# Crocodoctopus/zkstark

Measured on AMD Instinct MI355X. Metric: field-elements/s through LDE+Merkle+FRI (full STARK-101 prover), higher is better.
Workload: dtype u32 (mod 3*2^30+1) + SHA-256

## Files before the change

zkstark_amd/build.py:

```python
import concurrent.futures
import hashlib
import os
import shutil
import subprocess
import sys

HERE = os.path.dirname(os.path.abspath(__file__))
CSRC = os.path.join(HERE, "csrc")
OBJDIR = os.path.join(HERE, "build")
LIB = os.path.join(HERE, "libzkstark_amd.so")
HASHFILE = LIB + ".hash"
SOURCES = ["kernels.hip", "ntt_fast.hip", "domain.hip", "zkstark.hip", "batch.hip", "shard.hip", "verify.hip", "grind.hip", "host_sha.cpp", "version.cpp"]
HEADERS = ["field.hpp", "sha256.hpp", "blake2s.hpp", "sha256_quad.hpp", "fieldhash.hpp", "fieldhash_f64.hpp", "kernels.hpp", "transcript.hpp", "host_sha.hpp", "internal.hpp", "pool.hpp",
           "shard.hpp", "board.hpp", "peer.hpp", os.path.join("..", "..", "include", "zkstark_amd.h")]
ARCH = "gfx950"
FLAGS = ["-O3", "-std=c++17", f"--offload-arch={ARCH}", "-fPIC", "-Wall", "-Wno-unused-function"]
FLAGS += os.environ.get("ZK_BUILD_DEFS", "").split()


def _read(rel):
    with open(os.path.join(CSRC, rel), "rb") as f:
        return f.read()


def source_hash():
    h = hashlib.sha256()
    for rel in SOURCES + HEADERS:
        h.update(os.path.basename(rel).encode() + b"\0")
        h.update(_read(rel))
        h.update(b"\0")
    h.update(" ".join(FLAGS).encode())
    return h.hexdigest()[:24]


def built_hash():
    if not os.path.exists(LIB):
        return None
    try:
        with open(HASHFILE) as f:
            side = f.read().strip()
        if side and os.path.getmtime(HASHFILE) >= os.path.getmtime(LIB):
            return side
    except OSError:
        pass
    try:
        with open(LIB, "rb") as f:
            blob = f.read()
        i = blob.find(b"zkstark_amd.build_hash=")
        if i < 0:
            return None
        tail = blob[i + len(b"zkstark_amd.build_hash="):i + len(b"zkstark_amd.build_hash=") + 64]
        return tail.split(b"\0", 1)[0].decode("ascii", "replace") or None
    except OSError:
        return None


def is_stale():
    return built_hash() != source_hash()


def build(force=False, verbose=False, if_missing_only=False):
    if not force and os.path.exists(LIB) and (if_missing_only or not is_stale()):
        return LIB
    import fcntl
    with open(LIB + ".lock", "w") as lock:
        fcntl.flock(lock, fcntl.LOCK_EX)
        if not force and os.path.exists(LIB) and (if_missing_only or not is_stale()):
            return LIB
        return _build(verbose)


def _compile(hipcc, src, want, headers_blob, verbose):
    extra = [f'-DZK_SRC_HASH="{want}"'] if src == "version.cpp" else []
    key = hashlib.sha256(_read(src) + b"\0" + (want.encode() if extra else headers_blob) + " ".join(FLAGS).encode()).hexdigest()[:20]
    obj = os.path.join(OBJDIR, f"{os.path.splitext(src)[0]}.{key}.o")
    if os.path.exists(obj):
        return obj
    for old in os.listdir(OBJDIR):
        if old.startswith(os.path.splitext(src)[0] + ".") and old.endswith(".o"):
            os.unlink(os.path.join(OBJDIR, old))
    tmp = obj + f".tmp{os.getpid()}"
    cmd = [hipcc] + FLAGS + extra + ["-c", os.path.join(CSRC, src), "-o", tmp]
    if verbose:
        print(" ".join(cmd), file=sys.stderr)
    subprocess.check_call(cmd)
    os.replace(tmp, obj)
    return obj


def _build(verbose):
    hipcc = shutil.which("hipcc") or "/opt/rocm/bin/hipcc"
    if not os.path.exists(hipcc):
        raise RuntimeError("hipcc not found: cannot build libzkstark_amd.so")
    os.makedirs(OBJDIR, exist_ok=True)
    want = source_hash()
    headers_blob = b"\0".join(_read(h) for h in HEADERS)
    workers = max(1, min(len(SOURCES), (os.cpu_count() or 2) - 1, 6))
    with concurrent.futures.ThreadPoolExecutor(workers) as ex:
        objs = list(ex.map(lambda s: _compile(hipcc, s, want, headers_blob, verbose), SOURCES))
    tmp = LIB + f".tmp{os.getpid()}"
    cmd = [hipcc, f"--offload-arch={ARCH}", "-shared", "-fPIC", "-o", tmp] + objs + ["-ldl", "-lpthread", "-lrt"]
    if verbose:
        print(" ".join(cmd), file=sys.stderr)
    subprocess.check_call(cmd)
    os.replace(tmp, LIB)
    with open(HASHFILE + ".tmp", "w") as f:
        f.write(want + "\n")
    os.replace(HASHFILE + ".tmp", HASHFILE)
    return LIB


if __name__ == "__main__":
    print(build(force="--force" in sys.argv, verbose=True))
```

zkstark_amd/csrc/domain.hip:

```cpp
#include <chrono>
#include <cstdarg>
#include <cstdio>
#include <new>

#include "internal.hpp"

namespace zk {
namespace impl {

namespace {
thread_local std::string g_last_error;
}

int fail(int code, const char* fmt, ...) {
    char buf[512];
    va_list ap;
    va_start(ap, fmt);
    vsnprintf(buf, sizeof buf, fmt, ap);
    va_end(ap);
    g_last_error = buf;
    return code;
}
const char* last_error() { return g_last_error.c_str(); }

Plan make_plan(uint32_t log_m) {
    Plan p;
    uint32_t np = (log_m + kMaxRadixLog - 1) / kMaxRadixLog;
    if (np == 0) np = 1;
    uint32_t base = log_m / np, extra = log_m % np;
    p.nd = np;
    for (uint32_t d = 0; d < np; ++d) p.bits[d] = base + (d < extra ? 1 : 0);
    return p;
}

uint32_t pick_logC(uint32_t log_total, uint32_t logR) {
    uint32_t cols = log_total - logR, cap = ntt_pass_tile_log(log_total, logR) - logR;
    return cols < cap ? cols : cap;
}

int build_table(uint32_t root, uint32_t log_order, DevTable* t) {
    uint32_t lo_bits = (log_order + 1) / 2, hi_bits = log_order - lo_bits;
    std::vector<uint32_t> lo((size_t)1 << lo_bits), hi((size_t)1 << hi_bits);
    uint32_t acc = 1;
    for (size_t j = 0; j < lo.size(); ++j) { lo[j] = to_mont(acc); acc = mulmod(acc, root); }
    uint32_t step = powmod(root, (uint64_t)1 << lo_bits);
    acc = 1;
    for (size_t j = 0; j < hi.size(); ++j) { hi[j] = to_mont(acc); acc = mulmod(acc, step); }
    HIPCHK(hipMalloc(&t->lo, lo.size() * 4));
    HIPCHK(hipMalloc(&t->hi, hi.size() * 4));
    HIPCHK(hipMemcpy(t->lo, lo.data(), lo.size() * 4, hipMemcpyHostToDevice));
    HIPCHK(hipMemcpy(t->hi, hi.data(), hi.size() * 4, hipMemcpyHostToDevice));
    t->lo_bits = lo_bits;
    return ZK_OK;
}
void free_table(DevTable* t) {
    if (t->lo) (void)hipFree(t->lo);
    if (t->hi) (void)hipFree(t->hi);
    t->lo = t->hi = nullptr;
}

int run_dif(const uint32_t* src, uint32_t* data, uint32_t log_m, const Plan& pl, PowTable tw_inv, uint32_t L, uint32_t scale_mont, hipStream_t s, Profiler* prof,
            uint32_t batch, size_t src_stride, size_t data_stride) {
    uint32_t inner = log_m;
    for (uint32_t d = 0; d < pl.nd; ++d) {
        inner -= pl.bits[d];
        NttPassArgs a{};
        a.batch = batch; a.src_stride = d == 0 ? src_stride : data_stride; a.dst_stride = data_stride;
        a.src = d == 0 ? src : data; a.dst = data; a.log_total = log_m;
        a.logR = pl.bits[d]; a.logS = inner; a.logC = pick_logC(log_m, a.logR); a.tile_log = ntt_pass_tile_log(log_m, a.logR);
        a.L = L; a.tw = tw_inv; a.scale_mont = (inner == 0) ? scale_mont : 0;
        HIPCHK(launch_ntt_pass(a, NTT_DIF, s, prof));
    }
    return ZK_OK;
}
int run_dit(uint32_t* data, uint32_t log_m, const Plan& pl, PowTable tw, uint32_t L, hipStream_t s) {
    uint32_t inner = 0;
    for (int d = (int)pl.nd - 1; d >= 0; --d) {
        NttPassArgs a{};
        a.src = data; a.dst = data; a.log_total = log_m;
        a.logR = pl.bits[d]; a.logS = inner; a.logC = pick_logC(log_m, a.logR); a.tile_log = ntt_pass_tile_log(log_m, a.logR);
        a.L = L; a.tw = tw;
        HIPCHK(launch_ntt_pass(a, NTT_DIT, s));
        inner += pl.bits[d];
    }
    return ZK_OK;
}



void dom_free(zk_dom* d) {
    if (!d) return;
    free_table(&d->H); free_table(&d->Hinv); free_table(&d->W);
    if (d->d_inv_xm1) (void)hipFree(d->d_inv_xm1);
    delete d;
}

int dom_make(int device, uint32_t log_n, uint32_t log_b, uint32_t shift, bool fold_only, hipStream_t stream, zk_dom** out) {
    *out = nullptr;
    if (log_n < 1 || log_b > 5 || log_n + log_b > 30 || log_n + log_b < 1)
        return fail(ZK_ERR_INVALID, "domain: need 1 <= log_n, log_blowup <= 5, log_n + log_blowup <= 30 (got %u, %u)", log_n, log_b);
    if (shift == 0 || shift >= P) return fail(ZK_ERR_INVALID, "domain: shift must be a non-zero canonical residue");
    HIPCHK(hipSetDevice(device));
    zk_dom* d = new (std::nothrow) zk_dom();
    if (!d) return fail(ZK_ERR_NOMEM, "out of host memory");
    d->device = device;
    d->log_n = log_n; d->log_b = log_b; d->L = log_n + log_b;
    d->n = (size_t)1 << log_n; d->B = (size_t)1 << log_b; d->N = d->n << log_b;
    d->shift = shift;
    d->g = root_of_unity(log_n);
    d->h = root_of_unity(d->L);
    d->plan = make_plan(log_n);
    int rc;
    if ((rc = build_table(d->h, d->L, &d->H)) || (rc = build_table(invmod(d->h), d->L, &d->Hinv))) { dom_free(d); return rc; }
    uint32_t gm1 = invmod(d->g);
    d->shift_mont = to_mont(shift);
    d->gm1_mont = to_mont(gm1);
    d->gm2_mont = to_mont(mulmod(gm1, gm1));
    d->gm3_mont = to_mont(mulmod(mulmod(gm1, gm1), gm1));
    d->ninv_mont = to_mont(invmod((uint32_t)(d->n % P)));
    d->inv2_mont = to_mont(invmod(2));
    {
        const uint32_t inv2 = invmod(2);
        uint32_t wr = shift;
        for (uint32_t r = 0; r < d->L && r < 32; ++r) { d->fold_k[r] = mulmod(invmod(wr), inv2); wr = mulmod(wr, wr); }
        uint32_t xn = powmod(shift, d->n);
        const uint32_t hn = powmod(d->h, d->n);
        for (size_t r = 0; r < d->B; ++r) { const uint32_t den = sub(xn, 1); d->inv_den[r] = den ? invmod(den) : 0u; xn = mulmod(xn, hn); }
    }
    if (!fold_only) {
        if ((rc = build_table(shift, log_n, &d->W))) { dom_free(d); return rc; }
        if (powmod(shift, d->N) == 1) { dom_free(d); return fail(ZK_ERR_INVALID, "domain: shift lies in the evaluation subgroup"); }
        hipError_t e = hipMalloc((void**)&d->d_inv_xm1, d->N * 4);
        if (e != hipSuccess) { dom_free(d); return fail(ZK_ERR_NOMEM, "hipMalloc(%zu) failed", d->N * 4); }
        d->device_bytes += d->N * 4;
        e = launch_build_inv_xm1(d->d_inv_xm1, d->L, d->H.view(), d->shift_mont, stream);
        if (e == hipSuccess) e = hipStreamSynchronize(stream);
        if (e != hipSuccess) { dom_free(d); return fail(ZK_ERR_HIP, "inv_xm1 build failed: %s", hipGetErrorString(e)); }
    }
    *out = d;
    return ZK_OK;
}

int dom_lde(const zk_dom* d, const uint32_t* d_trace, uint32_t* d_coef, uint32_t* d_out, hipStream_t s, Profiler* prof, uint32_t batch) {
    const size_t ts = batch > 1 ? d->n : 0, cs = batch > 1 ? 2 * d->n : 0, os = batch > 1 ? d->N : 0;
    int rc = run_dif(d_trace, d_coef, d->log_n, d->plan, d->Hinv.view(), d->L, 0, s, prof, batch, ts, cs);
    if (rc) return rc;
    uint32_t* d_prep = d_coef + d->n;
    CoefPrepArgs pa{};
    pa.log_n = d->log_n; pa.log_b = d->log_b;
    pa.tw = d->H.view(); pa.wtab = d->W.view(); pa.ninv_mont = d->ninv_mont;
    pa.nd = d->plan.nd;
    for (uint32_t t = 0; t < d->plan.nd; ++t) pa.dig_bits[t] = d->plan.bits[t];
    uint32_t inner = d->log_b;
    for (int q = (int)d->plan.nd - 1; q >= 0; --q) {
        NttPassArgs a{};
        a.log_total = d->L; a.logR = d->plan.bits[q]; a.logS = inner; a.logC = pick_logC(d->L, a.logR); a.tile_log = ntt_pass_tile_log(d->L, a.logR);
        a.L = d->L; a.tw = d->H.view();
        a.dst = d_out;
        a.batch = batch; a.dst_stride = os; a.src_stride = os;
        if (q == (int)d->plan.nd - 1) {
            if (a.logC < d->log_b) a.logC = d->log_b;
            a.src_stride = cs;
            const bool fuse = ntt_fast_ok(a, NTT_DIT_LDE);
            if (fuse) {
                a.src = d_coef;
                a.prep = 1; a.prep_log_n = d->log_n; a.prep_log_b = d->log_b; a.prep_ninv_mont = d->ninv_mont;
                a.prep_nd = d->plan.nd; a.prep_wtab = d->W.view();
                for (uint32_t t = 0; t < d->plan.nd; ++t) a.prep_bits[t] = d->plan.bits[t];
            } else {
                HIPCHK(launch_coef_prepare(d_coef, d_prep, pa, s, prof, batch, cs, cs));
                a.src = d_prep;
            }
            HIPCHK(launch_ntt_pass(a, NTT_DIT_LDE, s, prof));
        } else {
            a.src = d_out;
            HIPCHK(launch_ntt_pass(a, NTT_DIT, s, prof));
        }
        inner += d->plan.bits[q];
    }
    return ZK_OK;
}

int compose_args(const zk_dom* d, const uint32_t* d_f, uint32_t* d_cp, uint32_t first, uint32_t last,
                 const uint32_t alpha_raw[3], ComposeArgs& a) {
    a = ComposeArgs{};
    a.f = d_f; a.inv_xm1 = d->d_inv_xm1; a.cp = d_cp;
    a.logN = d->L; a.log_b = d->log_b;
    a.htab = d->H.view();
    a.w_mont = d->shift_mont; a.gm1_mont = d->gm1_mont; a.gm2_mont = d->gm2_mont; a.gm3_mont = d->gm3_mont;
    a.first = first % P; a.last = last % P;
    uint32_t a0 = alpha_raw[0] % P, a1 = alpha_raw[1] % P, a2 = alpha_raw[2] % P;
    a.alpha0_mont = to_mont(a0);
    a.alpha1g2_mont = to_mont(mulmod(a1, mulmod(d->g, d->g)));
    for (size_t r = 0; r < d->B; ++r) {
        if (d->inv_den[r] == 0) return fail(ZK_ERR_INVALID, "compose: x^n = 1 on the domain");
        a.zz[r] = to_mont(to_mont(mulmod(a2, d->inv_den[r])));
    }
    return ZK_OK;
}
int dom_compose(const zk_dom* d, const uint32_t* d_f, uint32_t* d_cp, uint32_t first, uint32_t last,
                const uint32_t alpha_raw[3], hipStream_t s, Profiler* prof) {
    ComposeArgs a;
    int rc = compose_args(d, d_f, d_cp, first, last, alpha_raw, a);
    if (rc) return rc;
    HIPCHK(launch_compose(a, s, prof));
    return ZK_OK;
}

int fold_args(const zk_dom* d, const uint32_t* d_in, uint32_t* d_out, uint32_t log_m, uint32_t round, uint32_t beta_raw, FoldArgs& a) {
    if (log_m < 1 || log_m + round != d->L) return fail(ZK_ERR_INVALID, "fold: layer size 2^%u does not match round %u of a 2^%u domain", log_m, round, d->L);
    a = FoldArgs{};
    a.in = d_in; a.out = d_out; a.log_m = log_m; a.round = round;
    a.hinv = d->Hinv.view(); a.L = d->L;
    a.inv2_mont = d->inv2_mont;
    a.c_mont = to_mont(mulmod(beta_raw % P, d->fold_k[round]));
    return ZK_OK;
}
int dom_fold(const zk_dom* d, const uint32_t* d_in, uint32_t* d_out, uint32_t log_m, uint32_t round, uint32_t beta_raw,
             hipStream_t s, Profiler* prof) {
    FoldArgs a;
    int rc = fold_args(d, d_in, d_out, log_m, round, beta_raw, a);
    if (rc) return rc;
    HIPCHK(launch_fri_fold(a, s, prof));
    return ZK_OK;
}

int fold_multi_args(const zk_dom* d, const uint32_t* d_in, uint32_t* d_out, uint32_t log_m, uint32_t round, uint32_t steps, uint32_t beta_raw,
                    FoldMultiArgs& a) {
    if (steps < 1 || steps > 3) return fail(ZK_ERR_INVALID, "fold: steps must be 1..3 (got %u)", steps);
    if (log_m < steps || log_m + round != d->L)
        return fail(ZK_ERR_INVALID, "fold: layer size 2^%u does not match round %u + %u steps of a 2^%u domain", log_m, round, steps, d->L);
    a = FoldMultiArgs{};
    a.in = d_in; a.out = d_out; a.log_m = log_m; a.round = round; a.steps = steps;
    a.hinv = d->Hinv.view();
    a.scale_mont = to_mont(invmod(1u << steps));
    const uint32_t S = 1u << steps;
    const uint32_t om_inv = invmod(powmod(d->h, (uint64_t)d->N >> steps));
    uint32_t bk = beta_raw % P, ok = om_inv;
    for (uint32_t k = 0; k < steps; ++k) {
        const uint32_t base = mulmod(bk, mulmod(d->fold_k[round + k], 2));
        uint32_t tw = 1;
        for (uint32_t t = 0; t < (S >> (k + 1)); ++t) { a.c_mont[S - (S >> k) + t] = to_mont(mulmod(base, tw)); tw = mulmod(tw, ok); }
        bk = mulmod(bk, bk); ok = mulmod(ok, ok);
    }
    return ZK_OK;
}
int fold_multi_batch_args(const zk_dom* d, const uint32_t* d_in, uint32_t* d_out, uint32_t log_m, uint32_t round, uint32_t steps,
                          const uint32_t* d_beta_raw, uint32_t beta_stride, uint32_t* d_work, uint32_t batch, FoldMultiBatchArgs& a) {
    a = FoldMultiBatchArgs{};
    if (int rc = fold_multi_args(d, d_in, d_out, log_m, round, steps, 1u, a.a)) return rc;
    if (batch < 1 || ((uint64_t)batch << log_m) > ((uint64_t)1 << 32))
        return fail(ZK_ERR_INVALID, "fold: a batch of %u layers of 2^%u values does not fit 2^32 values", batch, log_m);
    a.beta_raw = d_beta_raw; a.beta_stride = beta_stride; a.cb = d_work; a.batch = batch;
    return ZK_OK;
}
int dom_fold_multi_batch(const zk_dom* d, const uint32_t* d_in, uint32_t* d_out, uint32_t log_m, uint32_t round, uint32_t steps,
                         const uint32_t* d_beta_raw, uint32_t beta_stride, uint32_t* d_work, uint32_t batch, hipStream_t s, Profiler* prof) {
    FoldMultiBatchArgs a;
    int rc = fold_multi_batch_args(d, d_in, d_out, log_m, round, steps, d_beta_raw, beta_stride, d_work, batch, a);
    if (rc) return rc;
    HIPCHK(launch_fri_fold_multi_batch(a, s, prof));
    return ZK_OK;
}
int dom_fold_multi(const zk_dom* d, const uint32_t* d_in, uint32_t* d_out, uint32_t log_m, uint32_t round, uint32_t steps, uint32_t beta_raw,
                   hipStream_t s, Profiler* prof) {
    if (steps == 1) return dom_fold(d, d_in, d_out, log_m, round, beta_raw, s, prof);
    FoldMultiArgs a;
    int rc = fold_multi_args(d, d_in, d_out, log_m, round, steps, beta_raw, a);
    if (rc) return rc;
    HIPCHK(launch_fri_fold_multi(a, s, prof));
    return ZK_OK;
}

int dom_final_poly(const zk_dom* d, const uint32_t* d_in, uint32_t* d_out, uint32_t log_m, uint32_t round, uint32_t bound, hipStream_t s,
                   Profiler* prof, uint32_t polys, size_t in_stride, size_t out_stride) {
    if (log_m < 1 || log_m > kFinalPolyMaxLog || log_m + round != d->L)
        return fail(ZK_ERR_INVALID, "final polynomial: layer size 2^%u does not match round %u of a 2^%u domain, or exceeds 2^%u values", log_m, round, d->L, kFinalPolyMaxLog);
    FinalPolyArgs a{};
    a.in = d_in; a.out = d_out; a.in_stride = in_stride; a.out_stride = out_stride; a.polys = polys;
    a.log_m = log_m; a.bound = bound;
    a.hinv = d->Hinv.view(); a.L = d->L;
    a.minv_mont = to_mont(invmod(1u << log_m));
    a.sinv_mont = to_mont(mulmod(d->fold_k[round], 2));
    HIPCHK(launch_fri_final_poly(a, s, prof));
    return ZK_OK;
}

int dom_final_poly_batch(const zk_dom* d, const uint32_t* d_in, uint32_t* d_out, uint32_t log_m, uint32_t round, uint32_t bound, uint32_t batch,
                         hipStream_t s, Profiler* prof) {
    if (log_m < 1 || log_m > kFinalPolyMaxLog || log_m + round != d->L || bound < 1 || bound > (1u << log_m) || batch < 1)
        return fail(ZK_ERR_INVALID, "final polynomials: %u layers of 2^%u values, bound %u, do not match round %u of a 2^%u domain (at most 2^%u values)",
                    batch, log_m, bound, round, d->L, kFinalPolyMaxLog);
    FinalPolyArgs a{};
    a.in = d_in; a.out = d_out; a.in_stride = (size_t)1 << log_m; a.out_stride = (size_t)bound + 1; a.polys = batch;
    a.log_m = log_m; a.bound = bound;
    a.hinv = d->Hinv.view(); a.L = d->L;
    a.minv_mont = to_mont(invmod(1u << log_m));
    a.sinv_mont = to_mont(mulmod(d->fold_k[round], 2));
    HIPCHK(launch_fri_final_poly_batch(a, s, prof));
    return ZK_OK;
}

int wait_flag(const uint32_t* flag, uint32_t want, hipStream_t stream, int (*poll)(void*), void* poll_user, double timeout_s) {
    auto t0 = std::chrono::steady_clock::now();
    uint64_t spins = 0;
    while (__atomic_load_n(flag, __ATOMIC_ACQUIRE) != want) {
#if !defined(__HIP_DEVICE_COMPILE__) && (defined(__x86_64__) || defined(__i386__))
        __builtin_ia32_pause();
#endif
        if (poll && (++spins & 0xFFF) == 0) {
            if (int prc = poll(poll_user)) return prc;
        } else if (!poll) {
            ++spins;
        }
        if ((spins & 0xFFFF) == 0) {
            hipError_t q = hipStreamQuery(stream);
            if (q == hipSuccess && __atomic_load_n(flag, __ATOMIC_ACQUIRE) != want)
                return fail(ZK_ERR_HIP, "merkle digests were never posted (stream drained)");
            if (q != hipSuccess && q != hipErrorNotReady)
                return fail(ZK_ERR_HIP, "device error while waiting for merkle digests: %s", hipGetErrorString(q));
            if (std::chrono::duration<double>(std::chrono::steady_clock::now() - t0).count() > timeout_s)
                return fail(ZK_ERR_HIP, "timed out after %.0f s waiting for merkle digests", timeout_s);
        }
    }
    return ZK_OK;
}

double now_us() { return std::chrono::duration<double, std::micro>(std::chrono::steady_clock::now().time_since_epoch()).count(); }

void path_nodes(size_t m, size_t leaf, std::vector<size_t>& out) {
    size_t i = leaf + (2 * m - 1) / 2;
    while (i != 0) {
        if (i % 2 == 0) { out.push_back(i - 1); i -= 2; }
        else { out.push_back(i + 1); i -= 1; }
        i >>= 1;
    }
}

}
}
```

zkstark_amd/csrc/host_sha.cpp:

```cpp
#include "host_sha.hpp"

#include <atomic>

#if !defined(__HIP_DEVICE_COMPILE__)
#include <immintrin.h>
#include <stdlib.h>
#include <string.h>

namespace zk {
namespace {

#define ZK_SHA_TARGET __attribute__((target("sha,sse4.1,ssse3")))

alignas(16) const uint32_t K[64] = {
    0x428a2f98u, 0x71374491u, 0xb5c0fbcfu, 0xe9b5dba5u, 0x3956c25bu, 0x59f111f1u, 0x923f82a4u, 0xab1c5ed5u,
    0xd807aa98u, 0x12835b01u, 0x243185beu, 0x550c7dc3u, 0x72be5d74u, 0x80deb1feu, 0x9bdc06a7u, 0xc19bf174u,
    0xe49b69c1u, 0xefbe4786u, 0x0fc19dc6u, 0x240ca1ccu, 0x2de92c6fu, 0x4a7484aau, 0x5cb0a9dcu, 0x76f988dau,
    0x983e5152u, 0xa831c66du, 0xb00327c8u, 0xbf597fc7u, 0xc6e00bf3u, 0xd5a79147u, 0x06ca6351u, 0x14292967u,
    0x27b70a85u, 0x2e1b2138u, 0x4d2c6dfcu, 0x53380d13u, 0x650a7354u, 0x766a0abbu, 0x81c2c92eu, 0x92722c85u,
    0xa2bfe8a1u, 0xa81a664bu, 0xc24b8b70u, 0xc76c51a3u, 0xd192e819u, 0xd6990624u, 0xf40e3585u, 0x106aa070u,
    0x19a4c116u, 0x1e376c08u, 0x2748774cu, 0x34b0bcb5u, 0x391c0cb3u, 0x4ed8aa4au, 0x5b9cca4fu, 0x682e6ff3u,
    0x748f82eeu, 0x78a5636fu, 0x84c87814u, 0x8cc70208u, 0x90befffau, 0xa4506cebu, 0xbef9a3f7u, 0xc67178f2u};
const uint32_t IV[8] = {0x6a09e667u, 0xbb67ae85u, 0x3c6ef372u, 0xa54ff53au, 0x510e527fu, 0x9b05688cu, 0x1f83d9abu, 0x5be0cd19u};

alignas(16) uint32_t PADKW[64];
bool g_cpu_has_sha = false, g_cpu_has_x16 = false;
std::atomic<bool> g_have_sha{false}, g_have_x16{false};
std::atomic<bool> g_want_x16{true};

inline uint32_t rotr(uint32_t x, int n) { return (x >> n) | (x << (32 - n)); }

struct Init {
    Init() {
        __builtin_cpu_init();
        g_cpu_has_sha = __builtin_cpu_supports("sha") && __builtin_cpu_supports("sse4.1") && __builtin_cpu_supports("ssse3");
        g_cpu_has_x16 = g_cpu_has_sha && __builtin_cpu_supports("avx512f");
        g_have_sha = g_cpu_has_sha;
        g_have_x16 = g_cpu_has_x16;
        uint32_t w[64] = {0x80000000u};
        w[15] = 512u;
        for (int t = 16; t < 64; ++t) {
            uint32_t s0 = rotr(w[t - 15], 7) ^ rotr(w[t - 15], 18) ^ (w[t - 15] >> 3);
            uint32_t s1 = rotr(w[t - 2], 17) ^ rotr(w[t - 2], 19) ^ (w[t - 2] >> 10);
            w[t] = w[t - 16] + s0 + w[t - 7] + s1;
        }
        for (int t = 0; t < 64; ++t) PADKW[t] = K[t] + w[t];
    }
} g_init;

ZK_SHA_TARGET inline void load_state(const uint32_t st[8], __m128i& s0, __m128i& s1) {
    __m128i t = _mm_loadu_si128((const __m128i*)st);
    s1 = _mm_loadu_si128((const __m128i*)(st + 4));
    t = _mm_shuffle_epi32(t, 0xB1);
    s1 = _mm_shuffle_epi32(s1, 0x1B);
    s0 = _mm_alignr_epi8(t, s1, 8);
    s1 = _mm_blend_epi16(s1, t, 0xF0);
}
ZK_SHA_TARGET inline void store_state(uint32_t st[8], __m128i s0, __m128i s1) {
    __m128i t = _mm_shuffle_epi32(s0, 0x1B);
    s1 = _mm_shuffle_epi32(s1, 0xB1);
    s0 = _mm_blend_epi16(t, s1, 0xF0);
    s1 = _mm_alignr_epi8(s1, t, 8);
    _mm_storeu_si128((__m128i*)st, s0);
    _mm_storeu_si128((__m128i*)(st + 4), s1);
}

ZK_SHA_TARGET inline void rounds_msg(__m128i& s0, __m128i& s1, __m128i m[4]) {
    const __m128i a0 = s0, a1 = s1;
#pragma GCC unroll 16
    for (int g = 0; g < 16; ++g) {
        __m128i cur = m[g & 3];
        __m128i msg = _mm_add_epi32(cur, _mm_load_si128((const __m128i*)(K + 4 * g)));
        s1 = _mm_sha256rnds2_epu32(s1, s0, msg);
        if (g >= 3 && g <= 14) {
            __m128i t = _mm_alignr_epi8(cur, m[(g + 3) & 3], 4);
            m[(g + 1) & 3] = _mm_sha256msg2_epu32(_mm_add_epi32(m[(g + 1) & 3], t), cur);
        }
        msg = _mm_shuffle_epi32(msg, 0x0E);
        s0 = _mm_sha256rnds2_epu32(s0, s1, msg);
        if (g >= 1 && g <= 12) m[(g + 3) & 3] = _mm_sha256msg1_epu32(m[(g + 3) & 3], cur);
    }
    s0 = _mm_add_epi32(s0, a0);
    s1 = _mm_add_epi32(s1, a1);
}
ZK_SHA_TARGET inline void rounds_pad64(__m128i& s0, __m128i& s1) {
    const __m128i a0 = s0, a1 = s1;
#pragma GCC unroll 16
    for (int g = 0; g < 16; ++g) {
        __m128i msg = _mm_load_si128((const __m128i*)(PADKW + 4 * g));
        s1 = _mm_sha256rnds2_epu32(s1, s0, msg);
        msg = _mm_shuffle_epi32(msg, 0x0E);
        s0 = _mm_sha256rnds2_epu32(s0, s1, msg);
    }
    s0 = _mm_add_epi32(s0, a0);
    s1 = _mm_add_epi32(s1, a1);
}

ZK_SHA_TARGET void inner_ni(const uint32_t* l, const uint32_t* r, uint32_t* out) {
    __m128i s0, s1, m[4];
    load_state(IV, s0, s1);
    m[0] = _mm_loadu_si128((const __m128i*)l);
    m[1] = _mm_loadu_si128((const __m128i*)(l + 4));
    m[2] = _mm_loadu_si128((const __m128i*)r);
    m[3] = _mm_loadu_si128((const __m128i*)(r + 4));
    rounds_msg(s0, s1, m);
    rounds_pad64(s0, s1);
    store_state(out, s0, s1);
}
ZK_SHA_TARGET void inner_ni_x2(const uint32_t* in, uint32_t* out) {
    __m128i s0, s1, u0, u1, m[4], n[4];
    load_state(IV, s0, s1);
    u0 = s0; u1 = s1;
    const __m128i a0 = s0, a1 = s1;
    for (int i = 0; i < 4; ++i) {
        m[i] = _mm_loadu_si128((const __m128i*)(in + 4 * i));
        n[i] = _mm_loadu_si128((const __m128i*)(in + 16 + 4 * i));
    }
#pragma GCC unroll 16
    for (int g = 0; g < 16; ++g) {
        const __m128i k = _mm_load_si128((const __m128i*)(K + 4 * g));
        __m128i cm = m[g & 3], cn = n[g & 3];
        __m128i xm = _mm_add_epi32(cm, k), xn = _mm_add_epi32(cn, k);
        s1 = _mm_sha256rnds2_epu32(s1, s0, xm);
        u1 = _mm_sha256rnds2_epu32(u1, u0, xn);
        if (g >= 3 && g <= 14) {
            __m128i tm = _mm_alignr_epi8(cm, m[(g + 3) & 3], 4), tn = _mm_alignr_epi8(cn, n[(g + 3) & 3], 4);
            m[(g + 1) & 3] = _mm_sha256msg2_epu32(_mm_add_epi32(m[(g + 1) & 3], tm), cm);
            n[(g + 1) & 3] = _mm_sha256msg2_epu32(_mm_add_epi32(n[(g + 1) & 3], tn), cn);
        }
        xm = _mm_shuffle_epi32(xm, 0x0E);
        xn = _mm_shuffle_epi32(xn, 0x0E);
        s0 = _mm_sha256rnds2_epu32(s0, s1, xm);
        u0 = _mm_sha256rnds2_epu32(u0, u1, xn);
        if (g >= 1 && g <= 12) {
            m[(g + 3) & 3] = _mm_sha256msg1_epu32(m[(g + 3) & 3], cm);
            n[(g + 3) & 3] = _mm_sha256msg1_epu32(n[(g + 3) & 3], cn);
        }
    }
    s0 = _mm_add_epi32(s0, a0); s1 = _mm_add_epi32(s1, a1);
    u0 = _mm_add_epi32(u0, a0); u1 = _mm_add_epi32(u1, a1);
    const __m128i b0 = s0, b1 = s1, c0 = u0, c1 = u1;
#pragma GCC unroll 16
    for (int g = 0; g < 16; ++g) {
        __m128i msg = _mm_load_si128((const __m128i*)(PADKW + 4 * g));
        s1 = _mm_sha256rnds2_epu32(s1, s0, msg);
        u1 = _mm_sha256rnds2_epu32(u1, u0, msg);
        msg = _mm_shuffle_epi32(msg, 0x0E);
        s0 = _mm_sha256rnds2_epu32(s0, s1, msg);
        u0 = _mm_sha256rnds2_epu32(u0, u1, msg);
    }
    s0 = _mm_add_epi32(s0, b0); s1 = _mm_add_epi32(s1, b1);
    u0 = _mm_add_epi32(u0, c0); u1 = _mm_add_epi32(u1, c1);
    store_state(out, s0, s1);
    store_state(out + 8, u0, u1);
}
ZK_SHA_TARGET void compress_ni(uint32_t* st, const uint32_t* blk) {
    __m128i s0, s1, m[4];
    load_state(st, s0, s1);
    for (int i = 0; i < 4; ++i) m[i] = _mm_loadu_si128((const __m128i*)(blk + 4 * i));
    rounds_msg(s0, s1, m);
    store_state(st, s0, s1);
}
ZK_SHA_TARGET void blocks_ni(uint32_t* st, const uint8_t* data, size_t blocks) {
    const __m128i be = _mm_set_epi64x(0x0c0d0e0f08090a0bLL, 0x0405060700010203LL);
    __m128i s0, s1, m[4];
    load_state(st, s0, s1);
    for (; blocks; --blocks, data += 64) {
        for (int i = 0; i < 4; ++i) m[i] = _mm_shuffle_epi8(_mm_loadu_si128((const __m128i*)(data + 16 * i)), be);
        rounds_msg(s0, s1, m);
    }
    store_state(st, s0, s1);
}
ZK_SHA_TARGET void leaf_ni(uint32_t v, uint32_t* out) {
    __m128i s0, s1, m[4];
    load_state(IV, s0, s1);
    m[0] = _mm_set_epi32(0, 0, (int)0x80000000u, (int)v);
    m[1] = _mm_setzero_si128();
    m[2] = _mm_setzero_si128();
    m[3] = _mm_set_epi32(32, 0, 0, 0);
    rounds_msg(s0, s1, m);
    store_state(out, s0, s1);
}
#define ZK_X16_TARGET __attribute__((target("avx512f")))
#define ZK_ROR(x, n) _mm512_ror_epi32((x), (n))
#define ZK_XOR3(a, b, c) _mm512_ternarylogic_epi32((a), (b), (c), 0x96)

ZK_X16_TARGET inline void transpose16(__m512i r[16]) {
    __m512i t[16], u[16];
    for (int i = 0; i < 8; ++i) {
        t[2 * i] = _mm512_unpacklo_epi32(r[2 * i], r[2 * i + 1]);
        t[2 * i + 1] = _mm512_unpackhi_epi32(r[2 * i], r[2 * i + 1]);
    }
    for (int i = 0; i < 16; i += 4) {
        u[i] = _mm512_unpacklo_epi64(t[i], t[i + 2]);
        u[i + 1] = _mm512_unpackhi_epi64(t[i], t[i + 2]);
        u[i + 2] = _mm512_unpacklo_epi64(t[i + 1], t[i + 3]);
        u[i + 3] = _mm512_unpackhi_epi64(t[i + 1], t[i + 3]);
    }
    for (int k = 0; k < 4; ++k) {
        t[k] = _mm512_shuffle_i32x4(u[k], u[4 + k], 0x88);
        t[4 + k] = _mm512_shuffle_i32x4(u[k], u[4 + k], 0xdd);
        t[8 + k] = _mm512_shuffle_i32x4(u[8 + k], u[12 + k], 0x88);
        t[12 + k] = _mm512_shuffle_i32x4(u[8 + k], u[12 + k], 0xdd);
    }
    for (int k = 0; k < 4; ++k) {
        r[k] = _mm512_shuffle_i32x4(t[k], t[8 + k], 0x88);
        r[8 + k] = _mm512_shuffle_i32x4(t[k], t[8 + k], 0xdd);
        r[4 + k] = _mm512_shuffle_i32x4(t[4 + k], t[12 + k], 0x88);
        r[12 + k] = _mm512_shuffle_i32x4(t[4 + k], t[12 + k], 0xdd);
    }
}

template <bool MSG>
ZK_X16_TARGET inline void rounds_x16(__m512i st[8], __m512i w[16]) {
    __m512i a = st[0], b = st[1], c = st[2], d = st[3], e = st[4], f = st[5], g = st[6], h = st[7];
#pragma GCC unroll 64
    for (int t = 0; t < 64; ++t) {
        __m512i wk;
        if (MSG) {
            if (t >= 16) {
                const __m512i w15 = w[(t + 1) & 15], w2 = w[(t + 14) & 15];
                const __m512i s0 = ZK_XOR3(ZK_ROR(w15, 7), ZK_ROR(w15, 18), _mm512_srli_epi32(w15, 3));
                const __m512i s1 = ZK_XOR3(ZK_ROR(w2, 17), ZK_ROR(w2, 19), _mm512_srli_epi32(w2, 10));
                w[t & 15] = _mm512_add_epi32(_mm512_add_epi32(w[t & 15], s0), _mm512_add_epi32(w[(t + 9) & 15], s1));
            }
            wk = _mm512_add_epi32(w[t & 15], _mm512_set1_epi32((int)K[t]));
        } else {
            wk = _mm512_set1_epi32((int)PADKW[t]);
        }
        const __m512i S1 = ZK_XOR3(ZK_ROR(e, 6), ZK_ROR(e, 11), ZK_ROR(e, 25));
        const __m512i t1 = _mm512_add_epi32(_mm512_add_epi32(h, S1), _mm512_add_epi32(_mm512_ternarylogic_epi32(e, f, g, 0xCA), wk));
        const __m512i S0 = ZK_XOR3(ZK_ROR(a, 2), ZK_ROR(a, 13), ZK_ROR(a, 22));
        const __m512i t2 = _mm512_add_epi32(S0, _mm512_ternarylogic_epi32(a, b, c, 0xE8));
        h = g; g = f; f = e; e = _mm512_add_epi32(d, t1); d = c; c = b; b = a; a = _mm512_add_epi32(t1, t2);
    }
    st[0] = _mm512_add_epi32(st[0], a); st[1] = _mm512_add_epi32(st[1], b); st[2] = _mm512_add_epi32(st[2], c); st[3] = _mm512_add_epi32(st[3], d);
    st[4] = _mm512_add_epi32(st[4], e); st[5] = _mm512_add_epi32(st[5], f); st[6] = _mm512_add_epi32(st[6], g); st[7] = _mm512_add_epi32(st[7], h);
}
ZK_X16_TARGET inline void store_x16(const __m512i st[8], uint32_t* out) {
    __m512i r[16];
    for (int i = 0; i < 8; ++i) { r[i] = st[i]; r[8 + i] = _mm512_setzero_si512(); }
    transpose16(r);
    for (int n = 0; n < 16; ++n) _mm256_storeu_si256((__m256i*)(out + 8 * n), _mm512_castsi512_si256(r[n]));
}
ZK_X16_TARGET void inner_x16(const uint32_t* in, uint32_t* out) {
    __m512i w[16], st[8];
    for (int n = 0; n < 16; ++n) w[n] = _mm512_loadu_si512((const void*)(in + 16 * n));
    transpose16(w);
    for (int i = 0; i < 8; ++i) st[i] = _mm512_set1_epi32((int)IV[i]);
    rounds_x16<true>(st, w);
    rounds_x16<false>(st, w);
    store_x16(st, out);
}
ZK_X16_TARGET void leaves_x16(const uint32_t* vals, uint32_t* out) {
    __m512i w[16], st[8];
    w[0] = _mm512_loadu_si512((const void*)vals);
    w[1] = _mm512_set1_epi32((int)0x80000000u);
    for (int i = 2; i < 15; ++i) w[i] = _mm512_setzero_si512();
    w[15] = _mm512_set1_epi32(32);
    for (int i = 0; i < 8; ++i) st[i] = _mm512_set1_epi32((int)IV[i]);
    rounds_x16<true>(st, w);
    store_x16(st, out);
}

void inner_run(const uint32_t* child, uint32_t* out, size_t cnt) {
    size_t i = 0;
    if (g_have_x16)
        for (; i + 16 <= cnt; i += 16) inner_x16(child + 16 * i, out + 8 * i);
    for (; i + 2 <= cnt; i += 2) inner_ni_x2(child + 16 * i, out + 8 * i);
    for (; i < cnt; ++i) inner_ni(child + 16 * i, child + 16 * i + 8, out + 8 * i);
}

ZK_SHA_TARGET void reduce_ni(uint32_t* nodes, uint32_t depth) {
    for (uint32_t d = depth; d-- > 0;) {
        const size_t base = ((size_t)1 << d) - 1, child = ((size_t)2 << d) - 1, cnt = (size_t)1 << d;
        inner_run(nodes + 8 * child, nodes + 8 * base, cnt);
    }
}

ZK_SHA_TARGET void reduce_sub_ni(uint32_t* nodes, uint32_t depth, uint32_t top, size_t sub) {
    for (uint32_t d = depth; d-- > top;) {
        const size_t cnt = (size_t)1 << (d - top);
        const size_t base = ((size_t)1 << d) - 1 + sub * cnt, child = ((size_t)2 << d) - 1 + 2 * sub * cnt;
        inner_run(nodes + 8 * child, nodes + 8 * base, cnt);
    }
}

void compress_generic(uint32_t st[8], const uint32_t blk[16]) {
    uint32_t w[64];
    memcpy(w, blk, 64);
    for (int t = 16; t < 64; ++t) {
        uint32_t s0 = rotr(w[t - 15], 7) ^ rotr(w[t - 15], 18) ^ (w[t - 15] >> 3);
        uint32_t s1 = rotr(w[t - 2], 17) ^ rotr(w[t - 2], 19) ^ (w[t - 2] >> 10);
        w[t] = w[t - 16] + s0 + w[t - 7] + s1;
    }
    uint32_t a = st[0], b = st[1], c = st[2], d = st[3], e = st[4], f = st[5], g = st[6], h = st[7];
    for (int t = 0; t < 64; ++t) {
        uint32_t t1 = h + (rotr(e, 6) ^ rotr(e, 11) ^ rotr(e, 25)) + ((e & f) ^ (~e & g)) + K[t] + w[t];
        uint32_t t2 = (rotr(a, 2) ^ rotr(a, 13) ^ rotr(a, 22)) + ((a & b) ^ (a & c) ^ (b & c));
        h = g; g = f; f = e; e = d + t1; d = c; c = b; b = a; a = t1 + t2;
    }
    st[0] += a; st[1] += b; st[2] += c; st[3] += d; st[4] += e; st[5] += f; st[6] += g; st[7] += h;
}

}

bool host_sha_available() { return g_have_sha; }
void host_sha_use_extensions(bool on) {
    g_have_sha = on && g_cpu_has_sha;
    g_have_x16 = on && g_cpu_has_x16 && g_want_x16.load(std::memory_order_relaxed);
}
bool host_sha_wide_available() { return g_have_x16; }
void host_sha_use_wide(bool on) {
    g_want_x16 = on;
    g_have_x16 = on && g_have_sha.load(std::memory_order_relaxed) && g_cpu_has_x16;
}

void host_sha_compress(uint32_t state[8], const uint32_t block[16]) {
    if (g_have_sha) compress_ni(state, block);
    else compress_generic(state, block);
}

void host_sha_blocks(uint32_t state[8], const uint8_t* data, size_t blocks) {
    if (g_have_sha) { blocks_ni(state, data, blocks); return; }
    for (; blocks; --blocks, data += 64) {
        uint32_t w[16];
        for (int i = 0; i < 16; ++i)
            w[i] = ((uint32_t)data[4 * i] << 24) | ((uint32_t)data[4 * i + 1] << 16) | ((uint32_t)data[4 * i + 2] << 8) | data[4 * i + 3];
        compress_generic(state, w);
    }
}

void host_sha_leaf(uint32_t v, uint32_t out[8]) {
    if (g_have_sha) { leaf_ni(v, out); return; }
    uint32_t blk[16] = {v, 0x80000000u, 0, 0, 0, 0, 0, 0, 0, 0, 0, 0, 0, 0, 0, 32u};
    uint32_t st[8];
    memcpy(st, IV, 32);
    compress_generic(st, blk);
    memcpy(out, st, 32);
}

void host_sha_leaves(const uint32_t* vals, size_t n, uint32_t* out) {
    size_t i = 0;
    if (g_have_x16)
        for (; i + 16 <= n; i += 16) leaves_x16(vals + i, out + 8 * i);
    for (; i < n; ++i) host_sha_leaf(vals[i], out + 8 * i);
}

void host_sha_inner(const uint32_t left[8], const uint32_t right[8], uint32_t out[8]) {
    if (g_have_sha) { inner_ni(left, right, out); return; }
    uint32_t blk[16], st[8];
    memcpy(blk, left, 32);
    memcpy(blk + 8, right, 32);
    memcpy(st, IV, 32);
    compress_generic(st, blk);
    uint32_t pad[16] = {0x80000000u, 0, 0, 0, 0, 0, 0, 0, 0, 0, 0, 0, 0, 0, 0, 512u};
    compress_generic(st, pad);
    memcpy(out, st, 32);
}

void host_sha_inner_run(const uint32_t* children, uint32_t* out, size_t cnt) {
    if (g_have_sha) { inner_run(children, out, cnt); return; }
    for (size_t i = 0; i < cnt; ++i) host_sha_inner(children + 16 * i, children + 16 * i + 8, out + 8 * i);
}

void host_sha_reduce_sub(uint32_t* nodes, uint32_t depth, uint32_t top, size_t sub) {
    if (g_have_sha) { reduce_sub_ni(nodes, depth, top, sub); return; }
    for (uint32_t d = depth; d-- > top;) {
        const size_t cnt = (size_t)1 << (d - top);
        const size_t base = ((size_t)1 << d) - 1 + sub * cnt, child = ((size_t)2 << d) - 1 + 2 * sub * cnt;
        for (size_t i = 0; i < cnt; ++i)
            host_sha_inner(nodes + 8 * (child + 2 * i), nodes + 8 * (child + 2 * i + 1), nodes + 8 * (base + i));
    }
}

void host_sha_reduce(uint32_t* nodes, uint32_t depth) {
    if (g_have_sha) { reduce_ni(nodes, depth); return; }
    for (uint32_t d = depth; d-- > 0;) {
        const size_t base = ((size_t)1 << d) - 1, child = ((size_t)2 << d) - 1, cnt = (size_t)1 << d;
        for (size_t i = 0; i < cnt; ++i)
            host_sha_inner(nodes + 8 * (child + 2 * i), nodes + 8 * (child + 2 * i + 1), nodes + 8 * (base + i));
    }
}

}
#endif
```

zkstark_amd/csrc/host_sha.hpp:

```cpp
#pragma once
#include <stddef.h>
#include <stdint.h>

namespace zk {

bool host_sha_available();
void host_sha_use_extensions(bool on);
bool host_sha_wide_available();
void host_sha_use_wide(bool on);
void host_sha_compress(uint32_t state[8], const uint32_t block[16]);
void host_sha_blocks(uint32_t state[8], const uint8_t* data, size_t blocks);
void host_sha_leaf(uint32_t v, uint32_t out[8]);
void host_sha_leaves(const uint32_t* vals, size_t n, uint32_t* out);
void host_sha_inner(const uint32_t left[8], const uint32_t right[8], uint32_t out[8]);
void host_sha_inner_run(const uint32_t* children, uint32_t* out, size_t cnt);
void host_sha_reduce(uint32_t* nodes, uint32_t depth);
void host_sha_reduce_sub(uint32_t* nodes, uint32_t depth, uint32_t top, size_t sub);

}
```

zkstark_amd/csrc/internal.hpp:

```cpp
#pragma once
#include <hip/hip_runtime.h>

#include <cstddef>
#include <cstring>
#include <string>
#include <vector>

#include "../../include/zkstark_amd.h"
#include "field.hpp"
#include "kernels.hpp"
#include "transcript.hpp"

struct zk_channel {
    zk::Channel ch;
};

namespace zk {
namespace impl {

int fail(int code, const char* fmt, ...);
const char* last_error();

#define HIPCHK(expr)                                                                          \
    do {                                                                                      \
        hipError_t _e = (expr);                                                               \
        if (_e != hipSuccess)                                                                 \
            return ::zk::impl::fail(ZK_ERR_HIP, "%s failed: %s (%s:%d)", #expr, hipGetErrorString(_e), __FILE__, __LINE__); \
    } while (0)

template <class T> struct AbiMin;
template <> struct AbiMin<zk_transcript_info> { static constexpr uint32_t v = 1244; static constexpr const char* name = "zk_transcript_info"; };
template <> struct AbiMin<zk_kernel_stat>     { static constexpr uint32_t v = 40;   static constexpr const char* name = "zk_kernel_stat"; };
template <> struct AbiMin<zk_shard_options>   { static constexpr uint32_t v = 48;   static constexpr const char* name = "zk_shard_options"; };
template <> struct AbiMin<zk_shard_stats>     { static constexpr uint32_t v = 112;  static constexpr const char* name = "zk_shard_stats"; };
template <> struct AbiMin<zk_shard_plan_info> { static constexpr uint32_t v = 200;  static constexpr const char* name = "zk_shard_plan_info"; };
template <> struct AbiMin<zk_chain_probe>     { static constexpr uint32_t v = 48;   static constexpr const char* name = "zk_chain_probe"; };
template <class T> inline size_t abi_bytes(const T* p, const char* who) {
    static_assert(sizeof(T) >= AbiMin<T>::v && offsetof(T, struct_size) == 0, "a struct of the C ABI shrank or lost its size field");
    const uint32_t n = p->struct_size;
    if (n < AbiMin<T>::v || n > (1u << 16) || (n > AbiMin<T>::v && n < sizeof(T))) {
        fail(ZK_ERR_INVALID, "%s: %s.struct_size is %u; the caller sets it to sizeof(%s) before the call (ZK_STRUCT_INIT): at least %u bytes "
                             "(ABI version 6), %zu in this library (ABI version %u) -- was the caller compiled against another zkstark_amd.h?",
             who, AbiMin<T>::name, n, AbiMin<T>::name, AbiMin<T>::v, sizeof(T), (unsigned)ZK_ABI_VERSION);
        return 0;
    }
    return n < sizeof(T) ? n : sizeof(T);
}
template <class T> inline int abi_put(T* out, const T& src, const char* who) {
    const size_t k = abi_bytes(out, who);
    if (!k) return ZK_ERR_INVALID;
    memcpy(reinterpret_cast<char*>(out) + sizeof(uint32_t), reinterpret_cast<const char*>(&src) + sizeof(uint32_t), k - sizeof(uint32_t));
    return ZK_OK;
}
template <class T> inline int abi_get(const T* in, T* local, const char* who) {
    const size_t k = abi_bytes(in, who);
    if (!k) return ZK_ERR_INVALID;
    memset(static_cast<void*>(local), 0, sizeof(T));
    memcpy(static_cast<void*>(local), in, k);
    local->struct_size = (uint32_t)sizeof(T);
    return ZK_OK;
}

constexpr uint32_t kMaxQueries = 64;
constexpr uint32_t kHostTopSingle = 8;
constexpr uint32_t kMaxHostLog = 10;
constexpr size_t kMailValsOff = kMailDigests + ((size_t)8 << kMaxHostLog);
constexpr size_t kMailWords = kMailValsOff + ((size_t)2 << kMaxHostLog);
constexpr uint32_t kMaxRadixLog = 8;

inline int check_proof_size(const char* who, uint32_t log_n, uint32_t log_b, uint32_t log_extra = 0) {
    if (log_n < 2 || log_b < 1 || log_b > 5 || log_n + log_b + log_extra > 30)
        return fail(ZK_ERR_INVALID, "%s: need 2 <= log_n, 1 <= log_blowup <= 5, log_n + log_blowup%s <= 30 (got %u, %u)", who,
                    log_extra ? " + log_batch" : "", log_n, log_b);
    if (log_n == 3)
        return fail(ZK_ERR_INVALID, "%s: n = 8 is degenerate for the Fibonacci-square constraints (the degree asserts of prover.rs:156/:169 would fail)", who);
    return ZK_OK;
}

struct Plan {
    uint32_t nd = 0;
    uint32_t bits[kMaxDigits] = {0};
};
Plan make_plan(uint32_t log_m);
uint32_t pick_logC(uint32_t log_total, uint32_t logR);

struct DevTable {
    uint32_t* lo = nullptr;
    uint32_t* hi = nullptr;
    uint32_t lo_bits = 0;
    PowTable view() const { return PowTable{lo, hi, lo_bits}; }
};
int build_table(uint32_t root, uint32_t log_order, DevTable* t);
void free_table(DevTable* t);

int run_dif(const uint32_t* src, uint32_t* data, uint32_t log_m, const Plan& pl, PowTable tw_inv, uint32_t L, uint32_t scale_mont,
            hipStream_t s, Profiler* prof = nullptr, uint32_t batch = 1, size_t src_stride = 0, size_t data_stride = 0);
int run_dit(uint32_t* data, uint32_t log_m, const Plan& pl, PowTable tw, uint32_t L, hipStream_t s);

constexpr uint32_t kGrindHostMaxBits = 10;
struct Grinder;
int grinder_create(int device, void* stream, uint32_t max_jobs, Grinder** out);
void grinder_destroy(Grinder* g);
int grind_device(Grinder* g, const uint8_t* states, size_t count, uint32_t bits, uint64_t start, uint64_t* nonces_out);
int grind_host(const uint8_t state[32], uint32_t bits, uint64_t start, uint32_t threads, uint64_t* nonce_out);
int grind_channel(Grinder* g, Channel& ch, uint32_t bits, uint64_t* nonce_out);

}
}

struct zk_dom {
    int device = 0;
    uint32_t log_n = 0, log_b = 0, L = 0;
    size_t n = 0, N = 0, B = 0;
    uint32_t shift = 0, g = 0, h = 0;
    zk::impl::DevTable H, Hinv, W;
    uint32_t* d_inv_xm1 = nullptr;
    zk::impl::Plan plan;
    uint32_t shift_mont = 0, gm1_mont = 0, gm2_mont = 0, gm3_mont = 0, ninv_mont = 0, inv2_mont = 0;
    uint32_t fold_k[32] = {0};
    uint32_t inv_den[32] = {0};
    size_t device_bytes = 0;
};

namespace zk {
namespace impl {

void dom_free(zk_dom* d);
int dom_make(int device, uint32_t log_n, uint32_t log_b, uint32_t shift, bool fold_only, hipStream_t stream, zk_dom** out);
int dom_lde(const zk_dom* d, const uint32_t* d_trace, uint32_t* d_coef, uint32_t* d_out, hipStream_t s, Profiler* prof, uint32_t batch = 1);
int compose_args(const zk_dom* d, const uint32_t* d_f, uint32_t* d_cp, uint32_t first, uint32_t last, const uint32_t alpha_raw[3], ComposeArgs& a);
int dom_compose(const zk_dom* d, const uint32_t* d_f, uint32_t* d_cp, uint32_t first, uint32_t last, const uint32_t alpha_raw[3],
                hipStream_t s, Profiler* prof);
int fold_args(const zk_dom* d, const uint32_t* d_in, uint32_t* d_out, uint32_t log_m, uint32_t round, uint32_t beta_raw, FoldArgs& a);
int dom_fold(const zk_dom* d, const uint32_t* d_in, uint32_t* d_out, uint32_t log_m, uint32_t round, uint32_t beta_raw, hipStream_t s,
             Profiler* prof);
int fold_multi_args(const zk_dom* d, const uint32_t* d_in, uint32_t* d_out, uint32_t log_m, uint32_t round, uint32_t steps, uint32_t beta_raw,
                    FoldMultiArgs& a);
int dom_fold_multi(const zk_dom* d, const uint32_t* d_in, uint32_t* d_out, uint32_t log_m, uint32_t round, uint32_t steps, uint32_t beta_raw,
                   hipStream_t s, Profiler* prof = nullptr);
int dom_final_poly(const zk_dom* d, const uint32_t* d_in, uint32_t* d_out, uint32_t log_m, uint32_t round, uint32_t bound, hipStream_t s,
                   Profiler* prof = nullptr, uint32_t polys = 1, size_t in_stride = 0, size_t out_stride = 0);
int dom_final_poly_batch(const zk_dom* d, const uint32_t* d_in, uint32_t* d_out, uint32_t log_m, uint32_t round, uint32_t bound, uint32_t batch,
                         hipStream_t s, Profiler* prof = nullptr);
int fold_multi_batch_args(const zk_dom* d, const uint32_t* d_in, uint32_t* d_out, uint32_t log_m, uint32_t round, uint32_t steps,
                          const uint32_t* d_beta_raw, uint32_t beta_stride, uint32_t* d_work, uint32_t batch, FoldMultiBatchArgs& a);
int dom_fold_multi_batch(const zk_dom* d, const uint32_t* d_in, uint32_t* d_out, uint32_t log_m, uint32_t round, uint32_t steps,
                         const uint32_t* d_beta_raw, uint32_t beta_stride, uint32_t* d_work, uint32_t batch, hipStream_t s,
                         Profiler* prof = nullptr);

int wait_flag(const uint32_t* flag, uint32_t want, hipStream_t stream, int (*poll)(void*) = nullptr, void* poll_user = nullptr, double timeout_s = 30.0);
double now_us();
int tail_open_begin(zk_ctx* tail, size_t x);
int tail_open_end(zk_ctx* tail, uint32_t* vals_out, uint8_t* paths_out);
void path_nodes(size_t m, size_t leaf, std::vector<size_t>& out);
int merkle_nodes_to_host(int device, hipStream_t s, const uint32_t* d_heap, size_t first, size_t count, uint8_t* out);

}
}
```

zkstark_amd/csrc/kernels.hip:

```cpp
#include "kernels.hpp"

#include <cstdlib>

#include "blake2s.hpp"
#include "field.hpp"
#include "fieldhash_f64.hpp"
#include "sha256_quad.hpp"
#include "sha256.hpp"

namespace zk {

__device__ __forceinline__ uint32_t pow_lookup(const PowTable& t, uint32_t e) {
    return mont_mul(t.hi[e >> t.lo_bits], t.lo[e & ((1u << t.lo_bits) - 1u)]);
}

constexpr uint32_t R2_MONT = R2;

__device__ uint32_t mont_inv(uint32_t a) {
    uint32_t r = R1, b = a;
    uint32_t e = P - 2;
#pragma unroll 1
    for (int i = 0; i < 32; ++i) {
        if (e & 1) r = mont_mul(r, b);
        b = mont_mul(b, b);
        e >>= 1;
    }
    return r;
}


constexpr int kNttThreads = 256;

__device__ __forceinline__ void tile_coords(uint32_t l, uint32_t logR, uint32_t logS, uint32_t logC,
                                            uint32_t& t, uint32_t& c) {
    if (logS >= logC) {
        t = l >> logC;
        c = l & ((1u << logC) - 1u);
    } else {
        uint32_t s = l & ((1u << logS) - 1u);
        t = (l >> logS) & ((1u << logR) - 1u);
        c = ((l >> (logR + logS)) << logS) | s;
    }
}

template <uint32_t MODE>
__global__ __launch_bounds__(kNttThreads) void ntt_pass_kernel(NttPassArgs p) {
    extern __shared__ __attribute__((aligned(16))) uint32_t smem[];
    p.src += (size_t)blockIdx.y * p.src_stride;
    p.dst += (size_t)blockIdx.y * p.dst_stride;
    const uint32_t logR = p.logR, logS = p.logS, logC = p.logC;
    const uint32_t R = 1u << logR, C = 1u << logC, pitch = C + 1u;
    uint32_t* tile = smem;
    uint32_t* twl = smem + R * pitch;
    const uint32_t tid = threadIdx.x;
    const uint32_t col0 = blockIdx.x << logC;
    const uint32_t tile_elems = R << logC;
    const uint32_t tw_shift = p.L - logR - logS;
    const uint32_t smask = (1u << logS) - 1u;

    for (uint32_t j = tid; j < (R >> 1); j += kNttThreads) twl[j] = pow_lookup(p.tw, j << (p.L - logR));

    if (MODE == NTT_DIT_LDE) {
        const uint32_t logB = logS;
        const uint32_t a0 = col0 >> logB;
        for (uint32_t u = tid; u < (tile_elems >> logB); u += kNttThreads) {
            uint32_t ao = u >> logR, t = u & (R - 1u);
            uint32_t v = p.src[((size_t)(a0 + ao) << logR) | t];
            uint32_t row = __brev(t) >> (32u - logR);
            uint32_t* dstp = &tile[row * pitch + (ao << logB)];
            dstp[0] = v;
            for (uint32_t s = 1; s <= smask; ++s) dstp[s] = mont_mul(v, pow_lookup(p.tw, (t * s) << tw_shift));
        }
    } else {
        for (uint32_t l = tid; l < tile_elems; l += kNttThreads) {
            uint32_t t, c;
            tile_coords(l, logR, logS, logC, t, c);
            uint32_t col = col0 + c, a = col >> logS, s = col & smask;
            size_t addr = ((size_t)a << (logR + logS)) | ((size_t)t << logS) | s;
            uint32_t v = p.src[addr];
            uint32_t row = t;
            if (MODE == NTT_DIT) {
                if (logS) v = mont_mul(v, pow_lookup(p.tw, (t * s) << tw_shift));
                row = __brev(t) >> (32u - logR);
            }
            tile[row * pitch + c] = v;
        }
    }
    __syncthreads();

    const uint32_t nb = tile_elems >> 1;
    if (MODE == NTT_DIF) {
        for (int ll = (int)logR - 1; ll >= 0; --ll) {
            for (uint32_t b = tid; b < nb; b += kNttThreads) {
                uint32_t c = b & (C - 1u), pi = b >> logC;
                uint32_t j = pi & ((1u << ll) - 1u);
                uint32_t i = ((pi >> ll) << (ll + 1)) | j;
                uint32_t* x0 = &tile[i * pitch + c];
                uint32_t* x1 = x0 + (pitch << ll);
                uint32_t u = *x0, v = *x1;
                *x0 = add(u, v);
                *x1 = mont_mul(sub(u, v), twl[j << (logR - 1u - ll)]);
            }
            __syncthreads();
        }
    } else {
        for (uint32_t ll = 0; ll < logR; ++ll) {
            for (uint32_t b = tid; b < nb; b += kNttThreads) {
                uint32_t c = b & (C - 1u), pi = b >> logC;
                uint32_t j = pi & ((1u << ll) - 1u);
                uint32_t i = ((pi >> ll) << (ll + 1)) | j;
                uint32_t* x0 = &tile[i * pitch + c];
                uint32_t* x1 = x0 + (pitch << ll);
                uint32_t u = *x0, v = mont_mul(*x1, twl[j << (logR - 1u - ll)]);
                *x0 = add(u, v);
                *x1 = sub(u, v);
            }
            __syncthreads();
        }
    }

    for (uint32_t l = tid; l < tile_elems; l += kNttThreads) {
        uint32_t t, c;
        tile_coords(l, logR, logS, logC, t, c);
        uint32_t col = col0 + c, a = col >> logS, s = col & smask;
        size_t addr = ((size_t)a << (logR + logS)) | ((size_t)t << logS) | s;
        uint32_t v;
        if (MODE == NTT_DIF) {
            v = tile[(__brev(t) >> (32u - logR)) * pitch + c];
            if (logS) v = mont_mul(v, pow_lookup(p.tw, (t * s) << tw_shift));
            else if (p.scale_mont) v = mont_mul(v, p.scale_mont);
        } else {
            v = tile[t * pitch + c];
        }
        p.dst[addr] = v;
    }
}

bool launch_ntt_pass_fast(const NttPassArgs& a, NttMode mode, hipStream_t s, hipError_t* err);

hipError_t launch_ntt_pass(const NttPassArgs& a, NttMode mode, hipStream_t s, Profiler* prof) {
    double bytes = mode == NTT_DIT_LDE ? 4.0 * ((double)((size_t)1 << (a.log_total - a.logS)) + (double)((size_t)1 << a.log_total))
                                       : 8.0 * (double)((size_t)1 << a.log_total);
    const uint32_t batch = a.batch ? a.batch : 1;
    ScopedKernelTimer tm(prof, K_NTT, bytes * batch, s, kNttOpsPerElement * (double)((size_t)1 << a.log_total) * batch * (double)a.logR / 7.0);
    hipError_t ferr = hipSuccess;
    if (launch_ntt_pass_fast(a, mode, s, &ferr)) return ferr;
    uint32_t cols_log = a.log_total - a.logR;
    uint32_t blocks = 1u << (cols_log - a.logC);
    size_t shmem = ((size_t)(1u << a.logR) * ((1u << a.logC) + 1u) + (1u << a.logR) / 2u) * sizeof(uint32_t);
    switch (mode) {
        case NTT_DIF: hipLaunchKernelGGL(ntt_pass_kernel<NTT_DIF>, dim3(blocks, batch), dim3(kNttThreads), shmem, s, a); break;
        case NTT_DIT: hipLaunchKernelGGL(ntt_pass_kernel<NTT_DIT>, dim3(blocks, batch), dim3(kNttThreads), shmem, s, a); break;
        case NTT_DIT_LDE: hipLaunchKernelGGL(ntt_pass_kernel<NTT_DIT_LDE>, dim3(blocks, batch), dim3(kNttThreads), shmem, s, a); break;
    }
    return hipGetLastError();
}

__global__ __launch_bounds__(256) void coef_prepare_kernel(const uint32_t* U, uint32_t* out, CoefPrepArgs a, size_t u_stride, size_t out_stride) {
    const uint32_t pos = blockIdx.x * blockDim.x + threadIdx.x, n = 1u << a.log_n;
    if (pos >= n) return;
    U += (size_t)blockIdx.y * u_stride;
    out += (size_t)blockIdx.y * out_stride;
    uint32_t k = 0, rem = a.log_n, sh = 0;
    for (uint32_t d = 0; d < a.nd; ++d) {
        rem -= a.dig_bits[d];
        k |= ((pos >> rem) & ((1u << a.dig_bits[d]) - 1u)) << sh;
        sh += a.dig_bits[d];
    }
    const uint32_t c_top = U[n - 1u];
    uint32_t v = sub(U[pos], mont_mul(c_top, pow_lookup(a.tw, ((k + 1u) & (n - 1u)) << a.log_b)));
    out[pos] = mont_mul(v, mont_mul(pow_lookup(a.wtab, k), a.ninv_mont));
}

hipError_t launch_coef_prepare(const uint32_t* U, uint32_t* out, const CoefPrepArgs& a, hipStream_t s, Profiler* prof,
                               uint32_t batch, size_t u_stride, size_t out_stride) {
    uint32_t n = 1u << a.log_n;
    ScopedKernelTimer tm(prof, K_NTT, 8.0 * n * batch, s);
    hipLaunchKernelGGL(coef_prepare_kernel, dim3((n + 255) / 256, batch), dim3(256), 0, s, U, out, a, u_stride, out_stride);
    return hipGetLastError();
}

struct DigitArgs {
    uint32_t nd;
    uint32_t bits[kMaxDigits];
};

__global__ void digit_reverse_kernel(const uint32_t* in, uint32_t* out, uint32_t log_m, DigitArgs dg, int to_natural) {
    size_t pos = (size_t)blockIdx.x * blockDim.x + threadIdx.x;
    if (pos >= ((size_t)1 << log_m)) return;
    uint32_t k = 0, rem = log_m, sh = 0;
    for (uint32_t d = 0; d < dg.nd; ++d) {
        rem -= dg.bits[d];
        k |= (((uint32_t)pos >> rem) & ((1u << dg.bits[d]) - 1u)) << sh;
        sh += dg.bits[d];
    }
    if (to_natural) out[k] = in[pos];
    else out[pos] = in[k];
}

hipError_t launch_digit_reverse(const uint32_t* in, uint32_t* out, uint32_t log_m, uint32_t nd,
                                const uint32_t* dig_bits, int to_natural, hipStream_t s) {
    DigitArgs dg{};
    dg.nd = nd;
    for (uint32_t i = 0; i < nd; ++i) dg.bits[i] = dig_bits[i];
    size_t m = (size_t)1 << log_m;
    uint32_t threads = 256, blocks = (uint32_t)((m + threads - 1) / threads);
    hipLaunchKernelGGL(digit_reverse_kernel, dim3(blocks), dim3(threads), 0, s, in, out, log_m, dg, to_natural);
    return hipGetLastError();
}

__global__ void degree_check_kernel(const uint32_t* coef, uint32_t log_m, DigitArgs dg, uint32_t bound, uint32_t* out) {
    size_t pos = (size_t)blockIdx.x * blockDim.x + threadIdx.x;
    if (pos >= ((size_t)1 << log_m)) return;
    uint32_t k = 0, rem = log_m, sh = 0;
    for (uint32_t d = 0; d < dg.nd; ++d) {
        rem -= dg.bits[d];
        k |= (((uint32_t)pos >> rem) & ((1u << dg.bits[d]) - 1u)) << sh;
        sh += dg.bits[d];
    }
    const uint32_t v = coef[pos];
    if (k >= bound && v != 0) atomicAdd(&out[0], 1u);
    if (k + 1 == bound) out[1] = v;
}
hipError_t launch_degree_check(const uint32_t* coef, uint32_t log_m, uint32_t nd, const uint32_t* dig_bits, uint32_t bound, uint32_t* out, hipStream_t s) {
    DigitArgs dg{};
    dg.nd = nd;
    for (uint32_t i = 0; i < nd; ++i) dg.bits[i] = dig_bits[i];
    size_t m = (size_t)1 << log_m;
    hipLaunchKernelGGL(degree_check_kernel, dim3((uint32_t)((m + 255) / 256)), dim3(256), 0, s, coef, log_m, dg, bound, out);
    return hipGetLastError();
}


constexpr int kInvBatch = 8;

__global__ __launch_bounds__(256) void build_inv_xm1_kernel(uint32_t* out, size_t count, uint32_t e0, uint32_t order_mask, PowTable htab, uint32_t w_mont) {
    size_t gid = (size_t)blockIdx.x * blockDim.x + threadIdx.x;
    size_t base = gid * kInvBatch;
    if (base >= count) return;
    uint32_t d[kInvBatch], pre[kInvBatch];
    uint32_t acc = R1;
#pragma unroll
    for (int e = 0; e < kInvBatch; ++e) {
        size_t i = base + e;
        uint32_t x = i < count ? mont_mul(pow_lookup(htab, (e0 + (uint32_t)i) & order_mask), w_mont) : add(R1, R1);
        d[e] = sub(x, R1);
        pre[e] = acc;
        acc = mont_mul(acc, d[e]);
    }
    uint32_t inv = mont_inv(acc);
#pragma unroll
    for (int e = kInvBatch - 1; e >= 0; --e) {
        size_t i = base + e;
        uint32_t r = mont_mul(inv, pre[e]);
        inv = mont_mul(inv, d[e]);
        if (i < count) out[i] = r;
    }
}

hipError_t launch_build_inv_xm1_range(uint32_t* out, size_t count, uint32_t e0, uint32_t log_order, PowTable htab, uint32_t shift_mont, hipStream_t s) {
    size_t threads_total = (count + kInvBatch - 1) / kInvBatch;
    uint32_t blocks = (uint32_t)((threads_total + 255) / 256);
    if (!blocks) return hipSuccess;
    hipLaunchKernelGGL(build_inv_xm1_kernel, dim3(blocks), dim3(256), 0, s, out, count, e0, (uint32_t)(((uint64_t)1 << log_order) - 1u), htab, shift_mont);
    return hipGetLastError();
}
hipError_t launch_build_inv_xm1(uint32_t* out, uint32_t logN, PowTable htab, uint32_t shift_mont, hipStream_t s) {
    return launch_build_inv_xm1_range(out, (size_t)1 << logN, 0u, logN, htab, shift_mont, s);
}

struct ComposeRaw { uint32_t f0, f1, f2, inv0, inv2, x_hi, x_lo, zz; };
__device__ __forceinline__ ComposeRaw compose_fetch(const ComposeArgs& a, const uint32_t* f, size_t i) {
    const size_t N = (size_t)1 << a.logN;
    const uint32_t B = 1u << a.log_b;
    const size_t i1 = (i + B) & (N - 1), i2 = (i + 2 * (size_t)B) & (N - 1);
    ComposeRaw r;
    r.f0 = f[i]; r.f1 = f[i1]; r.f2 = f[i2];
    r.inv0 = a.inv_xm1[i]; r.inv2 = a.inv_xm1[i2];
    r.x_hi = a.htab.hi[(uint32_t)i >> a.htab.lo_bits]; r.x_lo = a.htab.lo[(uint32_t)i & ((1u << a.htab.lo_bits) - 1u)];
    r.zz = a.zz[i & (B - 1)];
    return r;
}
template <bool BATCH>
__device__ __forceinline__ uint32_t compose_eval(const ComposeArgs& a, uint32_t f0, uint32_t f1, uint32_t f2, uint32_t inv0, uint32_t inv2,
                                                 uint32_t x, uint32_t zz, uint32_t first, uint32_t last, uint32_t al0, uint32_t al1g2, uint32_t al2) {
    uint32_t t0 = mont_mul(mont_mul(sub(f0, first), inv0), al0);
    uint32_t t1 = mont_mul(mont_mul(sub(f0, last), inv2), al1g2);
    uint32_t v3 = mont_mul(mont_mul(sub(x, a.gm3_mont), sub(x, a.gm2_mont)), sub(x, a.gm1_mont));
    uint32_t y = mont_mul(v3, zz);
    if (BATCH) y = mont_mul(y, al2);
    uint32_t num = sub(sub(mont_mul(f2, 1u), mont_mul(f1, f1)), mont_mul(f0, f0));
    uint32_t t2 = mont_mul(num, y);
    return add(add(t0, t1), t2);
}
template <bool BATCH>
__device__ __forceinline__ uint32_t compose_finish(const ComposeArgs& a, const ComposeRaw& r, uint32_t first, uint32_t last, uint32_t al0,
                                                   uint32_t al1g2, uint32_t al2) {
    const uint32_t x = mont_mul(mont_mul(r.x_hi, r.x_lo), a.w_mont);
    return compose_eval<BATCH>(a, r.f0, r.f1, r.f2, r.inv0, r.inv2, x, r.zz, first, last, al0, al1g2, al2);
}
template <bool BATCH>
__device__ __forceinline__ uint32_t compose_core(const ComposeArgs& a, const uint32_t* f, uint32_t first, uint32_t last, uint32_t al0,
                                                 uint32_t al1g2, uint32_t al2, size_t i) {
    return compose_finish<BATCH>(a, compose_fetch(a, f, i), first, last, al0, al1g2, al2);
// ... 818 lines not shown
            }
            __syncthreads();
            Digest d0;
            if (active && is_main) {
#pragma unroll
                for (int i = 0; i < 16; ++i) wv[i] = xb0[i * 128 + node];
                sha256_rounds16<48>(st, wv);
#pragma unroll
                for (int i = 0; i < 8; ++i) d0.w[i] = st[i] + SHA_IV[i];
                uint32_t pad[16] = {0x80000000u, 0, 0, 0, 0, 0, 0, 0, 0, 0, 0, 0, 0, 0, 0, 512u};
                sha256_compress(d0.w, pad);
            }
            __syncthreads();
            if (active && is_main) { lds_store(&lvl[2 * node], d0); store_digest(nodes, out_base + node, d0); }
            __syncthreads();
            continue;
        }
        if (HASH == 1 && w > kFieldRowMaxNodes && w <= kFieldQuadMaxNodes) {
            const uint32_t q = tid & 3u, grp = tid >> 2;
            uint32_t res[2][4];
#pragma unroll
            for (uint32_t b = 0; b < 2; ++b) {
                if (b * 64 >= w) break;
                const uint32_t node = b * 64 + grp;
                const uint4 v = lvl[4 * (node < w ? node : 0u) + q];
                const uint32_t in[4] = {v.x, v.y, v.z, v.w};
                fieldhash_inner_quad_f64(in, q, res[b], g_fh_consts64);
            }
            __syncthreads();
#pragma unroll
            for (uint32_t b = 0; b < 2; ++b) {
                if (b * 64 >= w) break;
                const uint32_t node = b * 64 + grp;
                if (node < w && q < 2) {
                    const uint4 o = make_uint4(res[b][0], res[b][1], res[b][2], res[b][3]);
                    lvl[2 * node + q] = o;
                    reinterpret_cast<uint4*>(nodes + (out_base + node) * 8)[q] = o;
                }
            }
            __syncthreads();
            continue;
        }
        if (HASH == 1 && w <= kFieldRowMaxNodes) {
            const uint32_t g = tid & 15u, grp = tid >> 4;
            uint32_t res[4];
#pragma unroll
            for (uint32_t b = 0; b < 4; ++b) {
                if (b * 16 >= w) break;
                const uint32_t node = b * 16 + grp;
                const uint32_t* words = reinterpret_cast<const uint32_t*>(&lvl[4 * (node < w ? node : 0u)]);
                res[b] = fieldhash_inner_row16_f64(words[g], g, g_fh_consts64);
            }
            __syncthreads();
#pragma unroll
            for (uint32_t b = 0; b < 4; ++b) {
                if (b * 16 >= w) break;
                const uint32_t node = b * 16 + grp;
                if (node < w && g < 8) {
                    reinterpret_cast<uint32_t*>(&lvl[2 * node])[g] = res[b];
                    nodes[(out_base + node) * 8 + g] = res[b];
                }
            }
            __syncthreads();
            continue;
        }
        Digest d0, d1;
        const bool a0 = tid < w, a1 = tid + kWgThreads < w;
        if (a0) d0 = Hasher<HASH>::inner(lds_digest(&lvl[4 * tid]), lds_digest(&lvl[4 * tid + 2]));
        if (a1) d1 = Hasher<HASH>::inner(lds_digest(&lvl[4 * (tid + kWgThreads)]), lds_digest(&lvl[4 * (tid + kWgThreads) + 2]));
        __syncthreads();
        if (a0) { lds_store(&lvl[2 * tid], d0); store_digest(nodes, out_base + tid, d0); }
        if (a1) { lds_store(&lvl[2 * (tid + kWgThreads)], d1); store_digest(nodes, out_base + tid + kWgThreads, d1); }
        __syncthreads();
    }
    WG_STAMP((phase ? 24u : 2u) + lv);
    if (phase == 1 || j2 == 0) break;
    __shared__ uint32_t go_on;
    if (gridDim.x > 1) {
        if (kWgRelaxedPublish) {
            publish_node(nodes, (((size_t)1 << (depth_in - j)) - 1) + blockIdx.x, lvl, tid);
        } else {
            asm volatile("s_waitcnt vmcnt(0)" ::: "memory");
            __syncthreads();
        }
    }
    if (tid == 0) {
        uint32_t last = 1;
        if (gridDim.x > 1) {
            last = (kWgRelaxedPublish ? __hip_atomic_fetch_add(mail.counter + 1, 1u, __ATOMIC_RELAXED, __HIP_MEMORY_SCOPE_AGENT)
                                      : __hip_atomic_fetch_add(mail.counter + 1, 1u, __ATOMIC_ACQ_REL, __HIP_MEMORY_SCOPE_AGENT)) == gridDim.x - 1;
            if (last) __hip_atomic_store(mail.counter + 1, 0u, __ATOMIC_RELAXED, __HIP_MEMORY_SCOPE_AGENT);
        }
        go_on = last;
    }
    __syncthreads();
    if (!go_on) return;
    if (kWgRelaxedPublish && LEAF && mail.dump_src) __builtin_amdgcn_fence(__ATOMIC_ACQUIRE, "agent");
#ifdef ZK_WG_TRACE
    if (tid == 0) wg_rec = __hip_atomic_load(&g_wg_trace_cur, __ATOMIC_RELAXED, __HIP_MEMORY_SCOPE_AGENT);
    WG_STAMP(15);
#endif
    d_in = depth_in - j; lv = j2; cnt = gridDim.x; first = 0;
    {
        const size_t base2 = ((size_t)1 << d_in) - 1;
        Digest dd[kPer];
#pragma unroll
        for (uint32_t u = 0; u < kPer; ++u)
            if (tid + u * kWgThreads < cnt)
                dd[u] = (kWgRelaxedPublish && gridDim.x > 1) ? load_digest_agent(nodes, base2 + tid + u * kWgThreads) : load_digest(nodes, base2 + tid + u * kWgThreads);
#pragma unroll
        for (uint32_t u = 0; u < kPer; ++u)
            if (tid + u * kWgThreads < cnt) lds_store(&lvl[2 * (tid + u * kWgThreads)], dd[u]);
    }
    __syncthreads();
    WG_STAMP(16);
  }
    if (mail.mailbox && depth_in - j - j2 == mail.top && off == 0) {
        __shared__ uint32_t is_last;
        const bool relaxed = kWgRelaxedPublish && gridDim.x > 1 && j2 == 0 && mail.dump_src == nullptr;
        if (relaxed) publish_node(nodes, (((size_t)1 << mail.top) - 1) + blockIdx.x, lvl, tid);
        if (tid == 0) {
            uint32_t last = 1;
            if (gridDim.x > 1 && j2 == 0) {
                last = (relaxed ? __hip_atomic_fetch_add(mail.counter, 1u, __ATOMIC_RELAXED, __HIP_MEMORY_SCOPE_AGENT)
                                : __hip_atomic_fetch_add(mail.counter, 1u, __ATOMIC_ACQ_REL, __HIP_MEMORY_SCOPE_AGENT)) == gridDim.x - 1;
                if (last) __hip_atomic_store(mail.counter, 0u, __ATOMIC_RELAXED, __HIP_MEMORY_SCOPE_AGENT);
            }
            is_last = last;
        }
        __syncthreads();
        if (is_last) {
#ifdef ZK_WG_TRACE
            if (tid == 0 && wg_rec == 0xffffffffu) wg_rec = __hip_atomic_load(&g_wg_trace_cur, __ATOMIC_RELAXED, __HIP_MEMORY_SCOPE_AGENT);
            WG_STAMP(40);
#endif
            const uint4* sq = reinterpret_cast<const uint4*>(nodes + (((size_t)1 << mail.top) - 1) * 8);
            uint4* dq = reinterpret_cast<uint4*>(mail.mailbox + kMailDigests);
            if (relaxed) {
                for (uint32_t i = tid; i < (1u << mail.top); i += kWgThreads) {
                    const Digest d = load_digest_agent(nodes, (((size_t)1 << mail.top) - 1) + i);
                    dq[2 * i] = make_uint4(d.w[0], d.w[1], d.w[2], d.w[3]);
                    dq[2 * i + 1] = make_uint4(d.w[4], d.w[5], d.w[6], d.w[7]);
                }
            } else {
                for (uint32_t i = tid; i < (2u << mail.top); i += kWgThreads) dq[i] = sq[i];
            }
            if (mail.dump_src) {
                const uint4* sv = reinterpret_cast<const uint4*>(mail.dump_src);
                uint4* dv = reinterpret_cast<uint4*>(mail.mailbox + mail.vals_off);
                for (uint32_t i = tid; i < (1u << mail.dump_log) / 4; i += kWgThreads) dv[i] = sv[i];
            }
            __threadfence_system();
            __syncthreads();
            WG_STAMP(41);
            if (tid == 0) __hip_atomic_store(&mail.mailbox[0], mail.seq, __ATOMIC_RELEASE, __HIP_MEMORY_SCOPE_SYSTEM);
            WG_STAMP(42);
        }
    }
}

#ifdef ZK_WG_TRACE
void dump_wg_trace() {
    const char* path = getenv("ZK_WG_TRACE_FILE");
    unsigned int n = 0;
    if (!path || hipMemcpyFromSymbol(&n, HIP_SYMBOL(g_wg_trace_n), sizeof n) != hipSuccess || !n) return;
    if (n > kWgTraceLaunches) n = kWgTraceLaunches;
    std::vector<unsigned long long> rec((size_t)n * kWgTraceSlots);
    if (hipMemcpyFromSymbol(rec.data(), HIP_SYMBOL(g_wg_trace), rec.size() * 8) != hipSuccess) return;
    FILE* f = fopen(path, "a");
    if (!f) return;
    for (unsigned int r = 0; r < n; ++r) {
        const unsigned long long* x = &rec[(size_t)r * kWgTraceSlots];
        const unsigned long long m = x[0];
        fprintf(f, "wg depth_in=%llu j=%llu j2=%llu leaf=%llu hash=%llu top=%lld wgs=%llu abs0=%llu :", m & 255, (m >> 8) & 255, (m >> 16) & 255, (m >> 24) & 1, (m >> 25) & 1,
                (long long)((m >> 26) & 63) - 1, m >> 32, x[1]);
        for (uint32_t i = 1; i < kWgTraceSlots; ++i) fprintf(f, " %lld", x[i] ? (long long)(x[i] - x[1]) : -1LL);
        fprintf(f, "\n");
    }
    fclose(f);
    const unsigned int zero = 0;
    (void)hipMemcpyToSymbol(HIP_SYMBOL(g_wg_trace_n), &zero, sizeof zero);
}
#endif

template <int HASH, int S>
__device__ __forceinline__ Digest coset_leaf_digest(const uint32_t (&v)[S]) {
    Digest d;
    if (HASH == ZK_HASH_BLAKE2S) {
        d = blake2s_slots<S>(v);
    } else if (HASH == ZK_HASH_FIELD) {
        uint32_t in[kFhT];
#pragma unroll
        for (int i = 0; i < kFhT; ++i) in[i] = i < S ? v[i] : 0u;
        in[kFhT - 1] = (uint32_t)S;
        fh64_compress(in, d.w, g_fh_consts64);
    } else {
        uint32_t w[16];
#pragma unroll
        for (int i = 0; i < 16; ++i) w[i] = i < S ? v[i] : 0u;
        w[S] = 0x80000000u;
        w[15] = 32u * S;
#pragma unroll
        for (int i = 0; i < 8; ++i) d.w[i] = SHA_IV[i];
        sha256_compress(d.w, w);
    }
    return d;
}
constexpr int kCosetThreads = 256;
template <int HASH, int STEPS>
__global__ __launch_bounds__(kCosetThreads) void coset_leaf_hash_kernel(const uint32_t* __restrict__ layer, uint32_t log_len, uint32_t* __restrict__ nodes) {
    constexpr int S = 1 << STEPS;
    const size_t leaves = (size_t)1 << (log_len - STEPS);
    const size_t stride = (size_t)gridDim.x * kCosetThreads;
    size_t c = (size_t)blockIdx.x * kCosetThreads + threadIdx.x;
    if (c >= leaves) return;
    uint32_t v[S], nx[S] = {};
#pragma unroll
    for (int u = 0; u < S; ++u) v[u] = layer[c + (size_t)u * leaves];
    bool more;
#pragma unroll 1
    do {
        const size_t cn = c + stride;
        more = cn < leaves;
        if (more) {
#pragma unroll
            for (int u = 0; u < S; ++u) nx[u] = layer[cn + (size_t)u * leaves];
        }
        store_digest(nodes, leaves - 1 + c, coset_leaf_digest<HASH, S>(v));
#pragma unroll
        for (int u = 0; u < S; ++u) v[u] = nx[u];
        c = cn;
    } while (more);
}

static double merkle_bytes(bool leaf, uint32_t depth, uint32_t k) {
    double in = (double)((size_t)1 << depth);
    double produced = (leaf ? in : 0.0) + in * (1.0 - 1.0 / (double)((size_t)1 << k));
    return (leaf ? 4.0 : 32.0) * in + 32.0 * produced;
}
static double hash_leaf_ops(int hash) { return hash == ZK_HASH_FIELD ? kFieldLeafOps : hash == ZK_HASH_BLAKE2S ? kB2sLeafOps : kShaLeafOps; }
static double merkle_ops(bool leaf, uint32_t depth, uint32_t k, int hash) {
    double in = (double)((size_t)1 << depth);
    double lo = hash_leaf_ops(hash), io = hash == ZK_HASH_FIELD ? kFieldInnerOps : hash == ZK_HASH_BLAKE2S ? kB2sInnerOps : kShaInnerOps;
    return (leaf ? in * lo : 0.0) + in * (1.0 - 1.0 / (double)((size_t)1 << k)) * io;
}

static hipError_t ensure_fieldhash_consts() {
    static bool done[64] = {false};
    int dev = 0;
    hipError_t e = hipGetDevice(&dev);
    if (e != hipSuccess) return e;
    if (dev < 0 || dev >= 64 || done[dev]) return hipSuccess;
    FieldHashConsts c;
    fieldhash_make_consts(c);
    e = hipMemcpyToSymbol(HIP_SYMBOL(g_fh_consts), &c, sizeof c);
    if (e != hipSuccess) return e;
    static FieldHashConsts64 c64;
    fieldhash_make_consts64(c, c64);
    e = hipMemcpyToSymbol(HIP_SYMBOL(g_fh_consts64), &c64, sizeof c64);
    if (e == hipSuccess) done[dev] = true;
    return e;
}

#ifndef ZK_MERKLE_MAX_K
#define ZK_MERKLE_MAX_K 4
#endif
#ifndef ZK_MERKLE_LATENCY_LOG
#define ZK_MERKLE_LATENCY_LOG 17
#endif
#ifndef ZK_MERKLE_CHUNK_K
#define ZK_MERKLE_CHUNK_K 3
#endif
static_assert(ZK_MERKLE_MAX_K >= 1 && ZK_MERKLE_MAX_K <= (int)kMerkleMaxK && ZK_MERKLE_CHUNK_K >= 1 && ZK_MERKLE_CHUNK_K <= (int)kMerkleMaxK, "levels per launch");
static_assert(ZK_MERKLE_LATENCY_LOG >= 12 && ZK_MERKLE_LATENCY_LOG <= 24, "latency switch");
static uint32_t g_merkle_latency_log = ZK_MERKLE_LATENCY_LOG;
static constexpr uint32_t merkle_max_k() { return ZK_MERKLE_MAX_K; }
static uint32_t merkle_latency_log() { return __atomic_load_n(&g_merkle_latency_log, __ATOMIC_RELAXED); }
bool set_merkle_latency_log(uint32_t v) {
    if (v == 0) v = ZK_MERKLE_LATENCY_LOG;
    if (v < 12 || v > 24) return false;
    __atomic_store_n(&g_merkle_latency_log, v, __ATOMIC_RELAXED);
    return true;
}

constexpr double kB2sLevelUs = kB2sInnerOps * 4.6 / kShaInnerOps, kB2sLeafUs = kB2sLeafOps * 2.6 / kShaLeafOps;
static double wg_level_us(uint32_t w, int hash) {
    if (w == 0) return 0.0;
    if (hash == ZK_HASH_BLAKE2S) return (double)((w + 255) / 256) * kB2sLevelUs;
    if (hash == ZK_HASH_FIELD) return w <= kFieldRowMaxNodes ? (double)((w + 15) / 16) * 3.7 : w <= kFieldQuadMaxNodes ? (double)((w + 63) / 64) * 5.3 : (double)((w + 255) / 256) * 10.8;
    return w <= 64 ? 3.1 : w <= 128 ? 4.9 : (double)((w + 255) / 256) * 4.6;
}
static double wg_phase_us(bool leaf, uint32_t cnt_log, uint32_t levels, int hash, uint32_t blocks) {
    const uint32_t cnt = 1u << cnt_log;
    double us = !leaf ? 1.0
                : hash == ZK_HASH_FIELD ? (cnt <= kFieldRowLeafMax ? (double)((cnt + 15) / 16) * 3.7 : (double)((cnt + 255) / 256) * 10.8)
                : (double)((cnt + 255) / 256) * (hash == ZK_HASH_BLAKE2S ? kB2sLeafUs : 2.6);
    for (uint32_t t = 1; t <= levels; ++t) us += wg_level_us(cnt >> t, hash);
    return blocks > 256 ? us * (double)blocks / 256.0 : us;
}
#ifndef ZK_MERKLE_CONTINUATION
#define ZK_MERKLE_CONTINUATION 1
#endif
static constexpr bool g_merkle_continuation = ZK_MERKLE_CONTINUATION != 0;
constexpr double kContinueUs = 6.0;
constexpr double kLaunchUs = 10.0;

template <class SRC>
static hipError_t merkle_build_t(SRC src, double src_bytes, uint32_t log_m, uint32_t* nodes, hipStream_t s, Profiler* prof,
                                 const MailArgs& mail_in, int hash, uint32_t log_sub = 0xffffffffu, size_t chunk = 0,
                                 bool leaf_mode = true, uint32_t tp_floor = 0) {
    if (hash == ZK_HASH_BLAKE2S && !B2sSrc<SRC>::ok) return hipErrorInvalidValue;
    if (hash == ZK_HASH_FIELD) {
        hipError_t e = ensure_fieldhash_consts();
        if (e != hipSuccess) return e;
    }
    if (log_sub == 0xffffffffu) log_sub = log_m;
    const uint32_t stop = log_m - log_sub;
    uint32_t depth = log_m;
    bool leaf = leaf_mode;
    const PlainSrc none{nullptr};
    auto first_bytes = [&](double b) { return leaf ? b - 4.0 * (double)((size_t)1 << log_sub) + src_bytes : b; };
    const uint32_t kMerkleLatencyLog = merkle_latency_log();
    auto off_at = [&](uint32_t d) { return (size_t)chunk << (d - stop); };
    const bool throughput_only = tp_floor != 0;
    const uint32_t floor_depth = throughput_only ? tp_floor : stop + kMerkleLatencyLog;
    while (depth > floor_depth) {
        uint32_t k = depth - floor_depth;
        if (k > merkle_max_k()) k = merkle_max_k();
        size_t lanes = (size_t)1 << (depth - stop - k);
        uint32_t blocks = (uint32_t)(lanes / kMerkleThreads);
        size_t sh = (size_t)(kMerkleThreads / 64) * (k + 1) * 128 * sizeof(uint4);
        ScopedKernelTimer tm(prof, leaf ? K_MERKLE_LEAF : K_MERKLE_INNER, first_bytes(merkle_bytes(leaf, depth - stop, k)), s, merkle_ops(leaf, depth - stop, k, hash));
        if (hash == ZK_HASH_BLAKE2S) {
            if constexpr (B2sSrc<SRC>::ok) {
                if (leaf) hipLaunchKernelGGL((b2s_subtree_kernel<SRC, true>), dim3(blocks), dim3(kMerkleThreads), sh, s, src, nodes, depth, k, off_at(depth));
                else hipLaunchKernelGGL((b2s_subtree_kernel<PlainSrc, false>), dim3(blocks), dim3(kMerkleThreads), sh, s, none, nodes, depth, k, off_at(depth));
            }
        } else if (hash == ZK_HASH_FIELD) {
            if (leaf) hipLaunchKernelGGL((merkle_subtree_kernel<SRC, true, 1>), dim3(blocks), dim3(kMerkleThreads), sh, s, src, nodes, depth, k, off_at(depth));
            else hipLaunchKernelGGL((merkle_subtree_kernel<PlainSrc, false, 1>), dim3(blocks), dim3(kMerkleThreads), sh, s, none, nodes, depth, k, off_at(depth));
        } else {
            if (leaf) hipLaunchKernelGGL((merkle_subtree_kernel<SRC, true, 0>), dim3(blocks), dim3(kMerkleThreads), sh, s, src, nodes, depth, k, off_at(depth));
            else hipLaunchKernelGGL((merkle_subtree_kernel<PlainSrc, false, 0>), dim3(blocks), dim3(kMerkleThreads), sh, s, none, nodes, depth, k, off_at(depth));
        }
        leaf = false;
        depth -= k;
    }
    if (throughput_only) return hipGetLastError();
    MailArgs mail = mail_in;
    if (stop != 0 || mail.top >= log_m) mail.top = 0;
    const uint32_t end = stop == 0 ? mail.top : stop;
    auto launch_wg = [&](uint32_t j, uint32_t j2) {
        const uint32_t span = depth - stop;
        const uint32_t blocks = 1u << (span - j);
        const uint32_t lds_log = j2 && span - j > j ? span - j : j;
        const size_t sh = ((size_t)2 << lds_log) * sizeof(uint4) + 2 * 16 * 128 * sizeof(uint32_t);
        ScopedKernelTimer tm(prof, K_MERKLE_TOP, first_bytes(merkle_bytes(leaf, span, j)) + (j2 ? merkle_bytes(false, span - j, j2) : 0.0), s,
                             merkle_ops(leaf, span, j, hash) + (j2 ? merkle_ops(false, span - j, j2, hash) : 0.0));
        if (hash == ZK_HASH_BLAKE2S) {
            if constexpr (B2sSrc<SRC>::ok) {
                if (leaf) hipLaunchKernelGGL((merkle_wg_kernel<SRC, true, 2>), dim3(blocks), dim3(kWgThreads), sh, s, src, nodes, depth, j, mail, off_at(depth), j2, lds_log);
                else hipLaunchKernelGGL((merkle_wg_kernel<PlainSrc, false, 2>), dim3(blocks), dim3(kWgThreads), sh, s, none, nodes, depth, j, mail, off_at(depth), j2, lds_log);
            }
        } else if (hash == ZK_HASH_FIELD) {
            if (leaf) hipLaunchKernelGGL((merkle_wg_kernel<SRC, true, 1>), dim3(blocks), dim3(kWgThreads), sh, s, src, nodes, depth, j, mail, off_at(depth), j2, lds_log);
            else hipLaunchKernelGGL((merkle_wg_kernel<PlainSrc, false, 1>), dim3(blocks), dim3(kWgThreads), sh, s, none, nodes, depth, j, mail, off_at(depth), j2, lds_log);
        } else {
            if (leaf) hipLaunchKernelGGL((merkle_wg_kernel<SRC, true, 0>), dim3(blocks), dim3(kWgThreads), sh, s, src, nodes, depth, j, mail, off_at(depth), j2, lds_log);
            else hipLaunchKernelGGL((merkle_wg_kernel<PlainSrc, false, 0>), dim3(blocks), dim3(kWgThreads), sh, s, none, nodes, depth, j, mail, off_at(depth), j2, lds_log);
        }
        leaf = false;
        depth -= j + j2;
    };
    const bool may_continue = stop == 0 && mail.counter != nullptr && g_merkle_continuation;
    do {
        const uint32_t span = depth - stop;
        const uint32_t levels = depth - end;
        const uint32_t launches = levels ? (levels + kWgMaxLog - 1) / kWgMaxLog : 1;
        const uint32_t jn = (levels + launches - 1) / launches;
        uint32_t best_j = jn, best_j2 = 0;
        if (may_continue && levels <= 2 * kWgMaxLog) {
            double best = wg_phase_us(leaf, jn, jn, hash, 1u << (span - jn));
            if (launches == 2 && span - jn <= kWgMaxLog) best += kLaunchUs + wg_phase_us(false, span - jn, levels - jn, hash, 1);
            else if (launches > 1) best = 0.0;
            for (uint32_t j = 1; j < levels && j <= kWgMaxLog; ++j) {
                const uint32_t j2 = levels - j;
                if (j2 > kWgMaxLog || span - j > kWgMaxLog) continue;
                const double us = wg_phase_us(leaf, j, j, hash, 1u << (span - j)) + kContinueUs + wg_phase_us(false, span - j, j2, hash, 1);
                if (us < best) { best = us; best_j = j; best_j2 = j2; }
            }
        }
        launch_wg(best_j, best_j2);
    } while (depth > end);
    return hipGetLastError();
}

hipError_t launch_merkle_build(const uint32_t* vals, uint32_t log_m, uint32_t* nodes, hipStream_t s, Profiler* prof,
                               const MailArgs& mail, int hash) {
    return merkle_build_t(PlainSrc{vals}, 4.0 * (double)((size_t)1 << log_m), log_m, nodes, s, prof, mail, hash);
}
template <int HASH>
static void coset_leaf_launch(const uint32_t* vals, uint32_t log_len, uint32_t steps, uint32_t* nodes, uint32_t blocks, hipStream_t s) {
    const dim3 g(blocks), b(kCosetThreads);
    if (steps == 1) hipLaunchKernelGGL((coset_leaf_hash_kernel<HASH, 1>), g, b, 0, s, vals, log_len, nodes);
    else if (steps == 2) hipLaunchKernelGGL((coset_leaf_hash_kernel<HASH, 2>), g, b, 0, s, vals, log_len, nodes);
    else hipLaunchKernelGGL((coset_leaf_hash_kernel<HASH, 3>), g, b, 0, s, vals, log_len, nodes);
}
hipError_t launch_merkle_build_coset(const uint32_t* vals, uint32_t log_len, uint32_t steps, uint32_t* nodes, hipStream_t s, Profiler* prof,
                                     const MailArgs& mail, int hash) {
    if (steps == 0) return launch_merkle_build(vals, log_len, nodes, s, prof, mail, hash);
    if (steps > 3 || log_len <= steps) return hipErrorInvalidValue;
    if (hash == ZK_HASH_FIELD) {
        hipError_t e = ensure_fieldhash_consts();
        if (e != hipSuccess) return e;
    }
    const uint32_t log_m = log_len - steps;
    const size_t leaves = (size_t)1 << log_m;
    const size_t lanes = leaves > 4 * (size_t)kCosetThreads ? leaves / 4 : leaves;
    const uint32_t blocks = (uint32_t)((lanes + kCosetThreads - 1) / kCosetThreads);
    {
        ScopedKernelTimer tm(prof, K_MERKLE_LEAF, 4.0 * (double)((size_t)1 << log_len) + 32.0 * (double)leaves, s,
                             (double)leaves * hash_leaf_ops(hash));
        if (hash == ZK_HASH_BLAKE2S) coset_leaf_launch<2>(vals, log_len, steps, nodes, blocks, s);
        else if (hash == ZK_HASH_FIELD) coset_leaf_launch<1>(vals, log_len, steps, nodes, blocks, s);
        else coset_leaf_launch<0>(vals, log_len, steps, nodes, blocks, s);
    }
    hipError_t e = hipGetLastError();
    if (e != hipSuccess) return e;
    return merkle_build_t(PlainSrc{nullptr}, 0.0, log_m, nodes, s, prof, mail, hash, log_m, 0, false);
}
template <int HASH, int STEPS>
__global__ __launch_bounds__(kCosetThreads) void coset_leaf_hash_batch_kernel(const uint32_t* __restrict__ vals, uint32_t log_len, uint32_t log_batch,
                                                                              uint32_t* __restrict__ nodes) {
    constexpr int S = 1 << STEPS;
    const uint32_t log_m = log_len - STEPS;
    const size_t m = (size_t)1 << log_m;
    const size_t total = m << log_batch;
    const size_t stride = (size_t)gridDim.x * kCosetThreads;
    size_t g = (size_t)blockIdx.x * kCosetThreads + threadIdx.x;
    if (g >= total) return;
    uint32_t v[S], nx[S] = {};
    {
        const uint32_t* src = vals + ((g >> log_m) << log_len) + (g & (m - 1));
#pragma unroll
        for (int u = 0; u < S; ++u) v[u] = src[(size_t)u * m];
    }
    bool more;
#pragma unroll 1
    do {
        const size_t gn = g + stride;
        more = gn < total;
        if (more) {
            const uint32_t* src = vals + ((gn >> log_m) << log_len) + (gn & (m - 1));
#pragma unroll
            for (int u = 0; u < S; ++u) nx[u] = src[(size_t)u * m];
        }
        store_digest(nodes, total - 1 + g, coset_leaf_digest<HASH, S>(v));
#pragma unroll
        for (int u = 0; u < S; ++u) v[u] = nx[u];
        g = gn;
    } while (more);
}
template <int HASH>
static void coset_leaf_batch_launch(const uint32_t* vals, uint32_t log_len, uint32_t steps, uint32_t log_batch, uint32_t* nodes, uint32_t blocks,
                                    hipStream_t s) {
    const dim3 g(blocks), b(kCosetThreads);
    if (steps == 1) hipLaunchKernelGGL((coset_leaf_hash_batch_kernel<HASH, 1>), g, b, 0, s, vals, log_len, log_batch, nodes);
    else if (steps == 2) hipLaunchKernelGGL((coset_leaf_hash_batch_kernel<HASH, 2>), g, b, 0, s, vals, log_len, log_batch, nodes);
    else hipLaunchKernelGGL((coset_leaf_hash_batch_kernel<HASH, 3>), g, b, 0, s, vals, log_len, log_batch, nodes);
}
hipError_t launch_merkle_build_coset_batch(const uint32_t* vals, uint32_t log_len, uint32_t steps, uint32_t log_batch, uint32_t* nodes, hipStream_t s,
                                           Profiler* prof, const MailArgs& mail, int hash) {
    if (steps < 1 || steps > 3 || log_len <= steps || log_len + log_batch > 32) return hipErrorInvalidValue;
    if (hash == ZK_HASH_BLAKE2S) return hipErrorInvalidValue;
    if (hash == ZK_HASH_FIELD) {
        hipError_t e = ensure_fieldhash_consts();
        if (e != hipSuccess) return e;
    }
    const uint32_t log_m = log_len - steps + log_batch;
    const size_t leaves = (size_t)1 << log_m;
    const size_t lanes = leaves > 4 * (size_t)kCosetThreads ? leaves / 4 : leaves;
    const uint32_t blocks = (uint32_t)((lanes + kCosetThreads - 1) / kCosetThreads);
    {
        ScopedKernelTimer tm(prof, K_MERKLE_LEAF, 4.0 * (double)((size_t)1 << (log_len + log_batch)) + 32.0 * (double)leaves, s,
                             (double)leaves * hash_leaf_ops(hash));
        if (hash == ZK_HASH_FIELD) coset_leaf_batch_launch<1>(vals, log_len, steps, log_batch, nodes, blocks, s);
        else coset_leaf_batch_launch<0>(vals, log_len, steps, log_batch, nodes, blocks, s);
    }
    hipError_t e = hipGetLastError();
    if (e != hipSuccess) return e;
    return merkle_build_t(PlainSrc{nullptr}, 0.0, log_m, nodes, s, prof, mail, hash, log_m, 0, false);
}
hipError_t launch_merkle_build_interleaved(const uint32_t* recv, uint32_t log_parts, uint32_t log_cnt, uint32_t* nodes, hipStream_t s,
                                           Profiler* prof, int hash, const MailArgs& mail) {
    uint32_t log_m = log_parts + log_cnt;
    return merkle_build_t(InterleaveSrc{recv, log_parts, log_cnt}, 4.0 * (double)((size_t)1 << log_m), log_m, nodes, s, prof, mail, hash);
}
static constexpr uint32_t merkle_chunk_k() { return ZK_MERKLE_CHUNK_K; }
static uint32_t chunk_handover_depth(uint32_t log_m, uint32_t log_chunks) {
    const uint32_t lat = merkle_latency_log();
    if (!(log_m > lat && lat >= log_chunks + 8)) return log_chunks;
    uint32_t k = log_m - lat < merkle_max_k() ? log_m - lat : merkle_max_k();
    if (k > merkle_chunk_k()) k = merkle_chunk_k();
    return log_m - k;
}
uint32_t merkle_finish_start_depth(uint32_t log_m, uint32_t log_chunks) { return chunk_handover_depth(log_m, log_chunks); }
hipError_t launch_merkle_build_chunk(const uint32_t* recv, uint32_t log_parts, uint32_t log_cnt, uint32_t* nodes, uint32_t log_m,
                                     uint32_t chunk, hipStream_t s, Profiler* prof, int hash) {
    uint32_t log_sub = log_parts + log_cnt;
    const uint32_t h = chunk_handover_depth(log_m, log_m - log_sub);
    return merkle_build_t(InterleaveSrc{recv, log_parts, log_cnt}, 4.0 * (double)((size_t)1 << log_sub), log_m, nodes, s, prof, MailArgs{}, hash,
                          log_sub, chunk, true, h != log_m - log_sub ? h : 0u);
}
hipError_t launch_merkle_finish(uint32_t* nodes, uint32_t log_m, uint32_t log_chunks, hipStream_t s, Profiler* prof, int hash,
                                const MailArgs& mail) {
    const uint32_t start = chunk_handover_depth(log_m, log_chunks);
    if (start == 0) return hipSuccess;
    return merkle_build_t(PlainSrc{nullptr}, 0.0, start, nodes, s, prof, mail, hash, start, 0, false);
}
hipError_t launch_fold_merkle(const FoldArgs& a, uint32_t* nodes, hipStream_t s, Profiler* prof, const MailArgs& mail, int hash) {
    uint32_t log_out = a.log_m - 1;
    return merkle_build_t(FoldSrc{a}, 12.0 * (double)((size_t)1 << log_out), log_out, nodes, s, prof, mail, hash);
}
hipError_t launch_compose_merkle(const ComposeArgs& a, uint32_t* nodes, hipStream_t s, Profiler* prof, const MailArgs& mail, int hash) {
    return merkle_build_t(ComposeSrc{a}, 8.0 * (double)((size_t)1 << a.logN), a.logN, nodes, s, prof, mail, hash);
}

hipError_t launch_compose_block_merkle(const ComposeBlockArgs& b, uint32_t* nodes, hipStream_t s, Profiler* prof, const MailArgs& mail, int hash) {
    return merkle_build_t(ComposeBlockSrc{b}, 8.0 * (double)((size_t)1 << b.log_m), b.log_m, nodes, s, prof, mail, hash);
}

hipError_t launch_compose_merkle_batch(const ComposeBatchArgs& a, uint32_t log_batch, uint32_t* nodes, hipStream_t s, Profiler* prof,
                                       const MailArgs& mail, int hash) {
    uint32_t log_m = a.a.logN + log_batch;
    return merkle_build_t(ComposeBatchSrc{a.a, a.chal}, 8.0 * (double)((size_t)1 << log_m), log_m, nodes, s, prof, mail, hash);
}
hipError_t launch_fold_merkle_batch(const FoldBatchArgs& a, uint32_t log_batch, uint32_t* nodes, hipStream_t s, Profiler* prof,
                                    const MailArgs& mail, int hash) {
    uint32_t log_out = a.a.log_m - 1 + log_batch;
    return merkle_build_t(FoldBatchSrc{a.a, a.chal}, 12.0 * (double)((size_t)1 << log_out), log_out, nodes, s, prof, mail, hash);
}

__global__ __launch_bounds__(1024) void scatter_kernel(const uint32_t* stage, const ScatterSeg* segs, uint32_t* trees, uint32_t* layers) {
    const ScatterSeg sg = segs[blockIdx.x];
    uint32_t* dst = (sg.kind ? layers : trees) + sg.dst;
    const uint32_t* src = stage + sg.src;
    if (((sg.src | sg.dst | sg.words) & 3) == 0) {
        const uint4* s4 = reinterpret_cast<const uint4*>(src);
        uint4* d4 = reinterpret_cast<uint4*>(dst);
        for (uint32_t i = threadIdx.x; i < sg.words / 4; i += blockDim.x) d4[i] = s4[i];
    } else {
        for (uint32_t i = threadIdx.x; i < sg.words; i += blockDim.x) dst[i] = src[i];
    }
}
hipError_t launch_scatter(const uint32_t* stage, const ScatterSeg* segs, uint32_t count, double words, uint32_t* trees, uint32_t* layers,
                          hipStream_t s, Profiler* prof) {
    if (!count) return hipSuccess;
    ScopedKernelTimer tm(prof, K_GATHER, 8.0 * words, s);
    hipLaunchKernelGGL(scatter_kernel, dim3(count), dim3(1024), 0, s, stage, segs, trees, layers);
    return hipGetLastError();
}

template <int HASH>
__global__ __launch_bounds__(256) void hash_chain_probe_kernel(uint32_t* out, uint32_t seed, uint32_t hashes, unsigned long long* rec) {
    Digest d;
#pragma unroll
    for (int i = 0; i < 8; ++i) d.w[i] = (seed * (uint32_t)(i + 1) + threadIdx.x + blockIdx.x * 977u) % P;
    const unsigned long long c0 = __builtin_amdgcn_s_memtime(), r0 = __builtin_amdgcn_s_memrealtime();
#pragma unroll 1
    for (uint32_t it = 0; it < hashes; ++it) {
        Digest r = d;
        r.w[0] ^= seed;
        if (HASH == ZK_HASH_FIELD) r.w[0] &= 0x7fffffffu;
        d = Hasher<HASH>::inner(d, r);
    }
    const unsigned long long c1 = __builtin_amdgcn_s_memtime(), r1 = __builtin_amdgcn_s_memrealtime();
    uint32_t x = 0;
#pragma unroll
    for (int i = 0; i < 8; ++i) x ^= d.w[i];
    out[blockIdx.x * 256 + threadIdx.x] = x;
    if (rec && (threadIdx.x & 63) == 0) {
        rec[((size_t)blockIdx.x * 4 + (threadIdx.x >> 6)) * 2] = c1 - c0;
        rec[((size_t)blockIdx.x * 4 + (threadIdx.x >> 6)) * 2 + 1] = r1 - r0;
    }
}
hipError_t launch_hash_chain_probe(int hash, uint32_t blocks, uint32_t* out, uint32_t seed, uint32_t hashes, unsigned long long* rec, hipStream_t s) {
    if (hash == ZK_HASH_BLAKE2S) {
        hipLaunchKernelGGL(hash_chain_probe_kernel<2>, dim3(blocks), dim3(256), 0, s, out, seed, hashes, rec);
    } else if (hash == ZK_HASH_FIELD) {
        hipError_t e = ensure_fieldhash_consts();
        if (e != hipSuccess) return e;
        hipLaunchKernelGGL(hash_chain_probe_kernel<1>, dim3(blocks), dim3(256), 0, s, out, seed, hashes, rec);
    } else {
        hipLaunchKernelGGL(hash_chain_probe_kernel<0>, dim3(blocks), dim3(256), 0, s, out, seed, hashes, rec);
    }
    return hipGetLastError();
}

__global__ __launch_bounds__(256) void fieldhash_forms_kernel(uint32_t seed, uint32_t* bad, uint32_t* first_bad) {
    const uint32_t t = blockIdx.x * blockDim.x + threadIdx.x;
    uint32_t x = (t + 1u) * 2654435761u + seed;
    auto rnd = [&]() { x ^= x << 13; x ^= x >> 17; x ^= x << 5; return x; };
    Digest l, r;
#pragma unroll
    for (int i = 0; i < 8; ++i) { l.w[i] = rnd() % P; r.w[i] = rnd() % P; }
    if ((t & 15u) == 1) { l.w[t & 7u] = 0; r.w[(t >> 4) & 7u] = P - 1; }
    if ((t & 15u) == 2) {
#pragma unroll
        for (int i = 0; i < 8; ++i) { l.w[i] = P - 1; r.w[i] = P - 1; }
    }
    if ((t & 15u) == 3) { l.w[0] = 0xFFFFFFFFu; r.w[7] = P; r.w[3] = P + 5; }
    if ((t & 15u) == 4) {
#pragma unroll
        for (int i = 0; i < 8; ++i) { l.w[i] = 0; r.w[i] = 0; }
    }
    uint32_t v = rnd();
    if ((t & 7u) == 0) v = (t & 8u) ? 0xFFFFFFFFu : P - 1;
    if (t == 5) v = 0;
    const Digest a = fieldhash_inner(l, r, g_fh_consts), b = fieldhash_inner64(l, r, g_fh_consts64);
    const Digest c = fieldhash_leaf(v, g_fh_consts), d = fieldhash_leaf64(v, g_fh_consts64);
    bool ok = true;
#pragma unroll
    for (int i = 0; i < 8; ++i) ok = ok && a.w[i] == b.w[i] && c.w[i] == d.w[i] && b.w[i] < P && d.w[i] < P;
    const uint32_t g = threadIdx.x & 15u;
    uint32_t word = 0;
#pragma unroll
    for (int i = 0; i < 8; ++i) {
        const uint32_t lw = __shfl(l.w[i], (int)(threadIdx.x & ~15u) & 63, 64), rw = __shfl(r.w[i], (int)(threadIdx.x & ~15u) & 63, 64);
        if (g == (uint32_t)i) word = lw;
        if (g == (uint32_t)i + 8u) word = rw;
    }
    {
        const uint32_t q4 = threadIdx.x & 3u;
        const int src = (int)(threadIdx.x & ~3u) & 63;
        uint32_t in4[4], out4[4];
#pragma unroll
        for (int j = 0; j < 4; ++j) {
            uint32_t wsel = 0;
#pragma unroll
            for (int i = 0; i < 8; ++i) {
                const uint32_t lw = __shfl(l.w[i], src, 64), rw = __shfl(r.w[i], src, 64);
                if ((int)(4 * q4) + j == i) wsel = lw;
                if ((int)(4 * q4) + j == i + 8) wsel = rw;
            }
            in4[j] = wsel;
        }
        fieldhash_inner_quad_f64(in4, q4, out4, g_fh_consts64);
#pragma unroll
        for (int i = 0; i < 8; ++i) {
            const uint32_t want = __shfl(b.w[i], src, 64);
            if (q4 < 2 && (int)(4 * q4) <= i && i < (int)(4 * q4) + 4 && out4[i - 4 * (int)q4 < 0 ? 0 : (i - 4 * (int)q4) & 3] != want) ok = false;
        }
    }
    const uint32_t row = fieldhash_inner_row16(word, g, g_fh_consts), row64 = fieldhash_inner_row16_f64(word, g, g_fh_consts64);
#pragma unroll
    for (int i = 0; i < 8; ++i) {
        const uint32_t want = __shfl(b.w[i], (int)(threadIdx.x & ~15u) & 63, 64);
        if (g == (uint32_t)i && (row != want || row64 != want)) ok = false;
    }
    {
        const double mags[6] = {236118324143.0 , 3829546563953.0 , 4104397301943.0 , 4398046511103.0 ,
                                (double)P * 1365.0, (double)P * 1024.0};
        const uint32_t k = t % 6u;
        double xd = mags[k] + (double)(int)((rnd() & 0xFFFFu)) - 32768.0 + (k >= 4 ? (double)(rnd() % 3u) - 1.0 : 0.0);
        if (t & 8u) xd = -xd;
        const long long xi = (long long)xd;
        const uint64_t res = (uint64_t)(((xi % (long long)P) + (long long)P) % (long long)P);
        const uint64_t x2 = res * res % P, x4 = x2 * x2 % P, want5 = x4 * res % P;
        if (fh64_canonical(fh64_sbox(xd)) != (uint32_t)want5) ok = false;
        double st[kFhT];
        uint64_t ref[kFhT];
#pragma unroll
        for (int i = 0; i < kFhT; ++i) { st[i] = i ? (double)(l.w[i & 7] >> 1) - (double)(r.w[i & 7] >> 2) : xd; }
#pragma unroll
        for (int i = 0; i < kFhT; ++i) { const long long v = (long long)st[i]; ref[i] = (uint64_t)(((v % (long long)P) + (long long)P) % (long long)P); }
        const double rc = g_fh_consts64.rc_part[t % kFhRP];
        fh64_partial_round<true>(st, rc);
        {
            const uint64_t y = (ref[0] + (uint64_t)rc) % P, y2 = y * y % P, y4 = y2 * y2 % P;
            ref[0] = y4 * y % P;
            uint64_t sum = 0;
#pragma unroll
            for (int i = 0; i < kFhT; ++i) sum = (sum + ref[i]) % P;
            uint64_t outw[kFhT];
            outw[0] = (sum + 2 * (P - ref[0])) % P;
#pragma unroll
            for (int i = 1; i < kFhT; ++i) outw[i] = (((uint64_t)1 << (i - 1)) % P * ref[i] + sum) % P;
#pragma unroll
            for (int i = 0; i < kFhT; ++i)
                if (fh64_canonical(st[i]) != (uint32_t)outw[i]) ok = false;
        }
    }
    if (!ok) { atomicAdd(bad, 1u); atomicMin(first_bad, t); }
// ... 138 lines not shown
```

zkstark_amd/csrc/zkstark.hip:

```cpp
#include <hip/hip_runtime.h>

#include <algorithm>
#include <chrono>
#include <cstdarg>
#include <cstdio>
#include <cstdlib>
#include <cstring>
#include <atomic>
#include <condition_variable>
#include <functional>
#include <mutex>
#include <new>
#include <thread>
#include <string>
#include <vector>

#include "../../include/zkstark_amd.h"
#include "field.hpp"
#include "kernels.hpp"
#include "sha256.hpp"
#include "transcript.hpp"
#include "host_sha.hpp"
#include "internal.hpp"
#include "pool.hpp"

using namespace zk;
using namespace zk::impl;

struct zk_ctx {
    int device = 0;
    uint32_t log_n = 0, log_b = 0, L = 0;
    size_t n = 0, N = 0, B = 0;
    uint32_t R = 0;
    hipStream_t stream = nullptr;
    zk_dom* dom = nullptr;
    uint32_t* d_trace = nullptr;
    uint32_t* d_coef = nullptr;
    uint32_t* d_layers = nullptr;
    std::vector<size_t> layer_off, layer_len;
    uint32_t* d_trees = nullptr;
    std::vector<size_t> tree_off;
    uint64_t* d_gather_off = nullptr;
    uint32_t* d_gather_out = nullptr;
    uint64_t* h_gather_off = nullptr;
    uint32_t* h_gather_out = nullptr;
    uint64_t* dm_gather_off = nullptr;
    uint32_t* dm_gather_out = nullptr;
    const uint32_t* host_nodes[40] = {};
    size_t host_node_cnt[40] = {};
    const uint32_t* host_vals[40] = {};
    std::vector<const uint32_t*> fetch_vals, fetch_nodes;
    std::vector<uint32_t> fetch_vdev;
    std::vector<uint64_t> fetch_ditems;
    std::vector<uint8_t> commit_buf;
    bool pending_top = false;
    uint32_t pending_tree = 0;
    size_t open_nv = 0, open_ndg = 0, open_vi = 0;
    bool open_pending = false;
    uint32_t* h_small = nullptr;
    uint32_t* h_mailbox = nullptr;
    uint32_t* d_mailbox = nullptr;
    uint32_t* d_counter = nullptr;
    bool counters_dirty = false;
    uint32_t mail_seq = 0;
    uint32_t tree_seq[40] = {};
    bool early = false, early_ok = false, gate_pending = false;
    uint32_t* h_gate = nullptr;
    uint32_t* d_gate = nullptr;
    uint32_t* h_dyn = nullptr;
    uint32_t* d_dyn = nullptr;
    uint32_t gate_seq = 0;
    uint32_t host_top = 0, host_tail = 0;
    Pool* pool = nullptr;
    uint32_t* h_stage = nullptr;
    uint32_t* d_stage = nullptr;
    size_t stage_words = 0, stage_used = 0;
    ScatterSeg* h_segs = nullptr;
    ScatterSeg* d_segs = nullptr;
    uint32_t n_segs = 0;
    double seg_words = 0;
    std::vector<uint32_t> tail_vals;
    uint32_t tail_log = 0;
    bool tail_have = false;
    double t_wait = 0, t_host_hash = 0, t_launch = 0;
    bool tail = false;
    uint32_t hinv_host = 0;
    uint32_t queries = 1;
    uint32_t grind = 0;
    Grinder* grinder = nullptr;
    uint32_t fold = 1;
    uint64_t skipped_layers = 0, skipped_trees = 0;
    bool coset = false;
    uint8_t tree_steps[40] = {};
    uint32_t stop = 0;
    uint32_t* d_final = nullptr;
    std::vector<uint32_t> final_poly;
    int hash = 0;
    bool checks = false;
    uint32_t* d_check = nullptr;
    DevTable ones;
    size_t gather_cap = 0;
    size_t device_bytes = 0;
    double setup_ms = 0;
    bool have_trace = false, have_lde = false;
    uint32_t first = 0, last = 0;
    zk_transcript_info info{};
    Profiler prof;
    zk_kernel_stat kstat[K_COUNT] = {};
};

namespace {

template <typename T>
int dmalloc(zk_ctx* c, T** p, size_t bytes) {
    hipError_t e = hipMalloc((void**)p, bytes ? bytes : 4);
    if (e != hipSuccess) return fail(ZK_ERR_NOMEM, "hipMalloc(%zu) failed: %s", bytes, hipGetErrorString(e));
    c->device_bytes += bytes;
    return ZK_OK;
}

size_t layer_size(const zk_ctx* c, uint32_t layer) { return layer == 0 ? c->N : (c->N >> (layer - 1)); }
uint32_t layer_log(const zk_ctx* c, uint32_t layer) { return layer == 0 ? c->L : c->L - (layer - 1); }
uint32_t tree_log(const zk_ctx* c, uint32_t tree) { return layer_log(c, tree) - c->tree_steps[tree]; }
size_t tree_leaves(const zk_ctx* c, uint32_t tree) { return (size_t)1 << tree_log(c, tree); }

Profiler* prof_of(zk_ctx* c) { return c->prof.mask ? &c->prof : nullptr; }

void collect_kernel_stats(zk_ctx* c) {
    for (auto& r : c->prof.recs) {
        float ms = 0;
        (void)hipEventSynchronize(r.b);
        (void)hipEventElapsedTime(&ms, r.a, r.b);
        c->kstat[r.cls].launches += 1;
        c->kstat[r.cls].ms += ms;
        c->kstat[r.cls].bytes += r.bytes;
        c->kstat[r.cls].ops += r.ops;
        c->prof.pool.push_back(r.a);
        c->prof.pool.push_back(r.b);
    }
    c->prof.recs.clear();
}

int do_lde(zk_ctx* c) {
    int rc = dom_lde(c->dom, c->d_trace, c->d_coef, c->d_layers + c->layer_off[0], c->stream, prof_of(c));
    if (!rc) c->have_lde = true;
    return rc;
}

#ifndef ZK_HOST_SUB_LOG
#define ZK_HOST_SUB_LOG 8
#endif
static_assert(ZK_HOST_SUB_LOG >= 4 && ZK_HOST_SUB_LOG <= (int)kMaxHostLog, "host sub-tree size");
constexpr uint32_t host_sub_log() { return ZK_HOST_SUB_LOG; }
uint32_t top_of(const zk_ctx* c, uint32_t tree) {
    if (c->hash != 0 || !c->host_top) return 0;
    const uint32_t lg = tree_log(c, tree);
    return lg > c->host_top ? c->host_top : lg - 1;
}
MailArgs mail_of(zk_ctx* c, uint32_t tree, bool host, bool feed_tail = true, uint32_t steps = 0) {
    MailArgs m;
    c->tree_steps[tree] = (uint8_t)steps;
    if (c->counters_dirty) {
        (void)hipMemsetAsync(c->d_counter, 0, 64, c->stream);
        c->counters_dirty = false;
    }
    m.mailbox = c->d_mailbox;
    m.seq = ++c->mail_seq;
    c->tree_seq[tree] = m.seq;
    m.counter = c->d_counter;
    m.top = host ? top_of(c, tree) : 0;
    if (feed_tail && c->fold == 1 && !c->coset && !c->stop && m.top && c->host_tail && tree >= 1 && layer_log(c, tree) == c->host_tail + 1) {
        m.dump_src = c->d_layers + c->layer_off[tree];
        m.dump_log = c->host_tail + 1;
        m.vals_off = (uint32_t)kMailValsOff;
        c->tail_log = m.dump_log;
        c->tail_have = true;
    }
    return m;
}

int do_merkle(zk_ctx* c, uint32_t layer, bool host = false, bool feed_tail = true, uint32_t steps = 0) {
    HIPCHK(launch_merkle_build_coset(c->d_layers + c->layer_off[layer], layer_log(c, layer), steps, c->d_trees + c->tree_off[layer], c->stream,
                                     prof_of(c), mail_of(c, layer, host, feed_tail, steps), c->hash));
    return ZK_OK;
}

int do_compose_commit(zk_ctx* c, const uint32_t alpha_raw[3]) {
    ComposeArgs a;
    int rc = compose_args(c->dom, c->d_layers + c->layer_off[0], c->d_layers + c->layer_off[1], c->first, c->last, alpha_raw, a);
    if (rc) return rc;
    HIPCHK(launch_compose_merkle(a, c->d_trees + c->tree_off[1], c->stream, prof_of(c), mail_of(c, 1, true), c->hash));
    return ZK_OK;
}
int do_fold_commit(zk_ctx* c, uint32_t round, uint32_t beta_raw) {
    FoldArgs a;
    int rc = fold_args(c->dom, c->d_layers + c->layer_off[1 + round], c->d_layers + c->layer_off[2 + round], c->L - round, round, beta_raw, a);
    if (rc) return rc;
    HIPCHK(launch_fold_merkle(a, c->d_trees + c->tree_off[2 + round], c->stream, prof_of(c), mail_of(c, 2 + round, true), c->hash));
    return ZK_OK;
}

int wait_mail(zk_ctx* c, uint32_t seq) {
    double t0 = now_us();
    int rc = wait_flag(c->h_mailbox, seq, c->stream);
    c->t_wait += now_us() - t0;
    if (rc) c->counters_dirty = true;
    return rc;
}

int read_root(zk_ctx* c, uint32_t tree, uint8_t out[32]) {
    int rc = wait_mail(c, c->tree_seq[tree]);
    if (rc) return rc;
    digest_words_to_bytes(c->h_mailbox + kMailDigests, out);
    return ZK_OK;
}

uint32_t* stage_alloc(zk_ctx* c, size_t words) {
    if (c->stage_used + words > c->stage_words) return nullptr;
    uint32_t* p = c->h_stage + c->stage_used;
    c->stage_used += (words + 7) & ~(size_t)7;
    return p;
}
int stage_seg(zk_ctx* c, const uint32_t* src, size_t dst, size_t words, uint32_t kind) {
    if (c->n_segs >= 4 * 34) return fail(ZK_ERR_STATE, "scatter segment table full");
    c->h_segs[c->n_segs++] = ScatterSeg{(uint64_t)(src - c->h_stage), (uint64_t)dst, (uint32_t)words, kind};
    c->seg_words += (double)words;
    return ZK_OK;
}

int read_commit(zk_ctx* c, uint32_t tree, uint8_t root[32]) {
    const uint32_t H = top_of(c, tree);
    if (!H) return read_root(c, tree, root);
    const size_t cnt = (size_t)1 << H;
    uint32_t* nodes = stage_alloc(c, (2 * cnt - 1) * 8);
    if (!nodes) return fail(ZK_ERR_STATE, "host staging buffer exhausted");
    int rc = wait_mail(c, c->tree_seq[tree]);
    if (rc) return rc;
    double t0 = now_us();
    memcpy(nodes + 8 * (cnt - 1), c->h_mailbox + kMailDigests, cnt * 32);
    const uint32_t sub_log = host_sub_log();
    if (H > sub_log && c->pool) {
        const uint32_t top = H - sub_log;
        c->pool->run((size_t)1 << top, 1, [&](size_t sub) { host_sha_reduce_sub(nodes, H, top, sub); });
        host_sha_reduce(nodes, top);
    } else {
        host_sha_reduce(nodes, H);
    }
    digest_words_to_bytes(nodes, root);
    c->t_host_hash += now_us() - t0;
    if (c->tail_have && c->tail_log == layer_log(c, tree) && tree >= 1) {
        c->tail_vals.assign(c->h_mailbox + kMailValsOff, c->h_mailbox + kMailValsOff + ((size_t)1 << c->tail_log));
    }
    c->host_nodes[tree] = nodes;
    c->host_node_cnt[tree] = 2 * cnt - 1;
    return stage_seg(c, nodes, c->tree_off[tree], (cnt - 1) * 8, 0);
}

int host_fold_commit(zk_ctx* c, uint32_t round, uint32_t beta_raw, uint8_t root[32]) {
    const uint32_t log_out = c->L - round - 1;
    const size_t half = (size_t)1 << log_out;
    const double t_begin = now_us();
    uint32_t* vals = stage_alloc(c, half);
    uint32_t* nodes = stage_alloc(c, (2 * half - 1) * 8);
    if (!vals || !nodes) return fail(ZK_ERR_STATE, "host staging buffer exhausted");
    const zk_dom* d = c->dom;
    const uint32_t cc_m = to_mont(mulmod(beta_raw % P, d->fold_k[round]));
    const uint32_t step_m = to_mont(powmod(c->hinv_host, (uint64_t)1 << round));
    const uint32_t* in = c->tail_vals.data();
    uint32_t xinv_m = to_mont(1);
    for (size_t i = 0; i < half; ++i) {
        uint32_t u = in[i], v = in[i + half];
        vals[i] = add(mont_mul(add(u, v), d->inv2_mont), mont_mul(mont_mul(sub(u, v), xinv_m), cc_m));
        xinv_m = mont_mul(xinv_m, step_m);
    }
    host_sha_leaves(vals, half, nodes + 8 * (half - 1));
    host_sha_reduce(nodes, log_out);
    digest_words_to_bytes(nodes, root);
    c->tail_vals.assign(vals, vals + half);
    c->tail_log = log_out;
    c->t_host_hash += now_us() - t_begin;
    c->tree_steps[2 + round] = 0;
    c->host_vals[2 + round] = vals;
    c->host_nodes[2 + round] = nodes;
    c->host_node_cnt[2 + round] = 2 * half - 1;
    int rc = stage_seg(c, vals, c->layer_off[2 + round], half, 1);
    if (!rc) rc = stage_seg(c, nodes, c->tree_off[2 + round], (2 * half - 1) * 8, 0);
    return rc;
}

int fri_round_commit(zk_ctx* c, uint32_t round, uint32_t beta_raw, uint8_t root[32]) {
    if (c->tail_have && c->tail_log == c->L - round && c->L - round - 1 <= c->host_tail) return host_fold_commit(c, round, beta_raw, root);
    int rc = do_fold_commit(c, round, beta_raw);
    return rc ? rc : read_commit(c, 2 + round, root);
}
bool round_on_host(const zk_ctx* c, uint32_t round) {
    return c->hash == 0 && c->host_top && c->host_tail && c->L >= c->host_tail + 1 && c->L - round <= c->host_tail + 1;
}
bool can_gate(const zk_ctx* c, uint32_t round) { return c->fold == 1 && !c->coset && !c->stop && c->early && c->early_ok && !c->checks && round < c->R && !round_on_host(c, round); }
int enqueue_gated_fold(zk_ctx* c, uint32_t round) {
    FoldArgs a;
    int rc = fold_args(c->dom, c->d_layers + c->layer_off[1 + round], c->d_layers + c->layer_off[2 + round], c->L - round, round, 0u, a);
    if (rc) return rc;
    ++c->gate_seq;
    a.dyn = c->d_dyn + 16 * (c->gate_seq & 1u);
    HIPCHK(hipStreamWaitValue32(c->stream, c->d_gate, c->gate_seq, hipStreamWaitValueEq, 0xFFFFFFFFu));
    c->gate_pending = true;
    HIPCHK(launch_fold_merkle(a, c->d_trees + c->tree_off[2 + round], c->stream, prof_of(c), mail_of(c, 2 + round, true), c->hash));
    return ZK_OK;
}
void release_gate(zk_ctx* c, uint32_t c_mont) {
    c->h_dyn[16 * (c->gate_seq & 1u)] = c_mont;
    __atomic_store_n(c->h_gate, c->gate_seq, __ATOMIC_RELEASE);
    c->gate_pending = false;
}
void release_gated_fold(zk_ctx* c, uint32_t round, uint32_t beta_raw) {
    release_gate(c, to_mont(mulmod(beta_raw % P, c->dom->fold_k[round])));
}
struct GateGuard {
    zk_ctx* c;
    ~GateGuard() { if (c->gate_pending) release_gate(c, 0u); }
};

void begin_proof(zk_ctx* c) {
    c->stage_used = 0; c->n_segs = 0; c->seg_words = 0; c->tail_log = 0; c->tail_have = false;
    c->t_wait = c->t_host_hash = c->t_launch = 0;
    memset(c->host_nodes, 0, sizeof c->host_nodes);
    memset(c->host_node_cnt, 0, sizeof c->host_node_cnt);
    memset(c->host_vals, 0, sizeof c->host_vals);
}
int flush_host_parts(zk_ctx* c) {
    HIPCHK(launch_scatter(c->d_stage, c->d_segs, c->n_segs, c->seg_words, c->d_trees, c->d_layers, c->stream, prof_of(c)));
    c->n_segs = 0;
    c->pending_top = false;
    return ZK_OK;
}
int settle_pending(zk_ctx* c) { return c->pending_top ? flush_host_parts(c) : (int)ZK_OK; }
int last_layer_value(zk_ctx* c, uint32_t* out) {
    const uint32_t* v;
    if (c->tail_have && c->tail_log == c->log_b) v = c->tail_vals.data();
    else {
        HIPCHK(hipMemcpyAsync(c->h_small, c->d_layers + c->layer_off[1 + c->R], c->B * 4, hipMemcpyDeviceToHost, c->stream));
        HIPCHK(hipStreamSynchronize(c->stream));
        v = c->h_small;
    }
    for (size_t i = 1; i < c->B; ++i)
        if (v[i] != v[0]) return fail(ZK_ERR_CHECK, "last FRI layer is not constant (prover.rs:238): trace does not satisfy the constraints");
    *out = v[0];
    return ZK_OK;
}

int final_alloc(zk_ctx* c) {
    return c->d_final ? (int)ZK_OK : dmalloc(c, &c->d_final, (((size_t)1 << kFinalPolyMaxLog) + 1) * 4);
}
int final_poly_value(zk_ctx* c) {
    const uint32_t Rp = c->R - c->stop;
    const size_t cnt = (size_t)1 << c->stop;
    int rc = final_alloc(c);
    if (rc) return rc;
    if ((rc = dom_final_poly(c->dom, c->d_layers + c->layer_off[1 + Rp], c->d_final, c->L - Rp, Rp, (uint32_t)cnt, c->stream, prof_of(c)))) return rc;
    HIPCHK(hipMemcpyAsync(c->h_small, c->d_final, (cnt + 1) * 4, hipMemcpyDeviceToHost, c->stream));
    HIPCHK(hipStreamSynchronize(c->stream));
    if (c->h_small[0])
        return fail(ZK_ERR_CHECK, "final FRI layer has degree >= 2^%u: trace does not satisfy the constraints (%u non-zero coefficients above; cf. prover.rs:238)", c->stop, c->h_small[0]);
    c->final_poly.assign(c->h_small + 1, c->h_small + 1 + cnt);
    return ZK_OK;
}

int do_compose(zk_ctx* c, const uint32_t alpha_raw[3]) {
    return dom_compose(c->dom, c->d_layers + c->layer_off[0], c->d_layers + c->layer_off[1], c->first, c->last,
                       alpha_raw, c->stream, prof_of(c));
}

int do_fold(zk_ctx* c, uint32_t round, uint32_t beta_raw) {
    return dom_fold(c->dom, c->d_layers + c->layer_off[1 + round], c->d_layers + c->layer_off[2 + round],
                    c->L - round, round, beta_raw, c->stream, prof_of(c));
}


int checks_alloc(zk_ctx* c) {
    if (c->d_check) return ZK_OK;
    int rc = dmalloc(c, &c->d_check, (c->N + 2) * 4);
    if (rc) return rc;
    return build_table(1, c->log_n, &c->ones);
}
int check_interpolant(zk_ctx* c) {
    const zk_dom* d = c->dom;
    CoefPrepArgs pa{};
    pa.log_n = d->log_n; pa.log_b = d->log_b;
    pa.tw = d->H.view(); pa.wtab = c->ones.view(); pa.ninv_mont = d->ninv_mont;
    pa.nd = d->plan.nd;
    for (uint32_t t = 0; t < d->plan.nd; ++t) pa.dig_bits[t] = d->plan.bits[t];
    HIPCHK(launch_coef_prepare(c->d_coef, c->d_check, pa, c->stream));
    int rc = run_dit(c->d_check, d->log_n, d->plan, d->H.view(), d->L, c->stream);
    if (rc) return rc;
    std::vector<uint32_t> got(c->n), want(c->n);
    HIPCHK(hipMemcpyAsync(got.data(), c->d_check, c->n * 4, hipMemcpyDeviceToHost, c->stream));
    HIPCHK(hipMemcpyAsync(want.data(), c->d_trace, c->n * 4, hipMemcpyDeviceToHost, c->stream));
    HIPCHK(hipStreamSynchronize(c->stream));
    for (size_t i = 0; i + 1 < c->n; ++i)
        if (got[i] != want[i])
            return fail(ZK_ERR_CHECK, "self-check prover.rs:64-66 failed: f(g^%zu) = %u, trace value %u", i, got[i], want[i]);
    return ZK_OK;
}
int check_degree(zk_ctx* c, uint32_t layer, uint32_t want_deg, const char* cite) {
    const uint32_t lg = layer_log(c, layer);
    const size_t m = (size_t)1 << lg;
    const uint32_t* src = c->d_layers + c->layer_off[layer];
    if (lg <= 10) {
        std::vector<uint32_t> v(m);
        if (c->tail_have && c->tail_log == lg && layer >= 2) v.assign(c->tail_vals.begin(), c->tail_vals.begin() + m);
        else {
            HIPCHK(hipMemcpyAsync(v.data(), src, m * 4, hipMemcpyDeviceToHost, c->stream));
            HIPCHK(hipStreamSynchronize(c->stream));
        }
        const uint32_t winv = invmod(root_of_unity(lg));
        for (size_t k = m; k-- > want_deg; ) {
            uint32_t acc = 0, step = powmod(winv, k), x = 1;
            for (size_t i = 0; i < m; ++i) { acc = add(acc, mulmod(v[i], x)); x = mulmod(x, step); }
            if (k > want_deg && acc != 0)
                return fail(ZK_ERR_CHECK, "self-check %s failed: layer %u has a non-zero coefficient of degree %zu > %u", cite, layer, k, want_deg);
            if (k == want_deg && acc == 0)
                return fail(ZK_ERR_CHECK, "self-check %s failed: layer %u has degree below %u", cite, layer, want_deg);
        }
        return ZK_OK;
    }
    const Plan pl = make_plan(lg);
    int rc = run_dif(src, c->d_check, lg, pl, c->dom->Hinv.view(), c->dom->L, 0, c->stream);
    if (rc) return rc;
    uint32_t* res = c->d_check + c->N;
    HIPCHK(hipMemsetAsync(res, 0, 8, c->stream));
    HIPCHK(launch_degree_check(c->d_check, lg, pl.nd, pl.bits, want_deg + 1, res, c->stream));
    uint32_t h[2];
    HIPCHK(hipMemcpyAsync(h, res, 8, hipMemcpyDeviceToHost, c->stream));
    HIPCHK(hipStreamSynchronize(c->stream));
    if (h[0]) return fail(ZK_ERR_CHECK, "self-check %s failed: layer %u has %u non-zero coefficients of degree > %u (a division left a remainder)", cite, layer, h[0], want_deg);
    if (!h[1]) return fail(ZK_ERR_CHECK, "self-check %s failed: layer %u has degree below %u", cite, layer, want_deg);
    return ZK_OK;
}

void open_begin(zk_ctx* c, size_t nvals) {
    c->fetch_vals.assign(nvals, nullptr); c->fetch_vdev.assign(nvals, 0); c->fetch_nodes.clear(); c->fetch_ditems.clear();
    c->open_nv = c->open_ndg = c->open_vi = 0;
}
void open_val(zk_ctx* c, uint32_t layer, size_t x) {
    if (c->host_vals[layer]) c->fetch_vals[c->open_vi++] = c->host_vals[layer] + x;
    else { c->fetch_vdev[c->open_vi++] = (uint32_t)c->open_nv; c->h_gather_off[c->open_nv++] = (uint64_t)c->layer_off[layer] + x; }
}
void open_path(zk_ctx* c, uint32_t tree, size_t m, size_t leaf) {
    for (size_t i = leaf + m - 1; i != 0; i = (i - 1) >> 1) {
        const size_t nd = (i & 1) ? i + 1 : i - 1;
        if (nd < c->host_node_cnt[tree]) c->fetch_nodes.push_back(c->host_nodes[tree] + 8 * nd);
        else { c->fetch_nodes.push_back(c->h_gather_out + 8 * c->open_ndg); ++c->open_ndg; c->fetch_ditems.push_back((uint64_t)c->tree_off[tree] + (uint64_t)nd * 8); }
    }
}
int open_launch(zk_ctx* c) {
    const size_t nv = c->open_nv, ndg = c->open_ndg;
    if (nv + ndg > c->gather_cap) return fail(ZK_ERR_STATE, "gather capacity exceeded");
    if (ndg) memcpy(c->h_gather_off + nv, c->fetch_ditems.data(), ndg * 8);
    for (size_t i = 0; i < c->fetch_vals.size(); ++i)
        if (!c->fetch_vals[i]) c->fetch_vals[i] = c->h_gather_out + 8 * ndg + c->fetch_vdev[i];
    c->open_pending = nv + ndg != 0;
    if (c->open_pending)
        HIPCHK(launch_fetch(c->d_layers, c->d_trees, c->dm_gather_off, (uint32_t)nv, (uint32_t)ndg, c->dm_gather_out, c->d_mailbox,
                            ++c->mail_seq, c->d_counter, c->stream, prof_of(c)));
    return ZK_OK;
}
int open_wait(zk_ctx* c) {
    if (!c->open_pending) return ZK_OK;
    c->open_pending = false;
    return wait_mail(c, c->mail_seq);
}

int prove_fold_rounds(zk_ctx* c, Channel& ch) {
    const uint32_t R = c->R - c->stop, K = c->fold;
    uint8_t root[32];
    int rc;
    for (uint32_t r0 = 0; r0 < R; r0 += K) {
        const uint32_t steps = R - r0 < K ? R - r0 : K, id = 1 + r0 + steps;
        const uint32_t beta = c->info.beta_raw[r0] = ch.get_u32();
        if ((rc = dom_fold_multi(c->dom, c->d_layers + c->layer_off[1 + r0], c->d_layers + c->layer_off[id], c->L - r0, r0, steps, beta,
                                 c->stream, prof_of(c)))) return rc;
        const uint32_t leaf_steps = c->coset && r0 + steps < R ? (R - r0 - steps < K ? R - r0 - steps : K) : 0;
        const bool stopped = c->stop && r0 + steps == R;
        if (!stopped && ((rc = do_merkle(c, id, true, false, leaf_steps)) || (rc = read_commit(c, id, root)))) return rc;
        const size_t deg = c->n >> (r0 + steps);
        if (c->checks && (rc = check_degree(c, id, (uint32_t)deg - (deg ? 1 : 0), "prover.rs:228-251 (FRI layer degree)"))) return rc;
        if (!stopped) {
            ch.commit_hash(root);
            memcpy(c->info.roots[id], root, 32);
        }
        for (uint32_t l = 2 + r0; l < id; ++l) { c->skipped_layers |= (uint64_t)1 << l; c->skipped_trees |= (uint64_t)1 << l; }
    }
    if (c->stop) {
        c->skipped_trees |= (uint64_t)1 << (1 + R);
        for (uint32_t l = 2 + R; l <= c->R + 1; ++l) { c->skipped_layers |= (uint64_t)1 << l; c->skipped_trees |= (uint64_t)1 << l; }
    }
    return ZK_OK;
}

struct HostLaps {
    const bool on;
    std::chrono::steady_clock::time_point t0 = std::chrono::steady_clock::now();
    void operator()(const char* what) {
        if (!on) return;
        auto t = std::chrono::steady_clock::now();
        fprintf(stderr, "[zk timing] %-28s %8.1f us\n", what, std::chrono::duration<double, std::micro>(t - t0).count());
        t0 = t;
    }
};

int prove_finish(zk_ctx* c, Channel& ch, HostLaps& lap) {
    const uint32_t R = c->R - c->stop, K = c->fold, Q = c->queries, G = fold_groups(R, K);
    const size_t B = c->B, N = c->N, Lp = c->L;
    int rc;
    if (c->stop) {
        if ((rc = final_poly_value(c))) return rc;
        c->info.free_term = c->final_poly[0];
        std::vector<uint8_t>& cb = c->commit_buf;
        cb.resize(4 * c->final_poly.size());
        for (size_t k = 0; k < c->final_poly.size(); ++k)
            for (int i = 0; i < 4; ++i) cb[4 * k + i] = (uint8_t)(c->final_poly[k] >> (8 * i));
        ch.commit_bytes(cb.data(), cb.size());
    } else {
        uint32_t free_term = 0;
        if ((rc = last_layer_value(c, &free_term))) return rc;
        c->info.free_term = free_term;
        ch.commit_u32(free_term);
        c->final_poly.assign(1, free_term);
    }
    if (c->grind) {
        uint64_t w = 0;
        if ((rc = grind_channel(c->grinder, ch, c->grind, &w))) return rc;
        c->info.grind_bits = c->grind;
        c->info.grind_nonce = w;
        lap("grind");
    }
    uint32_t qraws[64];
    for (uint32_t k = 0; k < Q; ++k) qraws[k] = ch.get_u32();
    c->info.query_raw = qraws[0];

    size_t per_query = 0;
    const bool coset = c->coset;
    for_each_opening(c->log_n, c->log_b, K, 0, [&](uint32_t, uint32_t, size_t, uint32_t slots_log) { per_query += (size_t)1 << slots_log; }, coset, c->stop);
    open_begin(c, (size_t)Q * per_query);
    for (uint32_t k = 0; k < Q; ++k)
        for_each_opening(c->log_n, c->log_b, K, (size_t)qraws[k] % (N - 2 * B), [&](uint32_t layer, uint32_t log_leaves, size_t leaf, uint32_t slots_log) {
            for (size_t u = 0; u < ((size_t)1 << slots_log); ++u) open_val(c, layer, leaf + (u << log_leaves));
            open_path(c, layer, (size_t)1 << log_leaves, leaf);
        }, coset, c->stop);
    if ((rc = open_launch(c))) return rc;
    if ((rc = flush_host_parts(c))) return rc;
    lap("free term + fetch enqueue");
    if ((rc = open_wait(c))) return rc;
    lap("fetch wait");
    const uint32_t* const* vsrc = c->fetch_vals.data();
    const uint32_t* const* dsrc = c->fetch_nodes.data();
    std::vector<uint8_t>& buf = c->commit_buf;
    buf.resize(Channel::group_bytes((size_t)1 << fold_steps(R, K, 0), Lp));
    auto tuple = [&](size_t s, size_t plen, bool one_leaf) {
        ch.commit_group(buf.data(), s, plen, [&](size_t t) { return *vsrc[t]; },
                        [&](size_t i, uint8_t* out) { digest_words_to_bytes(dsrc[i], out); }, one_leaf);
        vsrc += s; dsrc += (one_leaf ? 1 : s) * plen;
    };
    for (uint32_t q = 0; q < Q; ++q) {
        for (int k = 0; k < (coset ? 3 : 4); ++k) tuple(1, Lp, false);
        for (uint32_t j = 0; j < G; ++j) {
            const size_t steps = fold_steps(R, K, j);
            tuple((size_t)1 << steps, Lp - (size_t)j * K - (coset ? steps : 0), coset);
        }
    }
    lap("decommit host hashing");
    return ZK_OK;
}

int prove_resident(zk_ctx* c, Channel& ch) {
    if (!c->have_trace) return fail(ZK_ERR_STATE, "zk_prove_resident: no trace uploaded");
    static const bool timing = getenv("ZK_HOST_TIMING") != nullptr;
    HostLaps lap{timing};
    const uint32_t R = c->R;
    ch.data.reserve(ch.data.size() + proof_data_len(c->log_n, c->log_b, c->queries, c->grind, c->fold, c->coset, c->stop));
    c->skipped_layers = c->skipped_trees = 0;
    uint8_t root[32];
    int rc;
    memset(&c->info, 0, sizeof c->info);
    c->info.public_last = c->last;
    c->pending_top = false;
    begin_proof(c);
    GateGuard gate_guard{c};
    if ((rc = do_lde(c))) return rc;
    if (c->checks && ((rc = checks_alloc(c)) || (rc = check_interpolant(c)))) return rc;
    if ((rc = do_merkle(c, 0, true))) return rc;
    if ((rc = read_commit(c, 0, root))) return rc;
    ch.commit_hash(root);
    memcpy(c->info.roots[0], root, 32);
    uint32_t alpha[3];
    for (int i = 0; i < 3; ++i) alpha[i] = c->info.alpha_raw[i] = ch.get_u32();
    if (c->coset) {
        if ((rc = do_compose(c, alpha)) || (rc = do_merkle(c, 1, true, false, fold_steps(R - c->stop, c->fold, 0)))) return rc;
    } else if ((rc = do_compose_commit(c, alpha))) return rc;
    if (can_gate(c, 0) && (rc = enqueue_gated_fold(c, 0))) return rc;
    if ((rc = read_commit(c, 1, root))) return rc;
    if (c->checks && (rc = check_degree(c, 1, (uint32_t)c->n - 1, "prover.rs:148-159/:169 (exact divisions, deg cp = n - 1)"))) return rc;
    ch.commit_hash(root);
    memcpy(c->info.roots[1], root, 32);
    if (c->fold > 1 || c->coset || c->stop) {
        if ((rc = prove_fold_rounds(c, ch))) return rc;
    } else for (uint32_t r = 0; r < R; ++r) {
        uint32_t beta = c->info.beta_raw[r] = ch.get_u32();
        if (c->gate_pending) {
            release_gated_fold(c, r, beta);
            if (can_gate(c, r + 1) && (rc = enqueue_gated_fold(c, r + 1))) return rc;
            if ((rc = read_commit(c, 2 + r, root))) return rc;
        } else if (c->tail_have && c->tail_log == c->L - r && c->L - r - 1 <= c->host_tail) {
            if ((rc = host_fold_commit(c, r, beta, root))) return rc;
        } else {
            if ((rc = do_fold_commit(c, r, beta))) return rc;
            if (can_gate(c, r + 1) && (rc = enqueue_gated_fold(c, r + 1))) return rc;
            if ((rc = read_commit(c, 2 + r, root))) return rc;
        }
        if (c->checks && (rc = check_degree(c, 2 + r, (uint32_t)(c->n >> (r + 1)) - ((c->n >> (r + 1)) ? 1 : 0), "prover.rs:228-251 (FRI layer degree)"))) return rc;
        ch.commit_hash(root);
        memcpy(c->info.roots[2 + r], root, 32);
    }
    lap("lde .. last root");
    if (timing) fprintf(stderr, "[zk timing]   of which: waiting for the device %.1f us, host hashing (tops + tail) %.1f us\n", c->t_wait, c->t_host_hash);
    return prove_finish(c, ch, lap);
}

}

namespace zk {
namespace impl {
int tail_open_begin(zk_ctx* c, size_t x) {
    if (!c || !c->tail) return fail(ZK_ERR_INVALID, "tail_open_begin: not a tail context");
    HIPCHK(hipSetDevice(c->device));
    open_begin(c, 2 * (size_t)c->R);
    for (uint32_t i = 0; i < c->R; ++i) {
        const size_t len = c->N >> i, xi = x % len, nx = (xi + len / 2) % len;
        open_val(c, 1 + i, xi); open_path(c, 1 + i, len, xi);
        open_val(c, 1 + i, nx); open_path(c, 1 + i, len, nx);
    }
    return open_launch(c);
}
int tail_open_end(zk_ctx* c, uint32_t* vals_out, uint8_t* paths_out) {
    int rc = open_wait(c);
    if (rc) return rc;
    for (size_t i = 0; i < c->fetch_vals.size(); ++i) vals_out[i] = *c->fetch_vals[i];
    for (size_t i = 0; i < c->fetch_nodes.size(); ++i) digest_words_to_bytes(c->fetch_nodes[i], paths_out + 32 * i);
    return ZK_OK;
}
int merkle_nodes_to_host(int device, hipStream_t s, const uint32_t* d_heap, size_t first, size_t count, uint8_t* out) {
    if (!count) return ZK_OK;
    HIPCHK(hipSetDevice(device));
    HIPCHK(hipMemcpyAsync(out, d_heap + first * 8, count * 32, hipMemcpyDeviceToHost, s));
    HIPCHK(hipStreamSynchronize(s));
    for (size_t i = 0; i < count; ++i) {
        uint32_t w[8];
        memcpy(w, out + 32 * i, 32);
        digest_words_to_bytes(w, out + 32 * i);
    }
    return ZK_OK;
}
}
}

extern "C" {

const char* zk_last_error(void) { return last_error(); }
int zk_host_hash_mode(void) { return host_sha_wide_available() ? 2 : host_sha_available() ? 1 : 0; }
int zk_host_set_hash_mode(int mode) {
    if (mode < 0 || mode > 2) return fail(ZK_ERR_INVALID, "zk_host_set_hash_mode: mode %d out of range (0 portable, 1 SHA extensions, 2 + AVX-512)", mode);
    host_sha_use_extensions(mode >= 1);
    host_sha_use_wide(mode >= 2);
    return ZK_OK;
}

uint32_t zk_field_add(uint32_t a, uint32_t b) { return add(a % P, b % P); }
uint32_t zk_field_sub(uint32_t a, uint32_t b) { return sub(a % P, b % P); }
uint32_t zk_field_mul(uint32_t a, uint32_t b) { return mulmod(a % P, b % P); }
uint32_t zk_field_neg(uint32_t a) { return neg(a % P); }
uint32_t zk_field_inv(uint32_t a) { return invmod(a % P); }
uint32_t zk_field_pow(uint32_t a, uint32_t e) { return powmod(a, e); }
uint32_t zk_field_from_u32(uint32_t v) { return v % P; }
uint32_t zk_field_from_i32(int32_t v) {
    if (v < 0) return neg(uint32_t(-int64_t(v)) % P);
    return uint32_t(v) % P;
}
uint32_t zk_field_div(uint32_t a, uint32_t b) {
    if (b % P == 0) { fail(ZK_ERR_INVALID, "zk_field_div: division by zero (field.rs:165-177 panics)"); return 0; }
    return mulmod(a % P, invmod(b % P));
}
uint32_t zk_field_rem(uint32_t a, uint32_t rhs) {
    if (rhs == 0) { fail(ZK_ERR_INVALID, "zk_field_rem: remainder by zero (field.rs:89-94 panics)"); return 0; }
    return (a % P) % rhs;
}
uint32_t zk_field_generator(void) {
    static const uint32_t g = [] {
        uint32_t factors[32], nf = 0, p = P - 1;
        for (uint32_t it = 2; p != 1; ++it) {
            if (p % it == 0) factors[nf++] = it;
            while (p % it == 0) p /= it;
        }
        for (uint32_t x = 2; x < P; ++x) {
            bool primitive = true;
            for (uint32_t i = 0; i < nf && primitive; ++i) primitive = powmod(x, (P - 1) / factors[i]) != 1;
            if (primitive) return x;
        }
        return 0u;
    }();
    return g;
}
uint32_t zk_field_order(uint32_t a) {
    a %= P;
    if (a == 0) return 0;
    uint32_t ord = P - 1;
    if (powmod(a, ord / 3) == 1) ord /= 3;
    while (ord % 2 == 0 && powmod(a, ord / 2) == 1) ord /= 2;
    return ord;
}
uint32_t zk_field_root_of_unity(uint32_t log_order) { return log_order > 30 ? 0 : root_of_unity(log_order); }

static int ctx_make(int device, uint32_t log_n, uint32_t log_b, uint32_t shift, bool tail, zk_ctx** out);
static int ctx_team(zk_ctx* c) {
    const uint32_t sub_log = host_sub_log();
    const unsigned want = c->host_top > sub_log ? (1u << (c->host_top - sub_log)) - 1u : 0u;
    if (c->pool && c->pool->workers() == want) return ZK_OK;
    delete c->pool;
    c->pool = nullptr;
    if (!want) return ZK_OK;
    const double spin_us = 5000.0;
    c->pool = new (std::nothrow) Pool(want, spin_us);
    return c->pool ? (int)ZK_OK : fail(ZK_ERR_NOMEM, "out of host memory");
}

int zk_ctx_create(int device, uint32_t log_n, uint32_t log_b, zk_ctx** out) {
    if (!out) return fail(ZK_ERR_INVALID, "zk_ctx_create: out is null");
    *out = nullptr;
    if (int rc = check_proof_size("zk_ctx_create", log_n, log_b)) return rc;
    return ctx_make(device, log_n, log_b, GEN_W, false, out);
}

static int ctx_make(int device, uint32_t log_n, uint32_t log_b, uint32_t shift, bool tail, zk_ctx** out) {
    auto t0 = std::chrono::steady_clock::now();
    HIPCHK(hipSetDevice(device));
    zk_ctx* c = new (std::nothrow) zk_ctx();
    if (!c) return fail(ZK_ERR_NOMEM, "out of host memory");
    c->device = device;
    c->log_n = log_n; c->log_b = log_b; c->L = log_n + log_b;
    c->n = (size_t)1 << log_n; c->B = (size_t)1 << log_b; c->N = c->n << log_b;
    c->R = log_n;
    int rc = ZK_OK;
    auto bail = [&](int code) { zk_ctx_destroy(c); return code; };
#define HIPCHK_C(expr)                                                                        \
    do {                                                                                      \
        hipError_t _e = (expr);                                                               \
        if (_e != hipSuccess) {                                                               \
            zk_ctx_destroy(c);                                                                \
            return fail(ZK_ERR_HIP, "%s failed: %s (%s:%d)", #expr, hipGetErrorString(_e), __FILE__, __LINE__); \
        }                                                                                     \
    } while (0)
    HIPCHK_C(hipStreamCreateWithFlags(&c->stream, hipStreamNonBlocking));
    if ((rc = dom_make(device, log_n, log_b, shift, tail, c->stream, &c->dom))) return bail(rc);
    c->tail = tail;
    c->hinv_host = invmod(c->dom->h);
    c->device_bytes += c->dom->device_bytes;
    size_t off = 0;
    for (uint32_t l = 0; l <= c->R + 1; ++l) {
        c->layer_off.push_back(off);
        c->layer_len.push_back(layer_size(c, l));
        off += layer_size(c, l);
    }
    size_t layer_words = off;
    off = 0;
    for (uint32_t l = 0; l <= c->R + 1; ++l) {
        c->tree_off.push_back(off);
        off += (2 * layer_size(c, l) - 1) * 8;
    }
    size_t tree_words = off;
    if ((rc = dmalloc(c, &c->d_trace, c->n * 4))) return bail(rc);
    if ((rc = dmalloc(c, &c->d_coef, 2 * c->n * 4))) return bail(rc);
    if ((rc = dmalloc(c, &c->d_layers, layer_words * 4))) return bail(rc);
    if ((rc = dmalloc(c, &c->d_trees, tree_words * 4))) return bail(rc);
    c->gather_cap = (size_t)kMaxQueries * (4 + 2 * c->R) * (c->L + 1) + 64;
    if ((rc = dmalloc(c, &c->d_gather_off, c->gather_cap * 8))) return bail(rc);
    if ((rc = dmalloc(c, &c->d_gather_out, c->gather_cap * 32))) return bail(rc);
    HIPCHK_C(hipHostMalloc((void**)&c->h_gather_off, c->gather_cap * 8, hipHostMallocMapped | hipHostMallocCoherent));
    HIPCHK_C(hipHostMalloc((void**)&c->h_gather_out, c->gather_cap * 32, hipHostMallocMapped | hipHostMallocCoherent));
    HIPCHK_C(hipHostGetDevicePointer((void**)&c->dm_gather_off, c->h_gather_off, 0));
    HIPCHK_C(hipHostGetDevicePointer((void**)&c->dm_gather_out, c->h_gather_out, 0));
    HIPCHK_C(hipHostMalloc((void**)&c->h_small, 4096));
    const size_t mail_bytes = kMailWords * 4;
    if ((rc = dmalloc(c, &c->d_counter, 64))) return bail(rc);
    HIPCHK_C(hipMemsetAsync(c->d_counter, 0, 64, c->stream));
    HIPCHK_C(hipHostMalloc((void**)&c->h_mailbox, mail_bytes, hipHostMallocMapped | hipHostMallocCoherent));
    memset(c->h_mailbox, 0, mail_bytes);
    HIPCHK_C(hipHostGetDevicePointer((void**)&c->d_mailbox, c->h_mailbox, 0));
    HIPCHK_C(hipHostMalloc((void**)&c->h_gate, 64, hipHostMallocMapped | hipHostMallocCoherent));
    HIPCHK_C(hipHostMalloc((void**)&c->h_dyn, 2 * 16 * 4, hipHostMallocMapped | hipHostMallocCoherent));
    memset(c->h_gate, 0, 64);
    memset(c->h_dyn, 0, 2 * 16 * 4);
    HIPCHK_C(hipHostGetDevicePointer((void**)&c->d_gate, c->h_gate, 0));
    HIPCHK_C(hipHostGetDevicePointer((void**)&c->d_dyn, c->h_dyn, 0));
    {
        int can = 0;
        if (hipDeviceGetAttribute(&can, hipDeviceAttributeCanUseStreamWaitValue, device) != hipSuccess) { can = 0; (void)hipGetLastError(); }
        c->early_ok = can != 0 && !tail;
    }
    c->stage_words = (size_t)(c->R + 2) * ((size_t)16 << kMaxHostLog) + ((size_t)64 << kMaxHostLog);
    const size_t seg_bytes = 4 * 34 * sizeof(ScatterSeg);
    HIPCHK_C(hipHostMalloc((void**)&c->h_stage, c->stage_words * 4 + seg_bytes, hipHostMallocMapped | hipHostMallocCoherent));
    HIPCHK_C(hipHostGetDevicePointer((void**)&c->d_stage, c->h_stage, 0));
    c->h_segs = reinterpret_cast<ScatterSeg*>(c->h_stage + c->stage_words);
    c->d_segs = reinterpret_cast<ScatterSeg*>(c->d_stage + c->stage_words);
    if (host_sha_available()) {
        c->host_top = 8;
        c->host_tail = 9;
    }
    if (int prc = ctx_team(c)) { zk_ctx_destroy(c); return prc; }
#undef HIPCHK_C
    c->setup_ms = std::chrono::duration<double, std::milli>(std::chrono::steady_clock::now() - t0).count();
    *out = c;
    return ZK_OK;
}

#ifdef ZK_WG_TRACE
extern "C++" { namespace zk { void dump_wg_trace(); } }
#endif

int zk_ctx_destroy(zk_ctx* c) {
    if (!c) return ZK_OK;
    (void)hipSetDevice(c->device);
    if (c->stream) (void)hipStreamSynchronize(c->stream);
#ifdef ZK_WG_TRACE
    zk::dump_wg_trace();
#endif
    dom_free(c->dom);
    if (c->d_trace) (void)hipFree(c->d_trace);
    if (c->d_coef) (void)hipFree(c->d_coef);
    if (c->d_layers) (void)hipFree(c->d_layers);
    if (c->d_trees) (void)hipFree(c->d_trees);
    if (c->d_counter) (void)hipFree(c->d_counter);
    if (c->d_check) (void)hipFree(c->d_check);
    if (c->d_final) (void)hipFree(c->d_final);
    free_table(&c->ones);
    if (c->d_gather_off) (void)hipFree(c->d_gather_off);
    if (c->d_gather_out) (void)hipFree(c->d_gather_out);
    if (c->h_gather_off) (void)hipHostFree(c->h_gather_off);
    if (c->h_gather_out) (void)hipHostFree(c->h_gather_out);
    if (c->h_small) (void)hipHostFree(c->h_small);
    if (c->h_mailbox) (void)hipHostFree(c->h_mailbox);
    if (c->h_gate) (void)hipHostFree(c->h_gate);
    if (c->h_dyn) (void)hipHostFree(c->h_dyn);
    if (c->h_stage) (void)hipHostFree(c->h_stage);
    grinder_destroy(c->grinder);
    collect_kernel_stats(c);
    delete c->pool;
    for (hipEvent_t e : c->prof.pool) (void)hipEventDestroy(e);
    if (c->stream) (void)hipStreamDestroy(c->stream);
    delete c;
    return ZK_OK;
}

double zk_ctx_setup_ms(const zk_ctx* c) { return c ? c->setup_ms : 0.0; }
size_t zk_ctx_device_bytes(const zk_ctx* c) { return c ? c->device_bytes : 0; }
void* zk_ctx_stream(zk_ctx* c) {
    if (!c) return nullptr;
    if (c->pending_top && hipSetDevice(c->device) == hipSuccess) (void)settle_pending(c);
    return (void*)c->stream;
}
int zk_ctx_sync(zk_ctx* c) {
    if (!c) return fail(ZK_ERR_INVALID, "null context");
    HIPCHK(hipSetDevice(c->device));
    if (int rc = settle_pending(c)) return rc;
    HIPCHK(hipStreamSynchronize(c->stream));
    return ZK_OK;
}
int zk_ctx_set_early_launch(zk_ctx* c, int on) {
    if (!c) return fail(ZK_ERR_INVALID, "null context");
    c->early = on != 0;
    return ZK_OK;
}
int zk_ctx_get_early_launch(const zk_ctx* c) { return c && c->early && c->early_ok && c->fold == 1 && !c->coset && !c->stop ? 1 : 0; }
int zk_ctx_set_fold(zk_ctx* c, uint32_t fold_log) {
    if (!c) return fail(ZK_ERR_INVALID, "null context");
    if (c->tail) return fail(ZK_ERR_STATE, "zk_ctx_set_fold: FRI-tail context");
    if (fold_log < 1 || fold_log > kMaxFoldLog) return fail(ZK_ERR_INVALID, "zk_ctx_set_fold: need 1 <= fold_log <= %u (got %u)", kMaxFoldLog, fold_log);
    size_t opened = 4;
    for (uint32_t r0 = 0; r0 < c->R; r0 += fold_log) opened += (size_t)1 << (c->R - r0 < fold_log ? c->R - r0 : fold_log);
    const size_t cap = (size_t)kMaxQueries * opened * (c->L + 1) + 64;
    if (cap > c->gather_cap) {
        HIPCHK(hipSetDevice(c->device));
        HIPCHK(hipStreamSynchronize(c->stream));
        uint64_t *d_off = nullptr, *h_off = nullptr, *dm_off = nullptr;
        uint32_t *d_out = nullptr, *h_out = nullptr, *dm_out = nullptr;
        hipError_t e = hipMalloc((void**)&d_off, cap * 8);
        if (e == hipSuccess) e = hipMalloc((void**)&d_out, cap * 32);
        if (e == hipSuccess) e = hipHostMalloc((void**)&h_off, cap * 8, hipHostMallocMapped | hipHostMallocCoherent);
        if (e == hipSuccess) e = hipHostMalloc((void**)&h_out, cap * 32, hipHostMallocMapped | hipHostMallocCoherent);
        if (e == hipSuccess) e = hipHostGetDevicePointer((void**)&dm_off, h_off, 0);
        if (e == hipSuccess) e = hipHostGetDevicePointer((void**)&dm_out, h_out, 0);
        if (e != hipSuccess) {
            if (d_off) (void)hipFree(d_off);
            if (d_out) (void)hipFree(d_out);
            if (h_off) (void)hipHostFree(h_off);
            if (h_out) (void)hipHostFree(h_out);
            return fail(ZK_ERR_NOMEM, "zk_ctx_set_fold: decommitment buffers: %s", hipGetErrorString(e));
        }
        (void)hipFree(c->d_gather_off); (void)hipFree(c->d_gather_out);
        (void)hipHostFree(c->h_gather_off); (void)hipHostFree(c->h_gather_out);
        c->d_gather_off = d_off; c->d_gather_out = d_out; c->h_gather_off = h_off; c->h_gather_out = h_out;
        c->dm_gather_off = dm_off; c->dm_gather_out = dm_out;
        c->device_bytes += (cap - c->gather_cap) * 40;
        c->gather_cap = cap;
    }
    c->fold = fold_log;
    return ZK_OK;
}
uint32_t zk_ctx_get_fold(const zk_ctx* c) { return c ? c->fold : 0; }
int zk_ctx_set_coset_leaves(zk_ctx* c, int on) {
    if (!c) return fail(ZK_ERR_INVALID, "null context");
    if (c->tail) return fail(ZK_ERR_STATE, "zk_ctx_set_coset_leaves: FRI-tail context");
    c->coset = on != 0;
    return ZK_OK;
}
int zk_ctx_get_coset_leaves(const zk_ctx* c) { return c && c->coset ? 1 : 0; }
int zk_ctx_set_fri_stop(zk_ctx* c, uint32_t stop_log) {
    if (!c) return fail(ZK_ERR_INVALID, "null context");
    if (c->tail) return fail(ZK_ERR_STATE, "zk_ctx_set_fri_stop: FRI-tail context");
    if (!stop_ok(c->log_n, c->log_b, stop_log))
        return fail(ZK_ERR_INVALID, "zk_ctx_set_fri_stop: need stop_log <= %u, stop_log <= log_n - 1 = %u and stop_log + log_blowup <= %u (got %u)",
                    kMaxStopLog, c->log_n - 1, kMaxStopLayerLog, stop_log);
    if (stop_log) {
        HIPCHK(hipSetDevice(c->device));
        if (int rc = final_alloc(c)) return rc;
    }
    c->stop = stop_log;
    return ZK_OK;
}
uint32_t zk_ctx_get_fri_stop(const zk_ctx* c) { return c ? c->stop : 0; }
int zk_ctx_final_poly(const zk_ctx* c, uint32_t* out, size_t cap, size_t* count) {
    if (!c || !count || (!out && cap)) return fail(ZK_ERR_INVALID, "zk_ctx_final_poly: null argument");
    if (c->final_poly.empty()) return fail(ZK_ERR_STATE, "zk_ctx_final_poly: no proof made yet");
    *count = c->final_poly.size();
    if (c->final_poly.size() > cap) return fail(ZK_ERR_BUFFER, "zk_ctx_final_poly: %zu coefficients, room for %zu", c->final_poly.size(), cap);
    memcpy(out, c->final_poly.data(), c->final_poly.size() * 4);
    return ZK_OK;
}
int zk_ctx_set_queries(zk_ctx* c, uint32_t n_queries) {
    if (!c) return fail(ZK_ERR_INVALID, "null context");
    if (n_queries < 1 || n_queries > kMaxQueries) return fail(ZK_ERR_INVALID, "zk_ctx_set_queries: need 1 <= n_queries <= %u", kMaxQueries);
    c->queries = n_queries;
    return ZK_OK;
}
int zk_ctx_set_grinding(zk_ctx* c, uint32_t grind_bits) {
    if (!c) return fail(ZK_ERR_INVALID, "null context");
    if (c->tail) return fail(ZK_ERR_STATE, "zk_ctx_set_grinding: FRI-tail context");
    if (grind_bits > kMaxGrindBits) return fail(ZK_ERR_INVALID, "zk_ctx_set_grinding: need grind_bits <= %u (got %u)", kMaxGrindBits, grind_bits);
    if (grind_bits > kGrindHostMaxBits && !c->grinder) {
        HIPCHK(hipSetDevice(c->device));
        if (int rc = grinder_create(c->device, c->stream, 1, &c->grinder)) return rc;
    }
    c->grind = grind_bits;
    return ZK_OK;
}

int zk_ctx_set_host_levels(zk_ctx* c, uint32_t top_log, uint32_t tail_log) {
    if (!c) return fail(ZK_ERR_INVALID, "null context");
    if (top_log > kMaxHostLog || tail_log > kMaxHostLog || (tail_log && !top_log))
        return fail(ZK_ERR_INVALID, "zk_ctx_set_host_levels: need top_log, tail_log <= %u, and top_log > 0 when tail_log > 0", kMaxHostLog);
    c->host_top = top_log;
    c->host_tail = tail_log;
    return ctx_team(c);
}
int zk_ctx_get_host_levels(const zk_ctx* c, uint32_t* top_log, uint32_t* tail_log) {
    if (!c || !top_log || !tail_log) return fail(ZK_ERR_INVALID, "zk_ctx_get_host_levels: null argument");
    *top_log = c->host_top;
    *tail_log = c->host_tail;
    return ZK_OK;
}
int zk_ctx_set_checks(zk_ctx* c, int on) {
    if (!c) return fail(ZK_ERR_INVALID, "null context");
    if (c->tail) return fail(ZK_ERR_STATE, "zk_ctx_set_checks: FRI-tail context");
    c->checks = on != 0;
    return ZK_OK;
}
static const char kNoBlake2s[] = "BLAKE2s (hash 2) is not built for this entry point yet";
int zk_ctx_set_hash(zk_ctx* c, int hash_kind) {
    if (!c) return fail(ZK_ERR_INVALID, "null context");
    if (hash_kind != ZK_HASH_SHA256 && hash_kind != ZK_HASH_FIELD && hash_kind != ZK_HASH_BLAKE2S)
        return fail(ZK_ERR_INVALID, "zk_ctx_set_hash: unknown hash %d", hash_kind);
    if (hash_kind == ZK_HASH_BLAKE2S && c->tail) return fail(ZK_ERR_INVALID, "zk_ctx_set_hash: %s", kNoBlake2s);
    c->hash = hash_kind;
    return ZK_OK;
}

int zk_ctx_set_profiling(zk_ctx* c, uint32_t class_mask) {
    if (!c) return fail(ZK_ERR_INVALID, "null context");
    c->prof.mask = class_mask & ((1u << K_COUNT) - 1u);
    return ZK_OK;
}

static int put_kernel_stats(zk_kernel_stat* out, size_t count, const zk_kernel_stat* src, const char* who) {
    if (!count) return ZK_OK;
    const uint32_t stride = out[0].struct_size;
    if (!abi_bytes(out, who)) return ZK_ERR_INVALID;
    for (size_t i = 0; i < count && i < (size_t)K_COUNT; ++i) {
        zk_kernel_stat* o = reinterpret_cast<zk_kernel_stat*>(reinterpret_cast<char*>(out) + i * stride);
        o->struct_size = stride;
        if (int rc = abi_put(o, src[i], who)) return rc;
    }
    return ZK_OK;
}

int zk_kernel_stats(zk_ctx* c, zk_kernel_stat* out, size_t count, int reset) {
    if (!c || (!out && count)) return fail(ZK_ERR_INVALID, "zk_kernel_stats: null argument");
    collect_kernel_stats(c);
    if (int rc = put_kernel_stats(out, count, c->kstat, "zk_kernel_stats")) return rc;
    if (reset) for (int i = 0; i < K_COUNT; ++i) c->kstat[i] = zk_kernel_stat{};
    return ZK_OK;
}

int zk_trace_fibsq(uint32_t a0, uint32_t a1, size_t count, uint32_t* out) {
    if (!out && count) return fail(ZK_ERR_INVALID, "zk_trace_fibsq: out is null");
    if (count > 0) out[0] = a0 % P;
    if (count > 1) out[1] = a1 % P;
    for (size_t i = 2; i < count; ++i)
        out[i] = add(mulmod(out[i - 2], out[i - 2]), mulmod(out[i - 1], out[i - 1]));
    return ZK_OK;
}

int zk_trace_upload(zk_ctx* c, const uint32_t* trace, size_t count) {
    if (!c || !trace) return fail(ZK_ERR_INVALID, "zk_trace_upload: null argument");
    if (count != c->n - 1) return fail(ZK_ERR_INVALID, "zk_trace_upload: expected n-1 = %zu values, got %zu", c->n - 1, count);
    for (size_t i = 0; i < count; ++i)
        if (trace[i] >= P) return fail(ZK_ERR_INVALID, "zk_trace_upload: trace[%zu] = %u is not a canonical residue", i, trace[i]);
    HIPCHK(hipSetDevice(c->device));
    HIPCHK(hipMemcpyAsync(c->d_trace, trace, count * 4, hipMemcpyHostToDevice, c->stream));
    HIPCHK(hipMemsetAsync(c->d_trace + count, 0, 4, c->stream));
    HIPCHK(hipStreamSynchronize(c->stream));
    c->first = trace[0];
    c->last = trace[count - 1];
    c->have_trace = true;
    c->have_lde = false;
    return ZK_OK;
}

int zk_lde(zk_ctx* c) {
    if (!c) return fail(ZK_ERR_INVALID, "null context");
    if (!c->have_trace) return fail(ZK_ERR_STATE, "zk_lde: no trace uploaded");
    HIPCHK(hipSetDevice(c->device));
    static const bool timing = getenv("ZK_HOST_TIMING") != nullptr;
    const double t0 = now_us();
    int rc = do_lde(c);
    if (timing) fprintf(stderr, "[zk timing] lde: enqueue of %u passes %.1f us\n", 2 * c->dom->plan.nd, now_us() - t0);
    return rc;
}

int zk_merkle_commit(zk_ctx* c, uint32_t layer, uint8_t root_out[32]) { return zk_merkle_commit_coset(c, layer, 0, root_out); }
int zk_merkle_commit_coset(zk_ctx* c, uint32_t layer, uint32_t steps, uint8_t root_out[32]) {
    if (!c || !root_out) return fail(ZK_ERR_INVALID, "zk_merkle_commit: null argument");
    if (layer > c->R + 1) return fail(ZK_ERR_INVALID, "zk_merkle_commit: layer %u out of range", layer);
    if (steps > kMaxFoldLog || (steps && layer_log(c, layer) <= steps))
        return fail(ZK_ERR_INVALID, "zk_merkle_commit_coset: need steps <= %u and at least two leaves (layer %u has 2^%u values, steps %u)", kMaxFoldLog, layer, layer_log(c, layer), steps);
    HIPCHK(hipSetDevice(c->device));
    static const bool timing = getenv("ZK_HOST_TIMING") != nullptr;
    const double t0 = now_us();
    c->skipped_trees &= ~((uint64_t)1 << layer);
    if (c->pending_top && c->pending_tree == layer) c->pending_top = false;
    int rc = settle_pending(c);
    if (rc) return rc;
    begin_proof(c);
    rc = do_merkle(c, layer, true, false, steps);
    const double t1 = now_us();
    if (!rc) rc = read_commit(c, layer, root_out);
    const double t2 = now_us();
    if (!rc && c->n_segs) { c->pending_top = true; c->pending_tree = layer; }
    if (timing)
        fprintf(stderr, "[zk timing] merkle_commit(layer %u): enqueue %.1f us, wait for the device %.1f us, host top %.1f us, scatter enqueue %.1f us\n",
                layer, t1 - t0, c->t_wait, c->t_host_hash, now_us() - t2);
    return rc;
}

int zk_compose(zk_ctx* c, const uint32_t alpha_raw[3]) {
    if (!c || !alpha_raw) return fail(ZK_ERR_INVALID, "zk_compose: null argument");
    if (!c->have_lde) return fail(ZK_ERR_STATE, "zk_compose: run zk_lde first");
    HIPCHK(hipSetDevice(c->device));
    return do_compose(c, alpha_raw);
}

int zk_fri_fold(zk_ctx* c, uint32_t round, uint32_t beta_raw) {
    if (!c) return fail(ZK_ERR_INVALID, "null context");
    if (round >= c->R) return fail(ZK_ERR_INVALID, "zk_fri_fold: round %u out of range (%u rounds)", round, c->R);
    HIPCHK(hipSetDevice(c->device));
    c->skipped_layers &= ~((uint64_t)1 << (2 + round));
    return do_fold(c, round, beta_raw);
}
int zk_fri_fold_multi(zk_ctx* c, uint32_t round, uint32_t steps, uint32_t beta_raw) {
    if (!c) return fail(ZK_ERR_INVALID, "null context");
    if (steps < 1 || steps > kMaxFoldLog) return fail(ZK_ERR_INVALID, "zk_fri_fold_multi: steps must be 1..%u (got %u)", kMaxFoldLog, steps);
    if (round >= c->R || round + steps > c->R) return fail(ZK_ERR_INVALID, "zk_fri_fold_multi: rounds %u..%u out of range (%u rounds)", round, round + steps, c->R);
    HIPCHK(hipSetDevice(c->device));
    c->skipped_layers &= ~((uint64_t)1 << (1 + round + steps));
    return dom_fold_multi(c->dom, c->d_layers + c->layer_off[1 + round], c->d_layers + c->layer_off[1 + round + steps], c->L - round, round, steps,
                          beta_raw, c->stream, prof_of(c));
}

int zk_fri_final_poly(zk_ctx* c, uint32_t layer, uint32_t bound, uint32_t* coef_out, uint32_t* high_nonzero) {
    if (!c || !coef_out || !high_nonzero) return fail(ZK_ERR_INVALID, "zk_fri_final_poly: null argument");
    if (layer < 1 || layer > c->R + 1) return fail(ZK_ERR_INVALID, "zk_fri_final_poly: layer %u out of range (FRI layers are 1..%u)", layer, c->R + 1);
    const uint32_t lg = layer_log(c, layer);
    if (lg > kFinalPolyMaxLog) return fail(ZK_ERR_INVALID, "zk_fri_final_poly: layer %u has 2^%u values, the limit is 2^%u", layer, lg, kFinalPolyMaxLog);
    if ((c->skipped_layers >> layer) & 1) return fail(ZK_ERR_STATE, "zk_fri_final_poly: layer %u was not materialised by the last proof", layer);
    HIPCHK(hipSetDevice(c->device));
    int rc = settle_pending(c);
    if (!rc) rc = final_alloc(c);
    if (!rc) rc = dom_final_poly(c->dom, c->d_layers + c->layer_off[layer], c->d_final, lg, layer - 1, bound, c->stream, prof_of(c));
    if (rc) return rc;
    HIPCHK(hipMemcpyAsync(high_nonzero, c->d_final, 4, hipMemcpyDeviceToHost, c->stream));
    HIPCHK(hipMemcpyAsync(coef_out, c->d_final + 1, ((size_t)4) << lg, hipMemcpyDeviceToHost, c->stream));
    HIPCHK(hipStreamSynchronize(c->stream));
    return ZK_OK;
}

int zk_layer_read(zk_ctx* c, uint32_t layer, size_t offset, size_t count, uint32_t* out) {
    if (!c || (!out && count)) return fail(ZK_ERR_INVALID, "zk_layer_read: null argument");
    if (layer > c->R + 1 || offset + count > layer_size(c, layer)) return fail(ZK_ERR_INVALID, "zk_layer_read: out of range");
    if ((c->skipped_layers >> layer) & 1) return fail(ZK_ERR_STATE, "zk_layer_read: layer %u was not materialised by the last proof (fold_log %u, fri_stop %u)", layer, c->fold, c->stop);
    HIPCHK(hipSetDevice(c->device));
    if (int prc = settle_pending(c)) return prc;
    HIPCHK(hipMemcpyAsync(out, c->d_layers + c->layer_off[layer] + offset, count * 4, hipMemcpyDeviceToHost, c->stream));
    HIPCHK(hipStreamSynchronize(c->stream));
    return ZK_OK;
}

int zk_layer_write(zk_ctx* c, uint32_t layer, size_t offset, size_t count, const uint32_t* in) {
    if (!c || (!in && count)) return fail(ZK_ERR_INVALID, "zk_layer_write: null argument");
    if (layer > c->R + 1 || offset + count > layer_size(c, layer)) return fail(ZK_ERR_INVALID, "zk_layer_write: out of range");
    for (size_t i = 0; i < count; ++i)
        if (in[i] >= P) return fail(ZK_ERR_INVALID, "zk_layer_write: value %zu is not a canonical residue", i);
    HIPCHK(hipSetDevice(c->device));
    HIPCHK(hipMemcpyAsync(c->d_layers + c->layer_off[layer] + offset, in, count * 4, hipMemcpyHostToDevice, c->stream));
    HIPCHK(hipStreamSynchronize(c->stream));
    if (layer == 0) c->have_lde = true;
    c->skipped_layers &= ~((uint64_t)1 << layer);
    return ZK_OK;
}

int zk_merkle_node(zk_ctx* c, uint32_t tree, size_t index, uint8_t out[32]) {
    if (!c || !out) return fail(ZK_ERR_INVALID, "zk_merkle_node: null argument");
    if (tree > c->R + 1 || index >= 2 * tree_leaves(c, tree) - 1) return fail(ZK_ERR_INVALID, "zk_merkle_node: out of range");
    if ((c->skipped_trees >> tree) & 1) return fail(ZK_ERR_STATE, "zk_merkle_node: tree %u was not built by the last proof (fold_log %u, fri_stop %u)", tree, c->fold, c->stop);
    HIPCHK(hipSetDevice(c->device));
    if (int prc = settle_pending(c)) return prc;
    HIPCHK(hipMemcpyAsync(c->h_small, c->d_trees + c->tree_off[tree] + index * 8, 32, hipMemcpyDeviceToHost, c->stream));
    HIPCHK(hipStreamSynchronize(c->stream));
    digest_words_to_bytes(c->h_small, out);
    return ZK_OK;
}

int zk_merkle_nodes(zk_ctx* c, uint32_t tree, size_t first, size_t count, uint8_t* out) {
    if (!c || (!out && count)) return fail(ZK_ERR_INVALID, "zk_merkle_nodes: null argument");
    if (tree > c->R + 1 || first > 2 * tree_leaves(c, tree) - 1 || count > 2 * tree_leaves(c, tree) - 1 - first)
        return fail(ZK_ERR_INVALID, "zk_merkle_nodes: out of range");
    if ((c->skipped_trees >> tree) & 1) return fail(ZK_ERR_STATE, "zk_merkle_nodes: tree %u was not built by the last proof (fold_log %u, fri_stop %u)", tree, c->fold, c->stop);
    HIPCHK(hipSetDevice(c->device));
    if (int prc = settle_pending(c)) return prc;
    return merkle_nodes_to_host(c->device, c->stream, c->d_trees + c->tree_off[tree], first, count, out);
}

int zk_merkle_path(zk_ctx* c, uint32_t tree, size_t leaf, uint8_t* out, size_t* path_len) {
    if (!c || !out) return fail(ZK_ERR_INVALID, "zk_merkle_path: null argument");
    if (tree > c->R + 1 || leaf >= tree_leaves(c, tree)) return fail(ZK_ERR_INVALID, "zk_merkle_path: out of range");
    if ((c->skipped_trees >> tree) & 1) return fail(ZK_ERR_STATE, "zk_merkle_path: tree %u was not built by the last proof (fold_log %u, fri_stop %u)", tree, c->fold, c->stop);
    HIPCHK(hipSetDevice(c->device));
    if (int prc = settle_pending(c)) return prc;
    std::vector<size_t> nodes;
    path_nodes(tree_leaves(c, tree), leaf, nodes);
    for (size_t i = 0; i < nodes.size(); ++i) c->h_gather_off[i] = (uint64_t)c->tree_off[tree] + (uint64_t)nodes[i] * 8;
    HIPCHK(hipMemcpyAsync(c->d_gather_off, c->h_gather_off, nodes.size() * 8, hipMemcpyHostToDevice, c->stream));
    HIPCHK(launch_gather(c->d_trees, c->d_gather_off, (uint32_t)nodes.size(), 8, c->d_gather_out, c->stream));
    HIPCHK(hipMemcpyAsync(c->h_gather_out, c->d_gather_out, nodes.size() * 32, hipMemcpyDeviceToHost, c->stream));
    HIPCHK(hipStreamSynchronize(c->stream));
    for (size_t i = 0; i < nodes.size(); ++i) digest_words_to_bytes(c->h_gather_out + 8 * i, out + 32 * i);
    if (path_len) *path_len = nodes.size();
    return ZK_OK;
}

int zk_prove_resident(zk_ctx* c, uint8_t* proof_out, size_t cap, size_t* proof_len, uint8_t state_out[32]) {
    if (!c || !proof_out || !state_out) return fail(ZK_ERR_INVALID, "zk_prove_resident: null argument");
    HIPCHK(hipSetDevice(c->device));
    Channel ch;
    int rc = prove_resident(c, ch);
    if (rc) return rc;
    const std::vector<uint8_t>& proof = ch.data;
    if (proof_len) *proof_len = proof.size();
    if (proof.size() > cap) return fail(ZK_ERR_BUFFER, "zk_prove: proof needs %zu bytes, buffer has %zu", proof.size(), cap);
    memcpy(proof_out, proof.data(), proof.size());
    memcpy(state_out, ch.state, 32);
    return ZK_OK;
}

int zk_prove_channel(zk_ctx* c, zk_channel* chan) {
    if (!c || !chan) return fail(ZK_ERR_INVALID, "zk_prove_channel: null argument");
    if (c->tail) return fail(ZK_ERR_STATE, "zk_prove_channel: FRI-tail context");
    HIPCHK(hipSetDevice(c->device));
    return prove_resident(c, chan->ch);
}

int zk_prove(zk_ctx* c, const uint32_t* trace, size_t count, uint8_t* proof_out, size_t cap, size_t* proof_len,
             uint8_t state_out[32]) {
    int rc = zk_trace_upload(c, trace, count);
    if (rc) return rc;
    return zk_prove_resident(c, proof_out, cap, proof_len, state_out);
}

int zk_prove_many(zk_ctx* const* ctxs, size_t count, uint8_t* proofs_out, size_t stride, size_t* lens_out, uint8_t* states_out) {
    if (!ctxs || !proofs_out || !lens_out || !states_out || count == 0 || count > 16)
        return fail(ZK_ERR_INVALID, "zk_prove_many: need 1..16 contexts and non-null outputs");
    for (size_t i = 0; i < count; ++i) {
        if (!ctxs[i]) return fail(ZK_ERR_INVALID, "zk_prove_many: context %zu is null", i);
        for (size_t j = 0; j < i; ++j)
            if (ctxs[j] == ctxs[i]) return fail(ZK_ERR_INVALID, "zk_prove_many: context %zu appears twice", i);
    }
    std::vector<int> rcs(count, ZK_OK);
    std::vector<std::string> errs(count);
    auto one = [&](size_t i) {
        rcs[i] = zk_prove_resident(ctxs[i], proofs_out + i * stride, stride, &lens_out[i], states_out + 32 * i);
        if (rcs[i]) errs[i] = last_error();
    };
    std::vector<std::thread> th;
    for (size_t i = 1; i < count; ++i) th.emplace_back(one, i);
    one(0);
    for (auto& t : th) t.join();
    for (size_t i = 0; i < count; ++i)
        if (rcs[i]) return fail(rcs[i], "zk_prove_many: context %zu: %s", i, errs[i].c_str());
    return ZK_OK;
}

int zk_last_transcript(const zk_ctx* c, zk_transcript_info* out) {
    if (!c || !out) return fail(ZK_ERR_INVALID, "zk_last_transcript: null argument");
    return abi_put(out, c->info, "zk_last_transcript");
}

static int verify_entry(const char* who, const uint8_t* proof, size_t len, const uint8_t* state, uint32_t log_n, uint32_t log_b,
                        uint32_t public_last, int hash_kind, uint32_t q, uint32_t grind, uint32_t fold, int32_t* check_out,
                        const char* replay_note, const char* reject_note, bool coset = false, uint32_t stop = 0) {
    if (hash_kind != ZK_HASH_SHA256 && hash_kind != ZK_HASH_FIELD && hash_kind != ZK_HASH_BLAKE2S) return fail(ZK_ERR_INVALID, "%s: unknown hash %d", who, hash_kind);
    if (fold < 1 || fold > kMaxFoldLog) return fail(ZK_ERR_INVALID, "%s: need 1 <= fold_log <= %u (got %u)", who, kMaxFoldLog, fold);
    int rc = state ? verify_transcript(proof, len, state, log_n, log_b, q, grind, fold, coset, stop) : 0;
    const bool in_replay = rc != 0;
    if (!rc) rc = verify_proof(proof, len, log_n, log_b, public_last, hash_kind, q, grind, fold, coset, stop);
    if (check_out) *check_out = rc;
    if (!rc) return ZK_OK;
    if (in_replay && replay_note) return fail(ZK_ERR_VERIFY, "transcript replay failed at check %d%s", rc, replay_note);
    return fail(ZK_ERR_VERIFY, "proof rejected at check %d%s", rc, reject_note);
}
static const char kProofRs[] = " (proof.rs:15-149)";

int zk_verify_ex(const uint8_t* proof, size_t len, uint32_t log_n, uint32_t log_b, uint32_t public_last, int hash_kind) {
    if (!proof) return fail(ZK_ERR_INVALID, "zk_verify: null proof");
    return verify_entry("zk_verify", proof, len, nullptr, log_n, log_b, public_last, hash_kind, 1, 0, 1, nullptr, nullptr, kProofRs);
}
int zk_verify(const uint8_t* proof, size_t len, uint32_t log_n, uint32_t log_b, uint32_t public_last) {
    return zk_verify_ex(proof, len, log_n, log_b, public_last, ZK_HASH_SHA256);
}
int zk_verify_queries(const uint8_t* proof, size_t len, const uint8_t* state, uint32_t log_n, uint32_t log_b, uint32_t public_last,
                      int hash_kind, uint32_t n_queries) {
    if (!proof) return fail(ZK_ERR_INVALID, "zk_verify_queries: null proof");
    return verify_entry("zk_verify_queries", proof, len, state, log_n, log_b, public_last, hash_kind, n_queries, 0, 1, nullptr, "", kProofRs);
}
int zk_verify_strict(const uint8_t* proof, size_t len, const uint8_t state[32], uint32_t log_n, uint32_t log_b, uint32_t public_last) {
    if (!proof || !state) return fail(ZK_ERR_INVALID, "zk_verify_strict: null argument");
// ... 624 lines not shown
```

Before: 2.913 billion.

## Vectorise host FRI tail fold, add paired AVX-512 SHA, memoise WG plans

Moves the host-side FRI tail fold into an AVX-512 eight-lane Montgomery routine with precomputed per-round inverse-root steps. It adds a 32-lane SHA-256 path that interleaves two 16-lane streams, enabled on AMD CPUs, for leaves and inner nodes. Other changes: Merkle top reduction hashes straight from the mailbox, fusing the digest copy with the first level; tail values are held by pointer instead of copied into a vector; the tail cap rises to 11 levels; the workgroup-split plan search is memoised per shape. It also adds challenge-to-launch timing. The main risks are register pressure in the paired SHA kernel and larger staging buffers.

```diff
diff --git a/zkstark_amd/build.py b/zkstark_amd/build.py
--- a/zkstark_amd/build.py
+++ b/zkstark_amd/build.py
@@ -10,8 +10,8 @@
 OBJDIR = os.path.join(HERE, "build")
 LIB = os.path.join(HERE, "libzkstark_amd.so")
 HASHFILE = LIB + ".hash"
-SOURCES = ["kernels.hip", "ntt_fast.hip", "domain.hip", "zkstark.hip", "batch.hip", "shard.hip", "verify.hip", "grind.hip", "host_sha.cpp", "version.cpp"]
-HEADERS = ["field.hpp", "sha256.hpp", "blake2s.hpp", "sha256_quad.hpp", "fieldhash.hpp", "fieldhash_f64.hpp", "kernels.hpp", "transcript.hpp", "host_sha.hpp", "internal.hpp", "pool.hpp",
+SOURCES = ["kernels.hip", "ntt_fast.hip", "domain.hip", "zkstark.hip", "batch.hip", "shard.hip", "verify.hip", "grind.hip", "host_sha.cpp", "host_fold.cpp", "version.cpp"]
+HEADERS = ["field.hpp", "sha256.hpp", "blake2s.hpp", "sha256_quad.hpp", "fieldhash.hpp", "fieldhash_f64.hpp", "kernels.hpp", "transcript.hpp", "host_sha.hpp", "host_fold.hpp", "internal.hpp", "pool.hpp",
            "shard.hpp", "board.hpp", "peer.hpp", os.path.join("..", "..", "include", "zkstark_amd.h")]
 ARCH = "gfx950"
 FLAGS = ["-O3", "-std=c++17", f"--offload-arch={ARCH}", "-fPIC", "-Wall", "-Wno-unused-function"]
diff --git a/zkstark_amd/csrc/domain.hip b/zkstark_amd/csrc/domain.hip
--- a/zkstark_amd/csrc/domain.hip
+++ b/zkstark_amd/csrc/domain.hip
@@ -123,6 +123,8 @@
         const uint32_t inv2 = invmod(2);
         uint32_t wr = shift;
         for (uint32_t r = 0; r < d->L && r < 32; ++r) { d->fold_k[r] = mulmod(invmod(wr), inv2); wr = mulmod(wr, wr); }
+        uint32_t hs = invmod(d->h);
+        for (uint32_t r = 0; r < d->L && r < 32; ++r) { d->hinv_step_mont[r] = to_mont(hs); hs = mulmod(hs, hs); }
         uint32_t xn = powmod(shift, d->n);
         const uint32_t hn = powmod(d->h, d->n);
         for (size_t r = 0; r < d->B; ++r) { const uint32_t den = sub(xn, 1); d->inv_den[r] = den ? invmod(den) : 0u; xn = mulmod(xn, hn); }
diff --git a/zkstark_amd/csrc/host_fold.cpp b/zkstark_amd/csrc/host_fold.cpp
--- /dev/null
+++ b/zkstark_amd/csrc/host_fold.cpp
@@ -0,0 +1,63 @@
+#include "host_fold.hpp"
+
+#if defined(__HIPCC__)
+#include <hip/hip_runtime.h>
+#endif
+#include "field.hpp"
+#include "host_sha.hpp"
+
+#if !defined(__HIP_DEVICE_COMPILE__)
+#include <immintrin.h>
+
+namespace zk {
+namespace {
+
+void fold_scalar(const uint32_t* in, size_t half, size_t first, uint32_t* out, uint32_t c_mont, uint32_t step_mont, uint32_t inv2_mont, uint32_t x) {
+    for (size_t i = first; i < half; ++i) {
+        const uint32_t u = in[i], v = in[i + half];
+        out[i] = add(mont_mul(add(u, v), inv2_mont), mont_mul(mont_mul(sub(u, v), x), c_mont));
+        x = mont_mul(x, step_mont);
+    }
+}
+
+#define ZK_FOLD_TARGET __attribute__((target("avx512f")))
+ZK_FOLD_TARGET inline __m512i add8(__m512i a, __m512i b, __m512i p) {
+    const __m512i s = _mm512_add_epi64(a, b);
+    return _mm512_min_epu64(s, _mm512_sub_epi64(s, p));
+}
+ZK_FOLD_TARGET inline __m512i sub8(__m512i a, __m512i b, __m512i p) {
+    const __m512i d = _mm512_sub_epi64(a, b);
+    return _mm512_min_epu64(d, _mm512_add_epi64(d, p));
+}
+ZK_FOLD_TARGET inline __m512i mont_mul8(__m512i a, __m512i b, __m512i p) {
+    const __m512i t = _mm512_mul_epu32(a, b);
+    const __m512i m = _mm512_add_epi64(t, _mm512_slli_epi64(t, 30));
+    const __m512i hi = _mm512_srli_epi64(t, 32), mp_hi = _mm512_srli_epi64(_mm512_mul_epu32(m, p), 32);
+    const __m512i r = _mm512_sub_epi64(hi, mp_hi);
+    return _mm512_mask_add_epi64(r, _mm512_cmplt_epu64_mask(hi, mp_hi), r, p);
+}
+ZK_FOLD_TARGET void fold_x8(const uint32_t* in, size_t half, uint32_t* out, uint32_t c_mont, uint32_t step_mont, uint32_t inv2_mont) {
+    alignas(64) uint64_t x0[8];
+    uint32_t x = R1;
+    for (int k = 0; k < 8; ++k) { x0[k] = x; x = mont_mul(x, step_mont); }
+    const __m512i p = _mm512_set1_epi64(P), c = _mm512_set1_epi64(c_mont), i2 = _mm512_set1_epi64(inv2_mont), s8 = _mm512_set1_epi64(x);
+    __m512i xv = _mm512_load_si512(x0);
+    for (size_t i = 0; i < half; i += 8) {
+        const __m512i u = _mm512_cvtepu32_epi64(_mm256_loadu_si256((const __m256i*)(in + i)));
+        const __m512i v = _mm512_cvtepu32_epi64(_mm256_loadu_si256((const __m256i*)(in + i + half)));
+        const __m512i even = mont_mul8(add8(u, v, p), i2, p);
+        const __m512i odd = mont_mul8(mont_mul8(sub8(u, v, p), xv, p), c, p);
+        _mm256_storeu_si256((__m256i*)(out + i), _mm512_cvtepi64_epi32(add8(even, odd, p)));
+        xv = mont_mul8(xv, s8, p);
+    }
+}
+
+}
+
+void host_fold_layer(const uint32_t* in, size_t half, uint32_t* out, uint32_t c_mont, uint32_t step_mont, uint32_t inv2_mont) {
+    if (half >= 8 && half % 8 == 0 && host_sha_wide_available()) fold_x8(in, half, out, c_mont, step_mont, inv2_mont);
+    else fold_scalar(in, half, 0, out, c_mont, step_mont, inv2_mont, R1);
+}
+
+}
+#endif
diff --git a/zkstark_amd/csrc/host_fold.hpp b/zkstark_amd/csrc/host_fold.hpp
--- /dev/null
+++ b/zkstark_amd/csrc/host_fold.hpp
@@ -0,0 +1,9 @@
+#pragma once
+#include <stddef.h>
+#include <stdint.h>
+
+namespace zk {
+
+void host_fold_layer(const uint32_t* in, size_t half, uint32_t* out, uint32_t c_mont, uint32_t step_mont, uint32_t inv2_mont);
+
+}
diff --git a/zkstark_amd/csrc/host_sha.cpp b/zkstark_amd/csrc/host_sha.cpp
--- a/zkstark_amd/csrc/host_sha.cpp
+++ b/zkstark_amd/csrc/host_sha.cpp
@@ -25,8 +25,9 @@
 
 alignas(16) uint32_t PADKW[64];
 bool g_cpu_has_sha = false, g_cpu_has_x16 = false;
-std::atomic<bool> g_have_sha{false}, g_have_x16{false};
+std::atomic<bool> g_have_sha{false}, g_have_x16{false}, g_have_x32{false};
 std::atomic<bool> g_want_x16{true};
+std::atomic<bool> g_want_x32{true};
 
 inline uint32_t rotr(uint32_t x, int n) { return (x >> n) | (x << (32 - n)); }
 
@@ -37,6 +38,8 @@
         g_cpu_has_x16 = g_cpu_has_sha && __builtin_cpu_supports("avx512f");
         g_have_sha = g_cpu_has_sha;
         g_have_x16 = g_cpu_has_x16;
+        g_want_x32 = __builtin_cpu_is("amd");
+        g_have_x32 = g_cpu_has_x16 && g_want_x32.load(std::memory_order_relaxed);
         uint32_t w[64] = {0x80000000u};
         w[15] = 512u;
         for (int t = 16; t < 64; ++t) {
@@ -263,10 +266,102 @@
     store_x16(st, out);
 }
 
-void inner_run(const uint32_t* child, uint32_t* out, size_t cnt) {
+#define ZK_INLINE inline __attribute__((always_inline))
+ZK_X16_TARGET ZK_INLINE void round_x16(__m512i v[8], int t, __m512i wk) {
+    const __m512i a = v[(0 - t) & 7], b = v[(1 - t) & 7], c = v[(2 - t) & 7], e = v[(4 - t) & 7], f = v[(5 - t) & 7], g = v[(6 - t) & 7];
+    const __m512i S1 = ZK_XOR3(ZK_ROR(e, 6), ZK_ROR(e, 11), ZK_ROR(e, 25));
+    const __m512i t1 = _mm512_add_epi32(_mm512_add_epi32(v[(7 - t) & 7], S1), _mm512_add_epi32(_mm512_ternarylogic_epi32(e, f, g, 0xCA), wk));
+    const __m512i S0 = ZK_XOR3(ZK_ROR(a, 2), ZK_ROR(a, 13), ZK_ROR(a, 22));
+    const __m512i t2 = _mm512_add_epi32(S0, _mm512_ternarylogic_epi32(a, b, c, 0xE8));
+    v[(3 - t) & 7] = _mm512_add_epi32(v[(3 - t) & 7], t1);
+    v[(7 - t) & 7] = _mm512_add_epi32(t1, t2);
+}
+ZK_X16_TARGET ZK_INLINE __m512i sched_x16(__m512i* w, int k) {
+    const __m512i w15 = _mm512_load_si512(w + ((k + 1) & 15)), w2 = _mm512_load_si512(w + ((k + 14) & 15));
+    const __m512i s0 = ZK_XOR3(ZK_ROR(w15, 7), ZK_ROR(w15, 18), _mm512_srli_epi32(w15, 3));
+    const __m512i s1 = ZK_XOR3(ZK_ROR(w2, 17), ZK_ROR(w2, 19), _mm512_srli_epi32(w2, 10));
+    const __m512i nw = _mm512_add_epi32(_mm512_add_epi32(_mm512_load_si512(w + k), s0), _mm512_add_epi32(_mm512_load_si512(w + ((k + 9) & 15)), s1));
+    _mm512_store_si512(w + k, nw);
+    return nw;
+}
+template <bool MSG, bool SCHED>
+ZK_X16_TARGET ZK_INLINE void rounds16_x32(__m512i va[8], __m512i vb[8], __m512i* w, const uint32_t* kw) {
+#pragma GCC unroll 16
+    for (int k = 0; k < 16; ++k) {
+        const __m512i kk = _mm512_set1_epi32((int)kw[k]);
+        if (MSG) {
+            const __m512i wa = SCHED ? sched_x16(w, k) : _mm512_load_si512(w + k);
+            const __m512i wb = SCHED ? sched_x16(w + 16, k) : _mm512_load_si512(w + 16 + k);
+            round_x16(va, k, _mm512_add_epi32(wa, kk));
+            round_x16(vb, k, _mm512_add_epi32(wb, kk));
+        } else {
+            round_x16(va, k, kk);
+            round_x16(vb, k, kk);
+        }
+    }
+}
+template <bool MSG>
+ZK_X16_TARGET ZK_INLINE void rounds_x32(__m512i sa[8], __m512i sb[8], __m512i* w) {
+    __m512i va[8], vb[8];
+    for (int i = 0; i < 8; ++i) { va[i] = sa[i]; vb[i] = sb[i]; }
+    const uint32_t* kw = MSG ? K : PADKW;
+    if (MSG) asm volatile("" : "+r"(w) : : "memory");
+    rounds16_x32<MSG, false>(va, vb, w, kw);
+#pragma GCC unroll 1
+    for (int i = 1; i < 4; ++i) {
+        if (MSG) asm volatile("" : "+r"(w) : : "memory");
+        rounds16_x32<MSG, true>(va, vb, w, kw + 16 * i);
+    }
+    for (int i = 0; i < 8; ++i) { sa[i] = _mm512_add_epi32(sa[i], va[i]); sb[i] = _mm512_add_epi32(sb[i], vb[i]); }
+}
+ZK_X16_TARGET void inner_x32(const uint32_t* in, uint32_t* out, uint32_t* copy) {
+    alignas(64) __m512i w[32];
+    __m512i sa[8], sb[8];
+    for (int n = 0; n < 32; ++n) {
+        w[n] = _mm512_loadu_si512((const void*)(in + 16 * n));
+        if (copy) _mm512_storeu_si512((void*)(copy + 16 * n), w[n]);
+    }
+    transpose16(w);
+    transpose16(w + 16);
+    for (int i = 0; i < 8; ++i) sa[i] = sb[i] = _mm512_set1_epi32((int)IV[i]);
+    rounds_x32<true>(sa, sb, w);
+    rounds_x32<false>(sa, sb, w);
+    store_x16(sa, out);
+    store_x16(sb, out + 128);
+}
+ZK_X16_TARGET void leaves_x32(const uint32_t* vals, uint32_t* out) {
+    alignas(64) __m512i w[32];
+    __m512i sa[8], sb[8];
+    for (int b = 0; b < 2; ++b) {
+        __m512i* x = w + 16 * b;
+        x[0] = _mm512_loadu_si512((const void*)(vals + 16 * b));
+        x[1] = _mm512_set1_epi32((int)0x80000000u);
+        for (int i = 2; i < 15; ++i) x[i] = _mm512_setzero_si512();
+        x[15] = _mm512_set1_epi32(32);
+    }
+    for (int i = 0; i < 8; ++i) sa[i] = sb[i] = _mm512_set1_epi32((int)IV[i]);
+    rounds_x32<true>(sa, sb, w);
+    store_x16(sa, out);
+    store_x16(sb, out + 128);
+}
+ZK_X16_TARGET void inner_x16_copy(const uint32_t* in, uint32_t* out, uint32_t* copy) {
+    for (int n = 0; n < 16; ++n) _mm512_storeu_si512((void*)(copy + 16 * n), _mm512_loadu_si512((const void*)(in + 16 * n)));
+    inner_x16(copy, out);
+}
+
+void inner_run(const uint32_t* child, uint32_t* out, size_t cnt, uint32_t* copy = nullptr) {
     size_t i = 0;
+    if (g_have_x32)
+        for (; i + 32 <= cnt; i += 32) inner_x32(child + 16 * i, out + 8 * i, copy ? copy + 16 * i : nullptr);
     if (g_have_x16)
-        for (; i + 16 <= cnt; i += 16) inner_x16(child + 16 * i, out + 8 * i);
+        for (; i + 16 <= cnt; i += 16) {
+            if (copy) inner_x16_copy(child + 16 * i, out + 8 * i, copy + 16 * i);
+            else inner_x16(child + 16 * i, out + 8 * i);
+        }
+    if (copy && i < cnt) {
+        memcpy(copy + 16 * i, child + 16 * i, (cnt - i) * 64);
+        child = copy;
+    }
     for (; i + 2 <= cnt; i += 2) inner_ni_x2(child + 16 * i, out + 8 * i);
     for (; i < cnt; ++i) inner_ni(child + 16 * i, child + 16 * i + 8, out + 8 * i);
 }
@@ -309,11 +404,18 @@
 void host_sha_use_extensions(bool on) {
     g_have_sha = on && g_cpu_has_sha;
     g_have_x16 = on && g_cpu_has_x16 && g_want_x16.load(std::memory_order_relaxed);
+    g_have_x32 = g_have_x16.load(std::memory_order_relaxed) && g_want_x32.load(std::memory_order_relaxed);
 }
 bool host_sha_wide_available() { return g_have_x16; }
 void host_sha_use_wide(bool on) {
     g_want_x16 = on;
     g_have_x16 = on && g_have_sha.load(std::memory_order_relaxed) && g_cpu_has_x16;
+    g_have_x32 = g_have_x16.load(std::memory_order_relaxed) && g_want_x32.load(std::memory_order_relaxed);
+}
+bool host_sha_pair_available() { return g_have_x32; }
+void host_sha_use_pair(bool on) {
+    g_want_x32 = on;
+    g_have_x32 = on && g_have_x16.load(std::memory_order_relaxed);
 }
 
 void host_sha_compress(uint32_t state[8], const uint32_t block[16]) {
@@ -342,6 +444,8 @@
 
 void host_sha_leaves(const uint32_t* vals, size_t n, uint32_t* out) {
     size_t i = 0;
+    if (g_have_x32)
+        for (; i + 32 <= n; i += 32) leaves_x32(vals + i, out + 8 * i);
     if (g_have_x16)
         for (; i + 16 <= n; i += 16) leaves_x16(vals + i, out + 8 * i);
     for (; i < n; ++i) host_sha_leaf(vals[i], out + 8 * i);
@@ -374,6 +478,18 @@
     }
 }
 
+void host_sha_reduce_from(const uint32_t* digests, uint32_t* nodes, uint32_t depth) {
+    if (!depth) { memcpy(nodes, digests, 32); return; }
+    uint32_t* const level = nodes + 8 * (((size_t)1 << depth) - 1);
+    const size_t cnt = (size_t)1 << (depth - 1);
+    if (g_have_sha) inner_run(digests, nodes + 8 * (cnt - 1), cnt, level);
+    else {
+        memcpy(level, digests, cnt * 64);
+        for (size_t i = 0; i < cnt; ++i) host_sha_inner(level + 16 * i, level + 16 * i + 8, nodes + 8 * (cnt - 1 + i));
+    }
+    host_sha_reduce(nodes, depth - 1);
+}
+
 void host_sha_reduce(uint32_t* nodes, uint32_t depth) {
     if (g_have_sha) { reduce_ni(nodes, depth); return; }
     for (uint32_t d = depth; d-- > 0;) {
diff --git a/zkstark_amd/csrc/host_sha.hpp b/zkstark_amd/csrc/host_sha.hpp
--- a/zkstark_amd/csrc/host_sha.hpp
+++ b/zkstark_amd/csrc/host_sha.hpp
@@ -8,6 +8,8 @@
 void host_sha_use_extensions(bool on);
 bool host_sha_wide_available();
 void host_sha_use_wide(bool on);
+bool host_sha_pair_available();
+void host_sha_use_pair(bool on);
 void host_sha_compress(uint32_t state[8], const uint32_t block[16]);
 void host_sha_blocks(uint32_t state[8], const uint8_t* data, size_t blocks);
 void host_sha_leaf(uint32_t v, uint32_t out[8]);
@@ -15,6 +17,7 @@
 void host_sha_inner(const uint32_t left[8], const uint32_t right[8], uint32_t out[8]);
 void host_sha_inner_run(const uint32_t* children, uint32_t* out, size_t cnt);
 void host_sha_reduce(uint32_t* nodes, uint32_t depth);
+void host_sha_reduce_from(const uint32_t* digests, uint32_t* nodes, uint32_t depth);
 void host_sha_reduce_sub(uint32_t* nodes, uint32_t depth, uint32_t top, size_t sub);
 
 }
diff --git a/zkstark_amd/csrc/internal.hpp b/zkstark_amd/csrc/internal.hpp
--- a/zkstark_amd/csrc/internal.hpp
+++ b/zkstark_amd/csrc/internal.hpp
@@ -64,8 +64,9 @@
 constexpr uint32_t kMaxQueries = 64;
 constexpr uint32_t kHostTopSingle = 8;
 constexpr uint32_t kMaxHostLog = 10;
+constexpr uint32_t kMaxHostTail = 11;
 constexpr size_t kMailValsOff = kMailDigests + ((size_t)8 << kMaxHostLog);
-constexpr size_t kMailWords = kMailValsOff + ((size_t)2 << kMaxHostLog);
+constexpr size_t kMailWords = kMailValsOff + ((size_t)2 << kMaxHostTail);
 constexpr uint32_t kMaxRadixLog = 8;
 
 inline int check_proof_size(const char* who, uint32_t log_n, uint32_t log_b, uint32_t log_extra = 0) {
@@ -118,6 +119,7 @@
     zk::impl::Plan plan;
     uint32_t shift_mont = 0, gm1_mont = 0, gm2_mont = 0, gm3_mont = 0, ninv_mont = 0, inv2_mont = 0;
     uint32_t fold_k[32] = {0};
+    uint32_t hinv_step_mont[32] = {0};
     uint32_t inv_den[32] = {0};
     size_t device_bytes = 0;
 };
diff --git a/zkstark_amd/csrc/kernels.hip b/zkstark_amd/csrc/kernels.hip
--- a/zkstark_amd/csrc/kernels.hip
+++ b/zkstark_amd/csrc/kernels.hip
@@ -1,5 +1,6 @@
 #include "kernels.hpp"
 
+#include <atomic>
 #include <cstdlib>
 
 #include "blake2s.hpp"
@@ -1424,6 +1425,7 @@
 #define ZK_MERKLE_CONTINUATION 1
 #endif
 static constexpr bool g_merkle_continuation = ZK_MERKLE_CONTINUATION != 0;
+static std::atomic<uint16_t> g_wg_plan[2][3][32][2 * kWgMaxLog + 1];
 constexpr double kContinueUs = 6.0;
 constexpr double kLaunchUs = 10.0;
 
@@ -1501,7 +1503,12 @@
         const uint32_t launches = levels ? (levels + kWgMaxLog - 1) / kWgMaxLog : 1;
         const uint32_t jn = (levels + launches - 1) / launches;
         uint32_t best_j = jn, best_j2 = 0;
-        if (may_continue && levels <= 2 * kWgMaxLog) {
+        std::atomic<uint16_t>* memo = may_continue && levels <= 2 * kWgMaxLog && span < 32 && (unsigned)hash < 3u ? &g_wg_plan[leaf][hash][span][levels] : nullptr;
+        const uint16_t known = memo ? memo->load(std::memory_order_relaxed) : (uint16_t)0;
+        if (known) {
+            best_j = (known >> 5) & 31u;
+            best_j2 = known & 31u;
+        } else if (may_continue && levels <= 2 * kWgMaxLog) {
             double best = wg_phase_us(leaf, jn, jn, hash, 1u << (span - jn));
             if (launches == 2 && span - jn <= kWgMaxLog) best += kLaunchUs + wg_phase_us(false, span - jn, levels - jn, hash, 1);
             else if (launches > 1) best = 0.0;
@@ -1511,6 +1518,7 @@
                 const double us = wg_phase_us(leaf, j, j, hash, 1u << (span - j)) + kContinueUs + wg_phase_us(false, span - j, j2, hash, 1);
                 if (us < best) { best = us; best_j = j; best_j2 = j2; }
             }
+            if (memo) memo->store((uint16_t)(0x8000u | best_j << 5 | best_j2), std::memory_order_relaxed);
         }
         launch_wg(best_j, best_j2);
     } while (depth > end);
diff --git a/zkstark_amd/csrc/zkstark.hip b/zkstark_amd/csrc/zkstark.hip
--- a/zkstark_amd/csrc/zkstark.hip
+++ b/zkstark_amd/csrc/zkstark.hip
@@ -20,6 +20,7 @@
 #include "kernels.hpp"
 #include "sha256.hpp"
 #include "transcript.hpp"
+#include "host_fold.hpp"
 #include "host_sha.hpp"
 #include "internal.hpp"
 #include "pool.hpp"
@@ -79,12 +80,11 @@
     ScatterSeg* d_segs = nullptr;
     uint32_t n_segs = 0;
     double seg_words = 0;
-    std::vector<uint32_t> tail_vals;
+    const uint32_t* tail_vals = nullptr;
     uint32_t tail_log = 0;
     bool tail_have = false;
     double t_wait = 0, t_host_hash = 0, t_launch = 0;
     bool tail = false;
-    uint32_t hinv_host = 0;
     uint32_t queries = 1;
     uint32_t grind = 0;
     Grinder* grinder = nullptr;
@@ -237,19 +237,19 @@
     int rc = wait_mail(c, c->tree_seq[tree]);
     if (rc) return rc;
     double t0 = now_us();
-    memcpy(nodes + 8 * (cnt - 1), c->h_mailbox + kMailDigests, cnt * 32);
     const uint32_t sub_log = host_sub_log();
     if (H > sub_log && c->pool) {
+        memcpy(nodes + 8 * (cnt - 1), c->h_mailbox + kMailDigests, cnt * 32);
         const uint32_t top = H - sub_log;
         c->pool->run((size_t)1 << top, 1, [&](size_t sub) { host_sha_reduce_sub(nodes, H, top, sub); });
         host_sha_reduce(nodes, top);
     } else {
-        host_sha_reduce(nodes, H);
+        host_sha_reduce_from(c->h_mailbox + kMailDigests, nodes, H);
     }
     digest_words_to_bytes(nodes, root);
     c->t_host_hash += now_us() - t0;
     if (c->tail_have && c->tail_log == layer_log(c, tree) && tree >= 1) {
-        c->tail_vals.assign(c->h_mailbox + kMailValsOff, c->h_mailbox + kMailValsOff + ((size_t)1 << c->tail_log));
+        c->tail_vals = c->h_mailbox + kMailValsOff;
     }
     c->host_nodes[tree] = nodes;
     c->host_node_cnt[tree] = 2 * cnt - 1;
@@ -265,18 +265,11 @@
     if (!vals || !nodes) return fail(ZK_ERR_STATE, "host staging buffer exhausted");
     const zk_dom* d = c->dom;
     const uint32_t cc_m = to_mont(mulmod(beta_raw % P, d->fold_k[round]));
-    const uint32_t step_m = to_mont(powmod(c->hinv_host, (uint64_t)1 << round));
-    const uint32_t* in = c->tail_vals.data();
-    uint32_t xinv_m = to_mont(1);
-    for (size_t i = 0; i < half; ++i) {
-        uint32_t u = in[i], v = in[i + half];
-        vals[i] = add(mont_mul(add(u, v), d->inv2_mont), mont_mul(mont_mul(sub(u, v), xinv_m), cc_m));
-        xinv_m = mont_mul(xinv_m, step_m);
-    }
+    host_fold_layer(c->tail_vals, half, vals, cc_m, d->hinv_step_mont[round], d->inv2_mont);
     host_sha_leaves(vals, half, nodes + 8 * (half - 1));
     host_sha_reduce(nodes, log_out);
     digest_words_to_bytes(nodes, root);
-    c->tail_vals.assign(vals, vals + half);
+    c->tail_vals = vals;
     c->tail_log = log_out;
     c->t_host_hash += now_us() - t_begin;
     c->tree_steps[2 + round] = 0;
@@ -322,7 +315,7 @@
 };
 
 void begin_proof(zk_ctx* c) {
-    c->stage_used = 0; c->n_segs = 0; c->seg_words = 0; c->tail_log = 0; c->tail_have = false;
+    c->stage_used = 0; c->n_segs = 0; c->seg_words = 0; c->tail_log = 0; c->tail_have = false; c->tail_vals = nullptr;
     c->t_wait = c->t_host_hash = c->t_launch = 0;
     memset(c->host_nodes, 0, sizeof c->host_nodes);
     memset(c->host_node_cnt, 0, sizeof c->host_node_cnt);
@@ -337,7 +330,7 @@
 int settle_pending(zk_ctx* c) { return c->pending_top ? flush_host_parts(c) : (int)ZK_OK; }
 int last_layer_value(zk_ctx* c, uint32_t* out) {
     const uint32_t* v;
-    if (c->tail_have && c->tail_log == c->log_b) v = c->tail_vals.data();
+    if (c->tail_have && c->tail_log == c->log_b) v = c->tail_vals;
     else {
         HIPCHK(hipMemcpyAsync(c->h_small, c->d_layers + c->layer_off[1 + c->R], c->B * 4, hipMemcpyDeviceToHost, c->stream));
         HIPCHK(hipStreamSynchronize(c->stream));
@@ -406,9 +399,9 @@
     const uint32_t lg = layer_log(c, layer);
     const size_t m = (size_t)1 << lg;
     const uint32_t* src = c->d_layers + c->layer_off[layer];
-    if (lg <= 10) {
+    if (lg <= kMaxHostTail) {
         std::vector<uint32_t> v(m);
-        if (c->tail_have && c->tail_log == lg && layer >= 2) v.assign(c->tail_vals.begin(), c->tail_vals.begin() + m);
+        if (c->tail_have && c->tail_log == lg && layer >= 2) v.assign(c->tail_vals, c->tail_vals + m);
         else {
             HIPCHK(hipMemcpyAsync(v.data(), src, m * 4, hipMemcpyDeviceToHost, c->stream));
             HIPCHK(hipStreamSynchronize(c->stream));
@@ -595,9 +588,11 @@
     memcpy(c->info.roots[0], root, 32);
     uint32_t alpha[3];
     for (int i = 0; i < 3; ++i) alpha[i] = c->info.alpha_raw[i] = ch.get_u32();
+    double t_chal = now_us();
     if (c->coset) {
         if ((rc = do_compose(c, alpha)) || (rc = do_merkle(c, 1, true, false, fold_steps(R - c->stop, c->fold, 0)))) return rc;
     } else if ((rc = do_compose_commit(c, alpha))) return rc;
+    c->t_launch += now_us() - t_chal;
     if (can_gate(c, 0) && (rc = enqueue_gated_fold(c, 0))) return rc;
     if ((rc = read_commit(c, 1, root))) return rc;
     if (c->checks && (rc = check_degree(c, 1, (uint32_t)c->n - 1, "prover.rs:148-159/:169 (exact divisions, deg cp = n - 1)"))) return rc;
@@ -607,14 +602,17 @@
         if ((rc = prove_fold_rounds(c, ch))) return rc;
     } else for (uint32_t r = 0; r < R; ++r) {
         uint32_t beta = c->info.beta_raw[r] = ch.get_u32();
+        t_chal = now_us();
         if (c->gate_pending) {
             release_gated_fold(c, r, beta);
+            c->t_launch += now_us() - t_chal;
             if (can_gate(c, r + 1) && (rc = enqueue_gated_fold(c, r + 1))) return rc;
             if ((rc = read_commit(c, 2 + r, root))) return rc;
         } else if (c->tail_have && c->tail_log == c->L - r && c->L - r - 1 <= c->host_tail) {
             if ((rc = host_fold_commit(c, r, beta, root))) return rc;
         } else {
             if ((rc = do_fold_commit(c, r, beta))) return rc;
+            c->t_launch += now_us() - t_chal;
             if (can_gate(c, r + 1) && (rc = enqueue_gated_fold(c, r + 1))) return rc;
             if ((rc = read_commit(c, 2 + r, root))) return rc;
         }
@@ -623,7 +621,9 @@
         memcpy(c->info.roots[2 + r], root, 32);
     }
     lap("lde .. last root");
-    if (timing) fprintf(stderr, "[zk timing]   of which: waiting for the device %.1f us, host hashing (tops + tail) %.1f us\n", c->t_wait, c->t_host_hash);
+    if (timing)
+        fprintf(stderr, "[zk timing]   of which: waiting for the device %.1f us, host hashing (tops + tail) %.1f us, challenge to launch %.1f us\n", c->t_wait,
+                c->t_host_hash, c->t_launch);
     return prove_finish(c, ch, lap);
 }
 
@@ -762,7 +762,6 @@
     HIPCHK_C(hipStreamCreateWithFlags(&c->stream, hipStreamNonBlocking));
     if ((rc = dom_make(device, log_n, log_b, shift, tail, c->stream, &c->dom))) return bail(rc);
     c->tail = tail;
-    c->hinv_host = invmod(c->dom->h);
     c->device_bytes += c->dom->device_bytes;
     size_t off = 0;
     for (uint32_t l = 0; l <= c->R + 1; ++l) {
@@ -806,7 +805,7 @@
         if (hipDeviceGetAttribute(&can, hipDeviceAttributeCanUseStreamWaitValue, device) != hipSuccess) { can = 0; (void)hipGetLastError(); }
         c->early_ok = can != 0 && !tail;
     }
-    c->stage_words = (size_t)(c->R + 2) * ((size_t)16 << kMaxHostLog) + ((size_t)64 << kMaxHostLog);
+    c->stage_words = (size_t)(c->R + 2) * ((size_t)16 << kMaxHostLog) + ((size_t)36 << kMaxHostTail);
     const size_t seg_bytes = 4 * 34 * sizeof(ScatterSeg);
     HIPCHK_C(hipHostMalloc((void**)&c->h_stage, c->stage_words * 4 + seg_bytes, hipHostMallocMapped | hipHostMallocCoherent));
     HIPCHK_C(hipHostGetDevicePointer((void**)&c->d_stage, c->h_stage, 0));
@@ -966,8 +965,8 @@
 
 int zk_ctx_set_host_levels(zk_ctx* c, uint32_t top_log, uint32_t tail_log) {
     if (!c) return fail(ZK_ERR_INVALID, "null context");
-    if (top_log > kMaxHostLog || tail_log > kMaxHostLog || (tail_log && !top_log))
-        return fail(ZK_ERR_INVALID, "zk_ctx_set_host_levels: need top_log, tail_log <= %u, and top_log > 0 when tail_log > 0", kMaxHostLog);
+    if (top_log > kMaxHostLog || tail_log > kMaxHostTail || (tail_log && !top_log))
+        return fail(ZK_ERR_INVALID, "zk_ctx_set_host_levels: need top_log <= %u, tail_log <= %u, and top_log > 0 when tail_log > 0", kMaxHostLog, kMaxHostTail);
     c->host_top = top_log;
     c->host_tail = tail_log;
     return ctx_team(c);
```

Result: no change. 2.934 billion, median of 5 (+0.7%).
